# saidwivedi/InteractVLM

Hardware: AMD Instinct MI355X
Metric: images/sec end-to-end contact inference (higher is better)
Workload: dtype f16

## Files before the change

include/ivlm_hip.h:

```cpp
#ifndef IVLM_HIP_H
#define IVLM_HIP_H

#include <stddef.h>
#include <stdint.h>

#ifdef __cplusplus
extern "C" {
#endif

#define IVLM_OK 0
#define IVLM_ERR_INVALID_ARG (-1)
#define IVLM_ERR_WORKSPACE (-2)
#define IVLM_ERR_LAUNCH (-3)
#define IVLM_ERR_UNSUPPORTED (-4)

#define IVLM_F32 0
#define IVLM_BF16 1
#define IVLM_BF16_SPLIT 2
#define IVLM_F16 4
#define IVLM_F16_SPLIT 5
#define IVLM_FP8 3

#define IVLM_GEMM_A_F32 1
#define IVLM_GEMM_RES_F32 2
// ... 170 lines not shown
                     ivlm_stream_t stream);

int ivlm_llama_decode_attn_split(const void *qkv, void *kcache, void *kcache_lo, void *vcache, void *vcache_lo, int tmax, void *o,
                                 int H, int D, int pos, const int32_t *pos_dev, float theta, float scale, const float *cos_tab,
                                 const float *sin_tab, ivlm_stream_t stream);
int ivlm_llama_decode_attn_batch_split(const void *qkv, int64_t ldq, void *kcache, void *kcache_lo, void *vcache, void *vcache_lo,
                                       int64_t cache_stride, int tmax, void *o, int64_t ldo, int B, int H, int D,
                                       const int32_t *pos_dev, float theta, float scale, const float *cos_tab,
                                       const float *sin_tab, ivlm_stream_t stream);

typedef struct {
    int layers, hidden, heads, inter, max_len;
    float eps, theta;
    int fuse_attn_oproj;
} ivlm_llama_cfg;
typedef struct {
    const void *ln1, *qkv, *o, *ln2, *gu, *down;
} ivlm_llama_layer;
size_t ivlm_llama_prefill_workspace_bytes(const ivlm_llama_cfg *cfg, int T);
int ivlm_llama_prefill(const ivlm_llama_cfg *cfg, const ivlm_llama_layer *layers_host, const void *final_norm, void *kcache,
                       void *vcache, const float *cos_tab, const float *sin_tab, const float *x_in, int T, int pos0,
                       float *hidden_out, void *workspace, size_t workspace_bytes, ivlm_stream_t stream);
int ivlm_llama_prefill_f16(const ivlm_llama_cfg *cfg, const ivlm_llama_layer *layers16_host, const void *final_norm, void *kcache16,
                           void *vcache16, const float *cos_tab, const float *sin_tab, const float *x_in, int T, int pos0,
                           float *hidden_out, void *workspace, size_t workspace_bytes, ivlm_stream_t stream);
size_t ivlm_llama_decode_workspace_bytes(const ivlm_llama_cfg *cfg);
int ivlm_llama_decode_step(const ivlm_llama_cfg *cfg, const ivlm_llama_layer *layers_host, const void *final_norm, void *kcache,
                           void *vcache, const float *cos_tab, const float *sin_tab, const float *x_in, int32_t *pos_dev,
                           int advance, float *hidden_out, void *workspace, size_t workspace_bytes, ivlm_stream_t stream);
int ivlm_llama_decode_step_f16kv(const ivlm_llama_cfg *cfg, const ivlm_llama_layer *layers_host, const void *final_norm, void *kcache16,
                                 void *vcache16, const float *cos_tab, const float *sin_tab, const float *x_in, int32_t *pos_dev,
                                 int advance, float *hidden_out, void *workspace, size_t workspace_bytes, ivlm_stream_t stream);
typedef struct {
    const void *Pf, *Ef;
    const int32_t *ebase;
    const int32_t *patch_ptr;
    const int32_t *patch_col;
    const void *patch_val;
} ivlm_bf12m;
typedef struct {
    const void *ln1, *ln2;
    ivlm_bf12m qkv, o, gu, down;
} ivlm_llama_layer_bf12;
int ivlm_llama_decode_step_bf12(const ivlm_llama_cfg *cfg, const ivlm_llama_layer_bf12 *layers_host, const void *final_norm,
                                void *kcache, void *vcache, int cache_dtype, const float *cos_tab, const float *sin_tab,
                                const float *x_in, int32_t *pos_dev, int advance, float *hidden_out, void *workspace,
                                size_t workspace_bytes, ivlm_stream_t stream);
typedef struct {
    int layers_run, hidden, heads, inter, image_size, patch, kpad, tokens;
    float eps;
} ivlm_clip_cfg;
typedef struct {
    const void *patch_w, *pos, *cls_row, *pre_ln_w, *pre_ln_b;
} ivlm_clip_head;
typedef struct {
    const void *ln1_w, *ln1_b, *qkv_w, *qkv_b, *out_w, *out_b, *ln2_w, *ln2_b, *fc1_w, *fc1_b, *fc2_w, *fc2_b;
} ivlm_clip_layer;
size_t ivlm_clip_encode_workspace_bytes(const ivlm_clip_cfg *cfg, int B);
int ivlm_clip_encode(const ivlm_clip_cfg *cfg, const ivlm_clip_head *head, const ivlm_clip_layer *layers_host, const void *images,
                     int B, void *features_out, void *workspace, size_t workspace_bytes, ivlm_stream_t stream);
int ivlm_clip_encode_f16(const ivlm_clip_cfg *cfg, const ivlm_clip_head *head, const ivlm_clip_layer *layers16_host, const void *images,
                         int B, void *features_split_out, void *workspace, size_t workspace_bytes, ivlm_stream_t stream);

typedef struct {
    int embed_dim, depth, heads, grid, window, patch, img_size, out_chans, mlp_dim;
} ivlm_sam_cfg;
typedef struct {
    const void *patch_w, *patch_b, *pos_embed, *neck0_w, *neck1_w, *neck1_b, *neck2_w, *neck3_w, *neck3_b;
} ivlm_sam_head;
typedef struct {
    const void *norm1_w, *norm1_b, *qkv_w, *qkv_b, *rel_h, *rel_w, *rel_cat, *proj_w, *proj_b, *norm2_w, *norm2_b, *lin1_w, *lin1_b,
        *lin2_w, *lin2_b;
    int global_attn;
} ivlm_sam_block;
size_t ivlm_sam_encode_workspace_bytes(const ivlm_sam_cfg *cfg, int V);
int ivlm_sam_encode(const ivlm_sam_cfg *cfg, const ivlm_sam_head *head, const ivlm_sam_block *blocks_host, const void *images, int V,
                    float *embeddings_out, void *workspace, size_t workspace_bytes, ivlm_stream_t stream);
size_t ivlm_sam_encode_parity_workspace_bytes(const ivlm_sam_cfg *cfg, int V);
int ivlm_sam_encode_parity(const ivlm_sam_cfg *cfg, const ivlm_sam_head *head, const ivlm_sam_block *blocks_host, const void *images,
                           int V, float *embeddings_out, void *workspace, size_t workspace_bytes, ivlm_stream_t stream);
typedef struct {
    const void *lin1_w16, *lin2_w16;
} ivlm_sam_mlp_f16;
int ivlm_sam_encode_parity_f16mlp(const ivlm_sam_cfg *cfg, const ivlm_sam_head *head, const ivlm_sam_block *blocks_host,
                                  const ivlm_sam_mlp_f16 *mlp16_host, const void *images, int V, float *embeddings_out,
                                  void *workspace, size_t workspace_bytes, ivlm_stream_t stream);
typedef struct {
    const void *qkv_w16, *proj_w16, *lin1_w16, *lin2_w16, *qkv_b16, *rel_cat16;
} ivlm_sam_block_f16;
size_t ivlm_sam_encode_f16_workspace_bytes(const ivlm_sam_cfg *cfg, int V);
int ivlm_sam_encode_f16(const ivlm_sam_cfg *cfg, const ivlm_sam_head *head, const ivlm_sam_block *blocks_host,
                        const ivlm_sam_block_f16 *blocks16_host, const void *images, int V, float *embeddings_out, void *workspace,
                        size_t workspace_bytes, ivlm_stream_t stream);
int ivlm_bf16_to_f16(const void *src_bf16, void *dst_f16, int64_t n, ivlm_stream_t stream);

typedef struct {
    const void *w2, *b;
    int n, k;
} ivlm_lin;
typedef struct {
    ivlm_lin q, k, v, o;
} ivlm_dec_attn;
typedef struct {
    ivlm_dec_attn self_attn, t2i, i2t;
    const void *norm1_w, *norm1_b, *norm2_w, *norm2_b, *norm3_w, *norm3_b, *norm4_w, *norm4_b;
    ivlm_lin lin1, lin2;
} ivlm_dec_layer;
typedef struct {
    int C, heads, depth;
    const void *no_mask, *key_pe, *out_tokens;
    ivlm_dec_layer layers[4];
    ivlm_dec_attn final_attn;
    const void *norm_final_w, *norm_final_b, *up_ln_w, *up_ln_b;
    ivlm_lin up0, up1, hyper[3], iou[3];
} ivlm_sam_dec;
size_t ivlm_sam_decode_workspace_bytes(int V, int grid, int C, int n_text, int mlp_dim);
int ivlm_sam_decode(const ivlm_sam_dec *weights, int V, int grid, int n_text, const float *image_embeddings,
                    const float *text_embeds, float *low_res_out, float *iou_out, void *workspace, size_t workspace_bytes,
                    ivlm_stream_t stream);

int ivlm_gemm_splitk_choice(int M, int N, int K, int act, int has_rms);
int ivlm_stages_splitk_fused(int on);

int ivlm_gemv1_bf12(const float *x, const void *P, int64_t ldp, const void *E, int64_t lde, const int32_t *ebase,
                    const int32_t *patch_ptr, const int32_t *patch_col, const void *patch_val, void *C, const void *bias,
                    const void *residual, int N, int K, int act, int out_f32, const void *rms_w, float rms_eps, int flags,
                    ivlm_stream_t stream);
int ivlm_gemv1_bf12m(const float *x, const void *Pf, const void *Ef, const int32_t *ebase, const int32_t *patch_ptr,
                     const int32_t *patch_col, const void *patch_val, void *C, const void *bias, const void *residual, int N, int K,
                     int act, int out_f32, const void *rms_w, float rms_eps, int flags, ivlm_stream_t stream);
int ivlm_llama_decode_attn_parts(const float *qkv, int cache_dtype, void *kcache, void *vcache, int tmax, float *parts, int H, int D,
                                 int pos, const int32_t *pos_dev, float theta, float scale, const float *cos_tab, const float *sin_tab,
                                 ivlm_stream_t stream);
int ivlm_gemv1_bf12m_parts(const float *parts, int D, const void *Pf, const void *Ef, const int32_t *ebase, const int32_t *patch_ptr,
                           const int32_t *patch_col, const void *patch_val, void *C, const void *bias, const void *residual, int N, int K,
                           int act, int out_f32, int flags, ivlm_stream_t stream);
int ivlm_pack_bf12m_count(const void *w, int N_valid, int n_rows, int K, int32_t *ebase, int32_t *patch_ptr, ivlm_stream_t stream);
int ivlm_pack_bf12m_fill(const void *w, int N_valid, int n_rows, int K, const int32_t *ebase, const int32_t *patch_ptr, void *Pf, void *Ef,
                         int32_t *patch_col, void *patch_val, ivlm_stream_t stream);
int ivlm_gemv16_bf12m(const float *x, int64_t lda, int M, const void *Pf, const void *Ef, const int32_t *ebase,
                      const int32_t *patch_ptr, const int32_t *patch_col, const void *patch_val, void *C, int64_t ldc, const void *bias,
                      const void *residual, int64_t ldr, int N, int K, int act, int out_f32, const void *rms_w, float rms_eps, int flags,
                      ivlm_stream_t stream);
void ivlm_gemv16_bf12m_tuning(int tiles_per_block);
int ivlm_decode_parts_tuning(int ranges);
void ivlm_gemv1_bf12m_tuning(int wide_max_blocks);
int ivlm_gemv1_bf12m_staging(int form);
int ivlm_unpack_bf12(const void *P, int64_t ldp, const void *E, int64_t lde, const int32_t *ebase, const int32_t *patch_ptr,
                     const int32_t *patch_col, const void *patch_val, int N, int K, void *w_out, ivlm_stream_t stream);

int ivlm_argmax_f32(const float *x, int rows, int cols, int32_t *out, ivlm_stream_t stream);
int ivlm_argmax_f32_bump(const float *x, int rows, int cols, int32_t *out, int32_t *bump, ivlm_stream_t stream);

int ivlm_im2col_nchw(const void *x, void *out, int B, int C, int H, int W, int ks, int stride, int Kpad,
                     ivlm_stream_t stream);
int ivlm_im2col3x3_nhwc(const void *x, void *out, int B, int H, int W, int C, ivlm_stream_t stream);
int ivlm_im2col3x3_nhwc_strided(const void *x, int64_t ldx, void *out, int64_t ldo, int B, int H, int W, int C,
                                ivlm_stream_t stream);
int ivlm_gather_rows(void *dst, int dst_kind, int64_t ldd, const void *src, int src_dtype, int64_t lds, const int32_t *idx,
                     const void *add, int add_dtype, int64_t lda, int64_t rows, int cols, const float *fp8_scale,
                     ivlm_stream_t stream);
int ivlm_amax(const void *x, int dtype, int64_t n, float *out, ivlm_stream_t stream);
int ivlm_add_rows(void *out, int out_kind, const void *a, int a_dtype, const void *b, int b_dtype, int64_t rows, int cols,
                  int64_t b_rows, int op, ivlm_stream_t stream);
int ivlm_fill_rows(void *dst, int64_t ldd, const int32_t *idx, int64_t n_idx, const void *row, int cols,
                   ivlm_stream_t stream);
int ivlm_dense_pe(const void *gauss, void *pe, int pe_dtype, int h, int w, int F, ivlm_stream_t stream);
int ivlm_rope_kv(void *qkv, int64_t ld, int T, int H, int D, int pos0, float theta, void *kcache, void *vcache,
                 const float *cos_tab, const float *sin_tab, ivlm_stream_t stream);
int ivlm_rope_kv_f16(void *qkv, int64_t ld, int T, int H, int D, int pos0, float theta, void *kcache, void *vcache,
                     const float *cos_tab, const float *sin_tab, ivlm_stream_t stream);
int ivlm_rope_kv_split(void *qkv, int64_t ld, int T, int H, int D, int pos0, void *kcache, void *kcache_lo, void *vcache,
                       void *vcache_lo, const float *cos_tab, const float *sin_tab, ivlm_stream_t stream);
int ivlm_llama_attn_oproj(const float *qkv, void *kcache, void *vcache, int tmax, float *attn_scratch, const void *wo,
                          const float *x, float *x_out, int H, int D, float theta, float scale, const float *cos_tab,
                          const float *sin_tab, const int32_t *pos_dev, const int32_t *step_dev, int32_t *counter,
                          int32_t *status, ivlm_stream_t stream);
int ivlm_rope_table(float *cos_tab, float *sin_tab, int T, int D, float theta, ivlm_stream_t stream);
int ivlm_normalize_pad_u8(const uint8_t *src, int H, int W, int y0, int x0, int ch, int cw, const float *mean3_host,
                          const float *std3_host, void *out, int out_bf16, int OH, int OW, ivlm_stream_t stream);
int ivlm_mask_dot(const void *up, const void *hyper, int dtype, float *low, int B, int gh, int gw, int C,
                  ivlm_stream_t stream);

size_t ivlm_h_geo_workspace_bytes(int n);
int ivlm_h_geo_metric(const float *dist, const float *pred, const float *gt, int B, int n, float *out, void *workspace,
                      size_t workspace_bytes, ivlm_stream_t stream);
int ivlm_contact_prf(const float *gt, const float *pred, int B, int n, float thr, float *out, ivlm_stream_t stream);
int ivlm_spmv_csr(const int32_t *row_ptr, const int32_t *col, const float *val, const float *x, int B, int rows,
                  int cols, float *y, ivlm_stream_t stream);

int ivlm_contact_band_census(const float *p, int64_t ld, int B, int Nv, const float *thr, int J, float margin, int32_t *counts,
                             float *mindist, ivlm_stream_t stream);
size_t ivlm_mask_band_census_workspace_bytes(void);
int ivlm_mask_band_census(const float *logits, int V, int64_t HW, const int32_t *ent_pix, const int32_t *row_ptr, int n_rows,
                          float thr_p, float margin_p, int32_t *counts, void *workspace, size_t workspace_bytes,
                          ivlm_stream_t stream);

#define IVLM_SEG_GT_U8 0
#define IVLM_SEG_GT_I32 1
#define IVLM_SEG_GT_F32 2
size_t ivlm_seg_iou_workspace_bytes(int V);
int ivlm_seg_iou_counts(const float *pred, const void *gt, int gt_dtype, int V, int H, int W, int ignore_label, int32_t *out,
                        void *workspace, size_t workspace_bytes, ivlm_stream_t stream);
#define IVLM_AFFORD_MAX_N 4096
#define IVLM_AFFORD_MAX_T 64
int ivlm_afford_metrics(const float *gt, const float *pred, int B, int n, const float *thresholds, int T, float mae_div,
                        float *out, int32_t *valid, ivlm_stream_t stream);

#define IVLM_CONTACT_PAIR_CHAIN 512
size_t ivlm_contact_pair_workspace_bytes(int B, int N_o, int N_h);
int ivlm_contact_pair(const float *o, const float *h, const void *p, const void *q, int p_dtype, int B, int N_o, int N_h,
                      int64_t o_batch_stride, int64_t h_batch_stride, float *value_out, float *grad_o, float *grad_h,
                      void *workspace, size_t workspace_bytes, ivlm_stream_t stream);

#define IVLM_ICP_ESTIMATE_SCALE 1
#define IVLM_ICP_ALLOW_REFLECTION 2
#define IVLM_ICP_REQUERY 4
size_t ivlm_contact_icp_workspace_bytes(int B, int N_o);
int ivlm_contact_icp(const float *x, const float *y, const float *xn, const float *yn, const float *w, const float *init_R,
                     const float *init_T, const float *init_s, int B, int N_o, int N_h, int64_t x_batch_stride, int64_t y_batch_stride,
                     int64_t xn_batch_stride, int64_t yn_batch_stride, int64_t w_batch_stride, int max_iterations, float relative_rmse_thr,
                     int flags, float *R_out, float *T_out, float *s_out, float *rmse_out, int32_t *converged_out, int32_t *iterations_out,
                     int32_t *nn_idx_out, float *hist_R, float *hist_T, float *hist_s, void *workspace, size_t workspace_bytes,
                     ivlm_stream_t stream);

int ivlm_points_align(const float *X, const float *Y, const float *w, int B, int N, int64_t x_batch_stride, int64_t y_batch_stride,
                      int64_t w_batch_stride, int flags, float *R_out, float *T_out, float *s_out, void *workspace, size_t workspace_bytes,
                      ivlm_stream_t stream);

int ivlm_contact_nearest(const float *q, const float *t, int D, int B, int N_o, int N_h, int64_t q_batch_stride, int64_t t_batch_stride,
                         int32_t *idx_out, float *d2_out, ivlm_stream_t stream);

int ivlm_contact_normal_filter(const float *obj_normals, const float *human_normals, int N_o, int N_h, float c_pos, float c_neg,
                               int has_neg, uint8_t *keep_out, ivlm_stream_t stream);

#define IVLM_SILHOUETTE_CHAIN 32
#define IVLM_SILHOUETTE_POS_ULPS 12
#define IVLM_SILHOUETTE_REL_ULPS 6
#define IVLM_SILHOUETTE_EXP_ULPS 3
#define IVLM_SILHOUETTE_T_ULPS 8
size_t ivlm_soft_silhouette_workspace_bytes(int B, int N, int F, int H, int W);
int ivlm_soft_silhouette_forward(const float *verts, const int32_t *faces, int B, int N, int F, int H, int W, float fx, float fy,
                                 float px, float py, float sigma, float blur_radius, float *alpha_out, void *workspace,
                                 size_t workspace_bytes, ivlm_stream_t stream);
int ivlm_soft_silhouette_backward(const float *verts, const int32_t *vert_face_offsets, const int32_t *vert_face_list,
                                  const float *grad_alpha, int B, int N, int F, int H, int W, float fx, float fy, float px, float py,
                                  float sigma, float blur_radius, float *grad_verts_out, void *workspace, size_t workspace_bytes,
                                  ivlm_stream_t stream);

#define IVLM_SILHOUETTE_TERMS_CHAIN 1
#define IVLM_SILHOUETTE_TERMS_WORKSPACE(B, H) ((size_t)(B) * (size_t)(H) * 40)
int ivlm_silhouette_terms(const float *alpha, const float *target, int64_t target_batch_stride, int B, int H, int W, float *loss_out,
                          float *centroid_out, double *sums, const float *g_loss, const float *g_centroid, float *grad_alpha_out,
                          void *workspace, size_t workspace_bytes, ivlm_stream_t stream);

#define IVLM_POSE_CHUNK 1024
#define IVLM_POSE_CHAIN 1
#define IVLM_POSE_FWD_ULPS 6
#define IVLM_POSE_GRAD_ULPS 16
size_t ivlm_pose_transform_workspace_bytes(int B, int N);
int ivlm_pose_transform_forward(const float *verts, const float *rot6d, const float *translation, const float *scale, int B, int N,
                                float *out, ivlm_stream_t stream);
int ivlm_pose_transform_backward(const float *verts, const float *rot6d, const float *scale, const float *grad_out, int B, int N,
                                 float *grad_rot6d, float *grad_translation, float *grad_scale, void *workspace,
                                 size_t workspace_bytes, ivlm_stream_t stream);

size_t ivlm_raster_workspace_bytes(int n_verts_or_points, int H, int W);
int ivlm_rasterize_mesh(const float *verts, int nv, const int32_t *faces, int nf, const float *cam12_host,
                        float fov_deg, int H, int W, int32_t *p2v, float *bary, int32_t *pix_to_face,
                        void *workspace, size_t workspace_bytes, ivlm_stream_t stream);
int ivlm_rasterize_points(const float *pts, int np, const float *cam12_host, float fov_deg, float radius, int H,
                          int W, int32_t *map, void *workspace, size_t workspace_bytes, ivlm_stream_t stream);
int ivlm_phong_shade(const int32_t *p2v, const float *bary, const float *verts, const float *normals, const float *colors,
                     int npix, const float *light3_host, const float *cam3_host, float ambient, float diffuse,
                     float specular, float shininess, const float *bg3_host, uint8_t *out_rgb, ivlm_stream_t stream);

#ifdef __cplusplus
}
#endif
#endif
```

interactvlm_amd/csrc/elementwise.hip:

```cpp
#include "kernels.h"

namespace ivlm {
namespace {

constexpr int kT = 256;

inline int grid_for(int64_t work_items, int max_blocks = 8192) {
    int64_t b = (work_items + kT - 1) / kT;
    if (b < 1) b = 1;
    return (int)(b < max_blocks ? b : max_blocks);
}

__global__ __launch_bounds__(kT) void im2col_nchw_kernel(const bf16_t* __restrict__ x, bf16_t* __restrict__ out, int B,
                                                         int C, int H, int W, int ks, int stride, int Kpad) {
    const int gh = (H - ks) / stride + 1, gw = (W - ks) / stride + 1;
    const int K = C * ks * ks;
    const int64_t total = (int64_t)B * gh * gw * (Kpad >> 3);
    for (int64_t i = (int64_t)blockIdx.x * kT + threadIdx.x; i < total; i += (int64_t)gridDim.x * kT) {
        const int c8 = (int)(i % (Kpad >> 3));
        const int64_t row = i / (Kpad >> 3);
        const int gx = (int)(row % gw), gy = (int)((row / gw) % gh), b = (int)(row / ((int64_t)gw * gh));
        bf16_t v[8];
#pragma unroll
        for (int e = 0; e < 8; ++e) {
            const int col = c8 * 8 + e;
            bf16_t val = 0;
            if (col < K) {
                const int c = col / (ks * ks), r = col - c * ks * ks, ky = r / ks, kx = r - ky * ks;
                val = x[(((int64_t)b * C + c) * H + gy * stride + ky) * W + gx * stride + kx];
            }
            v[e] = val;
        }
        *reinterpret_cast<uint4*>(out + row * Kpad + c8 * 8) = *reinterpret_cast<const uint4*>(v);
    }
}

__global__ __launch_bounds__(kT) void im2col3x3_nhwc_kernel(const bf16_t* __restrict__ x, bf16_t* __restrict__ out,
                                                            int B, int H, int W, int C, int64_t ldx, int64_t ldo) {
    const int c8n = C >> 3;
    const int64_t total = (int64_t)B * H * W * 9 * c8n;
    for (int64_t i = (int64_t)blockIdx.x * kT + threadIdx.x; i < total; i += (int64_t)gridDim.x * kT) {
        const int c8 = (int)(i % c8n);
        const int tap = (int)((i / c8n) % 9);
        const int64_t row = i / ((int64_t)c8n * 9);
        const int xx = (int)(row % W), yy = (int)((row / W) % H), b = (int)(row / ((int64_t)W * H));
        const int sy = yy + tap / 3 - 1, sx = xx + tap % 3 - 1;
        uint4 v = make_uint4(0, 0, 0, 0);
        if (sy >= 0 && sy < H && sx >= 0 && sx < W)
            v = *reinterpret_cast<const uint4*>(x + (((int64_t)b * H + sy) * W + sx) * ldx + c8 * 8);
        *reinterpret_cast<uint4*>(out + row * ldo + tap * C + c8 * 8) = v;
    }
}

__device__ __forceinline__ void load8(const void* base, int kind, int64_t elem, float* f) {
    if (kind == 1) {
        const float4* p = reinterpret_cast<const float4*>(static_cast<const float*>(base) + elem);
        const float4 a = p[0], b = p[1];
        f[0] = a.x; f[1] = a.y; f[2] = a.z; f[3] = a.w; f[4] = b.x; f[5] = b.y; f[6] = b.z; f[7] = b.w;
    } else {
        const uint4 u = *reinterpret_cast<const uint4*>(static_cast<const bf16_t*>(base) + elem);
        f[0] = __uint_as_float(u.x << 16); f[1] = __uint_as_float(u.x & 0xffff0000u);
        f[2] = __uint_as_float(u.y << 16); f[3] = __uint_as_float(u.y & 0xffff0000u);
        f[4] = __uint_as_float(u.z << 16); f[5] = __uint_as_float(u.z & 0xffff0000u);
        f[6] = __uint_as_float(u.w << 16); f[7] = __uint_as_float(u.w & 0xffff0000u);
    }
}
__device__ __forceinline__ uint2 pack_fp8x8(const float* f, float inv_scale) {
    float c[8];
#pragma unroll
    for (int j = 0; j < 8; ++j) c[j] = fminf(fmaxf(f[j] * inv_scale, -448.0f), 448.0f);
    uint32_t a = 0, b = 0;
    a = __builtin_amdgcn_cvt_pk_fp8_f32(c[0], c[1], a, false);
    a = __builtin_amdgcn_cvt_pk_fp8_f32(c[2], c[3], a, true);
    b = __builtin_amdgcn_cvt_pk_fp8_f32(c[4], c[5], b, false);
    b = __builtin_amdgcn_cvt_pk_fp8_f32(c[6], c[7], b, true);
    return make_uint2(a, b);
}

__device__ __forceinline__ void store8(void* base, int kind, int64_t elem, int cols, const float* f, float inv_scale = 1.0f) {
    if (kind == 3) {
        *reinterpret_cast<uint2*>(static_cast<uint8_t*>(base) + elem) = pack_fp8x8(f, inv_scale);
        return;
    }
    if (kind == 1) {
        float4* p = reinterpret_cast<float4*>(static_cast<float*>(base) + elem);
        p[0] = make_float4(f[0], f[1], f[2], f[3]);
        p[1] = make_float4(f[4], f[5], f[6], f[7]);
        return;
    }
    bf16_t* o = static_cast<bf16_t*>(base) + elem;
    *reinterpret_cast<uint4*>(o) = make_uint4(pack_bf16x2(f[0], f[1]), pack_bf16x2(f[2], f[3]), pack_bf16x2(f[4], f[5]),
                                              pack_bf16x2(f[6], f[7]));
    if (kind == 2) {
        float l[8];
#pragma unroll
        for (int j = 0; j < 8; ++j) l[j] = f[j] - bf16_to_f32(f32_to_bf16(f[j]));
        *reinterpret_cast<uint4*>(o + cols) = make_uint4(pack_bf16x2(l[0], l[1]), pack_bf16x2(l[2], l[3]),
                                                         pack_bf16x2(l[4], l[5]), pack_bf16x2(l[6], l[7]));
    }
}

__global__ __launch_bounds__(kT) void gather_rows_kernel(void* __restrict__ dst, int dst_kind, int64_t ldd,
                                                         const void* __restrict__ src, int src_kind, int64_t lds_,
                                                         const int32_t* __restrict__ idx, const void* __restrict__ add,
                                                         int add_kind, int64_t lda, int64_t rows, int cols,
                                                         const float* __restrict__ scale) {
    const int c8n = cols >> 3;
    const int64_t total = rows * c8n;
    const float inv_scale = scale ? 1.0f / *scale : 1.0f;
    for (int64_t i = (int64_t)blockIdx.x * kT + threadIdx.x; i < total; i += (int64_t)gridDim.x * kT) {
        const int c8 = (int)(i % c8n);
        const int64_t r = i / c8n;
        const int64_t s = idx ? (int64_t)idx[r] : r;
        float v[8] = {0.f, 0.f, 0.f, 0.f, 0.f, 0.f, 0.f, 0.f};
        if (s >= 0) load8(src, src_kind, s * lds_ + c8 * 8, v);
        if (add) {
            float a[8];
            load8(add, add_kind, r * lda + c8 * 8, a);
#pragma unroll
            for (int j = 0; j < 8; ++j) v[j] += a[j];
        }
        store8(dst, dst_kind, r * ldd + c8 * 8, cols, v, inv_scale);
    }
}

__global__ __launch_bounds__(kT) void amax_kernel(const void* __restrict__ x, int kind, int64_t n8, float* __restrict__ out) {
    float m = 0.0f;
    for (int64_t i = (int64_t)blockIdx.x * kT + threadIdx.x; i < n8; i += (int64_t)gridDim.x * kT) {
        float v[8];
        load8(x, kind, i * 8, v);
#pragma unroll
        for (int j = 0; j < 8; ++j) m = fmaxf(m, fabsf(v[j]));
    }
    m = wave_max(m);
    if ((threadIdx.x & 63) == 0) atomicMax(reinterpret_cast<unsigned int*>(out), __float_as_uint(m));
}

__global__ __launch_bounds__(kT) void fill_rows_kernel(bf16_t* __restrict__ dst, int64_t ldd, const int32_t* __restrict__ idx,
                                                       int64_t n_idx, const bf16_t* __restrict__ row, int cols) {
    const int c8n = cols >> 3;
    const int64_t total = n_idx * c8n;
    for (int64_t i = (int64_t)blockIdx.x * kT + threadIdx.x; i < total; i += (int64_t)gridDim.x * kT) {
        const int c8 = (int)(i % c8n);
        const int64_t r = idx[i / c8n];
        *reinterpret_cast<uint4*>(dst + r * ldd + c8 * 8) = *reinterpret_cast<const uint4*>(row + c8 * 8);
    }
}

__global__ __launch_bounds__(kT) void bf16_to_f16_kernel(const bf16_t* __restrict__ src, uint16_t* __restrict__ dst, int64_t n) {
    const int64_t n8 = n >> 3;
    for (int64_t i = (int64_t)blockIdx.x * kT + threadIdx.x; i < n8; i += (int64_t)gridDim.x * kT) {
        const uint4 u = *reinterpret_cast<const uint4*>(src + i * 8);
        const uint32_t w[4] = {u.x, u.y, u.z, u.w};
        uint4 o;
        uint32_t* ow = reinterpret_cast<uint32_t*>(&o);
#pragma unroll
        for (int j = 0; j < 4; ++j) ow[j] = pack_f16x2(__uint_as_float(w[j] << 16), __uint_as_float(w[j] & 0xffff0000u));
        *reinterpret_cast<uint4*>(dst + i * 8) = o;
    }
    if (blockIdx.x == 0 && threadIdx.x < (n & 7)) {
        const int64_t i = n8 * 8 + threadIdx.x;
        dst[i] = (uint16_t)(pack_f16x2(bf16_to_f32(src[i]), 0.f) & 0xffffu);
    }
}

__global__ __launch_bounds__(kT) void add_rows_kernel(void* __restrict__ out, int out_kind, const void* __restrict__ a,
                                                      int a_kind, const void* __restrict__ b, int b_kind, int64_t rows,
                                                      int cols, int64_t b_rows, int op) {
    const int c8n = cols >> 3;
    const int64_t total = rows * c8n;
    const int64_t ldo = out_kind == 2 ? 2 * (int64_t)cols : cols;
    for (int64_t i = (int64_t)blockIdx.x * kT + threadIdx.x; i < total; i += (int64_t)gridDim.x * kT) {
        const int c8 = (int)(i % c8n);
        const int64_t r = i / c8n;
        float va[8], vb[8];
        load8(a, a_kind, r * cols + c8 * 8, va);
        load8(b, b_kind, (r % b_rows) * cols + c8 * 8, vb);
#pragma unroll
        for (int j = 0; j < 8; ++j) va[j] = op ? va[j] * vb[j] : va[j] + vb[j];
        store8(out, out_kind, r * ldo + c8 * 8, cols, va);
    }
}

__global__ __launch_bounds__(kT) void dense_pe_kernel(const float* __restrict__ gauss ,
                                                      void* __restrict__ pe , int pe_f32, int h, int w, int F) {
    const int64_t total = (int64_t)h * w * 2 * F;
    for (int64_t i = (int64_t)blockIdx.x * kT + threadIdx.x; i < total; i += (int64_t)gridDim.x * kT) {
        const int c = (int)(i % (2 * F));
        const int64_t p = i / (2 * F);
        const int xx = (int)(p % w), yy = (int)(p / w);
        const int f = c < F ? c : c - F;
        const float cx = 2.0f * (((float)xx + 0.5f) / (float)w) - 1.0f;
        const float cy = 2.0f * (((float)yy + 0.5f) / (float)h) - 1.0f;
        float t = cx * gauss[f] + cy * gauss[F + f];
        t = 6.283185307179586f * t;
        const float val = c < F ? sinf(t) : cosf(t);
        if (pe_f32) static_cast<float*>(pe)[i] = val;
        else static_cast<bf16_t*>(pe)[i] = f32_to_bf16(val);
    }
}

__global__ __launch_bounds__(kT) void rope_table_kernel(float* __restrict__ ct, float* __restrict__ st, int T, int D,
                                                        float theta) {
    const int half = D >> 1;
    const int i = blockIdx.x * kT + threadIdx.x;
    if (i >= T * half) return;
    const int j = i % half, pos = i / half;
    const float ang = (float)pos * powf(theta, -(float)(2 * j) / (float)D);
    ct[i] = cosf(ang);
    st[i] = sinf(ang);
}

template <bool F16>
__global__ __launch_bounds__(kT) void rope_kv_kernel(bf16_t* __restrict__ qkv, int64_t ld, int T, int H, int D,
                                                     int pos0, float theta, bf16_t* __restrict__ kcache,
                                                     bf16_t* __restrict__ vcache, const float* __restrict__ ct,
                                                     const float* __restrict__ stab) {
    const int half = D >> 1;
    const int64_t total = (int64_t)T * H * half;
    for (int64_t i = (int64_t)blockIdx.x * kT + threadIdx.x; i < total; i += (int64_t)gridDim.x * kT) {
        const int j = (int)(i % half);
        const int h = (int)((i / half) % H);
        const int t = (int)(i / ((int64_t)half * H));
        const int pos = pos0 + t;
        float c, s;
        if (ct) {
            c = ct[pos * half + j];
            s = stab[pos * half + j];
        } else {
            const float ang = (float)pos * powf(theta, -(float)(2 * j) / (float)D);
            c = cosf(ang);
            s = sinf(ang);
        }
        bf16_t* row = qkv + (int64_t)t * ld;
        bf16_t* q = row + h * D;
        bf16_t* k = row + (int64_t)H * D + h * D;
        const bf16_t* v = row + 2 * (int64_t)H * D + h * D;
        const float q0 = h16_to_f32<F16>(q[j]), q1 = h16_to_f32<F16>(q[j + half]);
        const float k0 = h16_to_f32<F16>(k[j]), k1 = h16_to_f32<F16>(k[j + half]);
        const bf16_t qa = f32_to_h16<F16>(q0 * c - q1 * s), qb = f32_to_h16<F16>(q1 * c + q0 * s);
        const bf16_t ka = f32_to_h16<F16>(k0 * c - k1 * s), kb = f32_to_h16<F16>(k1 * c + k0 * s);
        q[j] = qa;
        q[j + half] = qb;
        k[j] = ka;
        k[j + half] = kb;
        if (kcache) {
            bf16_t* kc = kcache + ((int64_t)pos * H + h) * D;
            bf16_t* vc = vcache + ((int64_t)pos * H + h) * D;
            kc[j] = ka;
            kc[j + half] = kb;
            vc[j] = v[j];
            vc[j + half] = v[j + half];
        }
    }
}

__global__ __launch_bounds__(kT) void rope_kv_split_kernel(bf16_t* __restrict__ qkv, int64_t ld, int T, int H, int D, int pos0,
                                                           bf16_t* __restrict__ kcache, bf16_t* __restrict__ kcache_lo,
                                                           bf16_t* __restrict__ vcache, bf16_t* __restrict__ vcache_lo,
                                                           const float* __restrict__ ct, const float* __restrict__ stab) {
    const int half = D >> 1;
    const int64_t total = (int64_t)T * H * half;
    const int64_t lo = 3 * (int64_t)H * D;
    for (int64_t i = (int64_t)blockIdx.x * kT + threadIdx.x; i < total; i += (int64_t)gridDim.x * kT) {
        const int j = (int)(i % half);
        const int h = (int)((i / half) % H);
        const int t = (int)(i / ((int64_t)half * H));
        const int pos = pos0 + t;
        const float c = ct[pos * half + j], s = stab[pos * half + j];
        bf16_t* row = qkv + (int64_t)t * ld;
        bf16_t* q = row + h * D;
        bf16_t* k = row + (int64_t)H * D + h * D;
        const bf16_t* v = row + 2 * (int64_t)H * D + h * D;
        auto val = [&](const bf16_t* p, int e) { return bf16_to_f32(p[e]) + bf16_to_f32(p[lo + e]); };
        const float q0 = val(q, j), q1 = val(q, j + half), k0 = val(k, j), k1 = val(k, j + half);
        const float qa = q0 * c - q1 * s, qb = q1 * c + q0 * s, ka = k0 * c - k1 * s, kb = k1 * c + k0 * s;
        auto put = [&](bf16_t* p, int e, float x, bf16_t* ch, bf16_t* cl) {
            const bf16_t hi = f32_to_bf16(x), l = f32_to_bf16(x - bf16_to_f32(hi));
            p[e] = hi;
            p[lo + e] = l;
            if (ch) {
                ch[e] = hi;
                cl[e] = l;
            }
        };
        const int64_t crow = ((int64_t)pos * H + h) * D;
        put(q, j, qa, nullptr, nullptr);
        put(q, j + half, qb, nullptr, nullptr);
        put(k, j, ka, kcache ? kcache + crow : nullptr, kcache ? kcache_lo + crow : nullptr);
        put(k, j + half, kb, kcache ? kcache + crow : nullptr, kcache ? kcache_lo + crow : nullptr);
        if (kcache) {
            vcache[crow + j] = v[j];
            vcache[crow + j + half] = v[j + half];
            vcache_lo[crow + j] = v[lo + j];
            vcache_lo[crow + j + half] = v[lo + j + half];
        }
    }
}

__global__ __launch_bounds__(kT) void mask_dot_kernel(const void* __restrict__ up, const void* __restrict__ hyper, int kind,
                                                      float* __restrict__ low, int B, int gh, int gw, int C) {
    const int64_t total = (int64_t)B * gh * gw * 16;
    for (int64_t i = (int64_t)blockIdx.x * kT + threadIdx.x; i < total; i += (int64_t)gridDim.x * kT) {
        const int sub = (int)(i & 15);
        const int64_t cell = i >> 4;
        const int xx = (int)(cell % gw), yy = (int)((cell / gw) % gh), b = (int)(cell / ((int64_t)gw * gh));
        const int dy = sub >> 3, dx = (sub >> 2) & 1, dy2 = (sub >> 1) & 1, dx2 = sub & 1;
        float acc = 0.0f;
        for (int c = 0; c < C; c += 8) {
            float a[8], h[8];
            load8(up, kind, i * C + c, a);
            load8(hyper, kind, (int64_t)b * C + c, h);
#pragma unroll
            for (int j = 0; j < 8; ++j) acc += a[j] * h[j];
        }
        const int Y = 4 * yy + 2 * dy + dy2, X = 4 * xx + 2 * dx + dx2;
        low[((int64_t)b * 4 * gh + Y) * (4 * gw) + X] = acc;
    }
}

template <typename T>
__global__ __launch_bounds__(kT) void normalize_pad_kernel(const uint8_t* __restrict__ src, int W, int y0, int x0,
                                                           int ch, int cw, float m0, float m1, float m2, float s0,
                                                           float s1, float s2, T* __restrict__ out, int OH, int OW) {
    const int64_t total = (int64_t)OH * OW;
    for (int64_t i = (int64_t)blockIdx.x * kT + threadIdx.x; i < total; i += (int64_t)gridDim.x * kT) {
        const int x = (int)(i % OW), y = (int)(i / OW);
        float r = 0.f, g = 0.f, b = 0.f;
        if (y < ch && x < cw) {
            const uint8_t* p = src + ((int64_t)(y0 + y) * W + (x0 + x)) * 3;
            r = ((float)p[0] - m0) / s0;
            g = ((float)p[1] - m1) / s1;
            b = ((float)p[2] - m2) / s2;
        }
        if (sizeof(T) == 2) {
            reinterpret_cast<bf16_t*>(out)[i] = f32_to_bf16(r);
            reinterpret_cast<bf16_t*>(out)[total + i] = f32_to_bf16(g);
            reinterpret_cast<bf16_t*>(out)[2 * total + i] = f32_to_bf16(b);
        } else {
            reinterpret_cast<float*>(out)[i] = r;
            reinterpret_cast<float*>(out)[total + i] = g;
            reinterpret_cast<float*>(out)[2 * total + i] = b;
        }
    }
}

}

int normalize_pad_u8(const uint8_t* src, int H, int W, int y0, int x0, int ch, int cw, const float* mean3,
                     const float* std3, void* out, int out_bf16, int OH, int OW, hipStream_t st) {
    if (!src || !out || !mean3 || !std3 || y0 < 0 || x0 < 0 || y0 + ch > H || x0 + cw > W || ch > OH || cw > OW)
        return IVLM_ERR_INVALID_ARG;
    const int grid = grid_for((int64_t)OH * OW);
    if (out_bf16)
        normalize_pad_kernel<bf16_t><<<grid, kT, 0, st>>>(src, W, y0, x0, ch, cw, mean3[0], mean3[1], mean3[2], std3[0],
                                                          std3[1], std3[2], static_cast<bf16_t*>(out), OH, OW);
    else
        normalize_pad_kernel<float><<<grid, kT, 0, st>>>(src, W, y0, x0, ch, cw, mean3[0], mean3[1], mean3[2], std3[0],
                                                         std3[1], std3[2], static_cast<float*>(out), OH, OW);
    return ivlm_launch_status();
}

int im2col_nchw(const bf16_t* x, bf16_t* out, int B, int C, int H, int W, int ks, int stride, int Kpad,
                hipStream_t st) {
    if (!x || !out || (Kpad & 7) || Kpad < C * ks * ks) return IVLM_ERR_INVALID_ARG;
    const int gh = (H - ks) / stride + 1, gw = (W - ks) / stride + 1;
    im2col_nchw_kernel<<<grid_for((int64_t)B * gh * gw * (Kpad >> 3)), kT, 0, st>>>(x, out, B, C, H, W, ks, stride, Kpad);
    return ivlm_launch_status();
}
int im2col3x3_nhwc(const bf16_t* x, bf16_t* out, int B, int H, int W, int C, hipStream_t st, int64_t ldx, int64_t ldo) {
    if (!x || !out || (C & 7)) return IVLM_ERR_INVALID_ARG;
    if (ldx == 0) ldx = C;
    if (ldo == 0) ldo = 9 * (int64_t)C;
    if (ldx < C || ldo < 9 * (int64_t)C || ((ldx | ldo) & 7)) return IVLM_ERR_INVALID_ARG;
    im2col3x3_nhwc_kernel<<<grid_for((int64_t)B * H * W * 9 * (C >> 3)), kT, 0, st>>>(x, out, B, H, W, C, ldx, ldo);
    return ivlm_launch_status();
}
int gather_rows(void* dst, int dst_kind, int64_t ldd, const void* src, int src_kind, int64_t lds_, const int32_t* idx,
                const void* add, int add_kind, int64_t lda, int64_t rows, int cols, hipStream_t st, const float* scale) {
    if (!dst || !src || rows <= 0 || (cols & 7) || (ldd & 7) || (lds_ & 7) || (lda & 7)) return IVLM_ERR_INVALID_ARG;
    if (dst_kind < 0 || dst_kind > 3 || (src_kind & ~1) || (add_kind & ~1)) return IVLM_ERR_INVALID_ARG;
    if (dst_kind == 2 && ldd < 2 * (int64_t)cols) return IVLM_ERR_INVALID_ARG;
    if (dst_kind == 3 && !scale) return IVLM_ERR_INVALID_ARG;
    gather_rows_kernel<<<grid_for(rows * (cols >> 3)), kT, 0, st>>>(dst, dst_kind, ldd, src, src_kind, lds_, idx, add,
                                                                    add_kind, lda, rows, cols, scale);
    return ivlm_launch_status();
}
int amax(const void* x, int kind, int64_t n, float* out, hipStream_t st) {
    if (!x || !out || n <= 0 || (n & 7) || (kind & ~1)) return IVLM_ERR_INVALID_ARG;
    amax_kernel<<<grid_for(n >> 3, 2048), kT, 0, st>>>(x, kind, n >> 3, out);
    return ivlm_launch_status();
}
int add_rows(void* out, int out_kind, const void* a, int a_kind, const void* b, int b_kind, int64_t rows, int cols,
             int64_t b_rows, hipStream_t st, int op) {
    if (!out || !a || !b || rows <= 0 || b_rows <= 0 || (cols & 7)) return IVLM_ERR_INVALID_ARG;
    if (out_kind < 0 || out_kind > 2 || (a_kind & ~1) || (b_kind & ~1)) return IVLM_ERR_INVALID_ARG;
    add_rows_kernel<<<grid_for(rows * (cols >> 3)), kT, 0, st>>>(out, out_kind, a, a_kind, b, b_kind, rows, cols, b_rows, op);
    return ivlm_launch_status();
}
int fill_rows(bf16_t* dst, int64_t ldd, const int32_t* idx, int64_t n_idx, const bf16_t* row, int cols, hipStream_t st) {
    if (n_idx == 0) return IVLM_OK;
    if (!dst || !idx || !row || n_idx < 0 || (cols & 7) || (ldd & 7)) return IVLM_ERR_INVALID_ARG;
    fill_rows_kernel<<<grid_for(n_idx * (cols >> 3)), kT, 0, st>>>(dst, ldd, idx, n_idx, row, cols);
    return ivlm_launch_status();
}
int dense_pe(const float* gauss, void* pe, int pe_f32, int h, int w, int F, hipStream_t st) {
    if (!gauss || !pe) return IVLM_ERR_INVALID_ARG;
    dense_pe_kernel<<<grid_for((int64_t)h * w * 2 * F), kT, 0, st>>>(gauss, pe, pe_f32, h, w, F);
    return ivlm_launch_status();
}
int rope_kv(bf16_t* qkv, int64_t ld, int T, int H, int D, int pos0, float theta, bf16_t* kcache, bf16_t* vcache,
            hipStream_t st, const float* cos_tab, const float* sin_tab, int f16) {
    if (!qkv || T <= 0 || (D & 1) || (kcache && !vcache) || (cos_tab && !sin_tab)) return IVLM_ERR_INVALID_ARG;
    if (f16)
        rope_kv_kernel<true><<<grid_for((int64_t)T * H * (D >> 1)), kT, 0, st>>>(qkv, ld, T, H, D, pos0, theta, kcache, vcache,
                                                                                 cos_tab, sin_tab);
    else
        rope_kv_kernel<false><<<grid_for((int64_t)T * H * (D >> 1)), kT, 0, st>>>(qkv, ld, T, H, D, pos0, theta, kcache, vcache,
                                                                                  cos_tab, sin_tab);
    return ivlm_launch_status();
}
int rope_kv_split(bf16_t* qkv, int64_t ld, int T, int H, int D, int pos0, bf16_t* kcache, bf16_t* kcache_lo, bf16_t* vcache,
                  bf16_t* vcache_lo, const float* cos_tab, const float* sin_tab, hipStream_t st) {
    if (!qkv || T <= 0 || (D & 1) || !cos_tab || !sin_tab || ld < 6LL * H * D) return IVLM_ERR_INVALID_ARG;
    if (kcache && (!kcache_lo || !vcache || !vcache_lo)) return IVLM_ERR_INVALID_ARG;
    rope_kv_split_kernel<<<grid_for((int64_t)T * H * (D >> 1)), kT, 0, st>>>(qkv, ld, T, H, D, pos0, kcache, kcache_lo, vcache,
                                                                             vcache_lo, cos_tab, sin_tab);
    return ivlm_launch_status();
}
int rope_table(float* cos_tab, float* sin_tab, int T, int D, float theta, hipStream_t st) {
    if (!cos_tab || !sin_tab || T <= 0 || (D & 1)) return IVLM_ERR_INVALID_ARG;
    rope_table_kernel<<<(T * (D >> 1) + kT - 1) / kT, kT, 0, st>>>(cos_tab, sin_tab, T, D, theta);
    return ivlm_launch_status();
}
int mask_dot(const void* up, const void* hyper, int kind, float* low, int B, int gh, int gw, int C, hipStream_t st) {
    if (!up || !hyper || !low || (C & 7) || (kind & ~1)) return IVLM_ERR_INVALID_ARG;
    mask_dot_kernel<<<grid_for((int64_t)B * gh * gw * 16), kT, 0, st>>>(up, hyper, kind, low, B, gh, gw, C);
    return ivlm_launch_status();
}

}

extern "C" {
#define BF(p) static_cast<bf16_t*>(p)
#define CBF(p) static_cast<const bf16_t*>(p)
int ivlm_im2col_nchw(const void* x, void* out, int B, int C, int H, int W, int ks, int stride, int Kpad,
                     ivlm_stream_t s) {
    ivlm_enter();
    return ivlm::im2col_nchw(CBF(x), BF(out), B, C, H, W, ks, stride, Kpad, ivlm_stream(s));
}
int ivlm_im2col3x3_nhwc(const void* x, void* out, int B, int H, int W, int C, ivlm_stream_t s) {
    ivlm_enter();
    return ivlm::im2col3x3_nhwc(CBF(x), BF(out), B, H, W, C, ivlm_stream(s));
}
int ivlm_im2col3x3_nhwc_strided(const void* x, int64_t ldx, void* out, int64_t ldo, int B, int H, int W, int C, ivlm_stream_t s) {
    ivlm_enter();
    return ivlm::im2col3x3_nhwc(CBF(x), BF(out), B, H, W, C, ivlm_stream(s), ldx, ldo);
}
int ivlm_gather_rows(void* dst, int dst_kind, int64_t ldd, const void* src, int src_dtype, int64_t lds_, const int32_t* idx,
                     const void* add, int add_dtype, int64_t lda, int64_t rows, int cols, const float* fp8_scale,
                     ivlm_stream_t s) {
    ivlm_enter();
    const int k = dst_kind == IVLM_F32 ? 1 : (dst_kind == IVLM_BF16 ? 0 : (dst_kind == IVLM_BF16_SPLIT ? 2 : (dst_kind == IVLM_FP8 ? 3 : -1)));
    return ivlm::gather_rows(dst, k, ldd, src, src_dtype == IVLM_F32, lds_, idx, add, add_dtype == IVLM_F32, lda, rows, cols,
                             ivlm_stream(s), fp8_scale);
}
int ivlm_amax(const void* x, int dtype, int64_t n, float* out, ivlm_stream_t s) {
    ivlm_enter();
    return ivlm::amax(x, dtype == IVLM_F32, n, out, ivlm_stream(s));
}
int ivlm_add_rows(void* out, int out_kind, const void* a, int a_dtype, const void* b, int b_dtype, int64_t rows, int cols,
                  int64_t b_rows, int op, ivlm_stream_t s) {
    ivlm_enter();
    return ivlm::add_rows(out, out_kind == IVLM_F32 ? 1 : (out_kind == IVLM_BF16 ? 0 : (out_kind == IVLM_BF16_SPLIT ? 2 : -1)),
                          a, a_dtype == IVLM_F32, b, b_dtype == IVLM_F32, rows, cols, b_rows, ivlm_stream(s), op);
}
int ivlm_fill_rows(void* dst, int64_t ldd, const int32_t* idx, int64_t n_idx, const void* row, int cols, ivlm_stream_t s) {
    ivlm_enter();
    return ivlm::fill_rows(BF(dst), ldd, idx, n_idx, CBF(row), cols, ivlm_stream(s));
}
int ivlm_dense_pe(const void* gauss, void* pe, int pe_dtype, int h, int w, int F, ivlm_stream_t s) {
    ivlm_enter();
    return ivlm::dense_pe(static_cast<const float*>(gauss), pe, pe_dtype == IVLM_F32, h, w, F, ivlm_stream(s));
}
int ivlm_rope_kv(void* qkv, int64_t ld, int T, int H, int D, int pos0, float theta, void* kcache, void* vcache,
                 const float* cos_tab, const float* sin_tab, ivlm_stream_t s) {
    ivlm_enter();
    return ivlm::rope_kv(BF(qkv), ld, T, H, D, pos0, theta, BF(kcache), BF(vcache), ivlm_stream(s), cos_tab, sin_tab);
}
int ivlm_rope_kv_f16(void* qkv, int64_t ld, int T, int H, int D, int pos0, float theta, void* kcache, void* vcache,
                     const float* cos_tab, const float* sin_tab, ivlm_stream_t s) {
    ivlm_enter();
    return ivlm::rope_kv(BF(qkv), ld, T, H, D, pos0, theta, BF(kcache), BF(vcache), ivlm_stream(s), cos_tab, sin_tab, 1);
}
int ivlm_rope_kv_split(void* qkv, int64_t ld, int T, int H, int D, int pos0, void* kcache, void* kcache_lo, void* vcache,
                       void* vcache_lo, const float* cos_tab, const float* sin_tab, ivlm_stream_t s) {
    ivlm_enter();
    return ivlm::rope_kv_split(BF(qkv), ld, T, H, D, pos0, BF(kcache), BF(kcache_lo), BF(vcache), BF(vcache_lo), cos_tab, sin_tab,
                               ivlm_stream(s));
}
int ivlm_bf16_to_f16(const void* src, void* dst, int64_t n, ivlm_stream_t s) {
    ivlm_enter();
    if (n == 0) return IVLM_OK;
    if (!src || !dst || n < 0 || ((uintptr_t)src & 15) || ((uintptr_t)dst & 15)) return IVLM_ERR_INVALID_ARG;
    ivlm::bf16_to_f16_kernel<<<ivlm::grid_for((n >> 3) + 1), ivlm::kT, 0, ivlm_stream(s)>>>(CBF(src), static_cast<uint16_t*>(dst), n);
    return ivlm_launch_status();
}
int ivlm_rope_table(float* cos_tab, float* sin_tab, int T, int D, float theta, ivlm_stream_t s) {
    ivlm_enter();
    return ivlm::rope_table(cos_tab, sin_tab, T, D, theta, ivlm_stream(s));
}
int ivlm_mask_dot(const void* up, const void* hyper, int dtype, float* low, int B, int gh, int gw, int C, ivlm_stream_t s) {
    ivlm_enter();
    return ivlm::mask_dot(up, hyper, dtype == IVLM_F32, low, B, gh, gw, C, ivlm_stream(s));
}
int ivlm_normalize_pad_u8(const uint8_t* src, int H, int W, int y0, int x0, int ch, int cw, const float* mean3_host,
                          const float* std3_host, void* out, int out_bf16, int OH, int OW, ivlm_stream_t s) {
    ivlm_enter();
    return ivlm::normalize_pad_u8(src, H, W, y0, x0, ch, cw, mean3_host, std3_host, out, out_bf16, OH, OW,
                                  ivlm_stream(s));
}
#undef BF
#undef CBF
}
```

interactvlm_amd/csrc/gemv.hip:

```cpp
#include <stdlib.h>

#include <algorithm>

#include "gemv_common.h"

namespace ivlm {
namespace {

constexpr int kMaxM = 8;

__device__ __forceinline__ float dot8(const u32x4_t& w, const u32x4_t& x) {
    float acc = 0.0f;
#pragma unroll
    for (int j = 0; j < 4; ++j) {
        acc += __uint_as_float(w[j] << 16) * __uint_as_float(x[j] << 16);
        acc += __uint_as_float(w[j] & 0xffff0000u) * __uint_as_float(x[j] & 0xffff0000u);
    }
    return acc;
}

__device__ __forceinline__ float dot8f(const u32x4_t& w, const f32x4v_t& xa, const f32x4v_t& xb) {
    float acc = __uint_as_float(w[0] << 16) * xa[0];
    acc = fmaf(__uint_as_float(w[0] & 0xffff0000u), xa[1], acc);
    acc = fmaf(__uint_as_float(w[1] << 16), xa[2], acc);
// ... 157 lines not shown
                } else {
                    bf16_t* C = static_cast<bf16_t*>(g.C) + (int64_t)m * g.ldc;
                    C[n0] = f32_to_bf16(v0);
                    if (n1 != n0) C[n1] = f32_to_bf16(v1);
                }
            }
        }
#pragma unroll
        for (int m = 0; m < M; ++m) a0[m] = a1[m] = 0.0f;
    };

    u32x4_t wa0[U], wb0[U], wa1[U], wb1[U];
    if (nsteps > 0) issue(wa0, wb0, 0);
    if (XLDS) prologue();
    for (int s2 = 0; s2 < nsteps; s2 += 2) {
        if (s2 + 1 < nsteps) issue(wa1, wb1, s2 + 1);
        consume(wa0, wb0, s2);
        if (s2 + 1 < nsteps) {
            if (s2 + 2 < nsteps) issue(wa0, wb0, s2 + 2);
            consume(wa1, wb1, s2 + 1);
        }
    }
}

constexpr int kG1Waves = kRowWaves;

template <bool RMS, int KS>
__global__ __launch_bounds__(64 * kG1Waves, 8) void gemv1_kernel(GemmArgs g) {
    extern __shared__ __attribute__((aligned(16))) unsigned char smem[];
    __shared__ float s_red[kG1Waves];
    __shared__ float s_val[kG1Waves];
    constexpr int U = 8 / KS;
    const int lane = threadIdx.x & 63, wave = threadIdx.x >> 6;
    const int nchunk = g.K >> 3;
    f32x4v_t* xf = reinterpret_cast<f32x4v_t*>(smem);
    const int row = blockIdx.x * (kG1Waves / KS) + wave / KS;
    const bool live = row < g.N;
    const u32x4_t* wp = reinterpret_cast<const u32x4_t*>(g.W + (int64_t)(live ? row : g.N - 1) * g.ldw);
    const int cpp = KS == 1 ? nchunk : ((nchunk + 64 * KS - 1) / (64 * KS)) * 64;
    const int c_lo = (wave % KS) * cpp, c_hi = min(nchunk, c_lo + cpp);
    u32x4_t w[U];
#pragma unroll
    for (int u = 0; u < U; ++u) w[u] = __builtin_nontemporal_load(wp + min(c_lo + lane + 64 * u, nchunk - 1));
    stage_row_f32<RMS, false>(g, xf, nchunk, 64 * kG1Waves, s_red, lane, wave);
    __syncthreads();
    float acc = 0.0f;
    constexpr int UH = U / 2;
    for (int c = c_lo + lane; c < c_hi; c += 64 * U) {
#pragma unroll
        for (int hf = 0; hf < 2; ++hf) {
#pragma unroll
            for (int u = hf * UH; u < (hf + 1) * UH; ++u) {
                const int cc = c + 64 * u;
                if (cc < c_hi) acc += dot8f(w[u], xf[cc], xf[nchunk + cc]);
            }
#pragma unroll
            for (int u = hf * UH; u < (hf + 1) * UH; ++u) {
                const int nc = c + 64 * (U + u);
                if (nc < c_hi) w[u] = __builtin_nontemporal_load(wp + nc);
            }
        }
    }
    acc = wave_sum(acc);
    if (KS > 1) {
        if (lane == 0) s_val[wave] = acc;
        __syncthreads();
        if (wave % KS) return;
        acc = s_val[wave];
#pragma unroll
        for (int i = 1; i < KS; ++i) acc += s_val[wave + i];
    }
    finish_row<RMS, KS == 1>(g, acc, row, live, lane, wave, s_red, s_val);
}

typedef __attribute__((ext_vector_type(2))) float f32x2v_t;

__device__ __forceinline__ float dot16_fp8(const u32x4_t& w, const f32x4v_t& a0, const f32x4v_t& a1, const f32x4v_t& b0,
                                           const f32x4v_t& b1, float acc) {
    const f32x4v_t* xs[4] = {&a0, &a1, &b0, &b1};
#pragma unroll
    for (int j = 0; j < 4; ++j) {
        const f32x2v_t lo = __builtin_amdgcn_cvt_pk_f32_fp8(w[j], false);
        const f32x2v_t hi = __builtin_amdgcn_cvt_pk_f32_fp8(w[j], true);
        const f32x4v_t& x = *xs[j];
        acc = fmaf(lo[0], x[0], acc);
        acc = fmaf(lo[1], x[1], acc);
        acc = fmaf(hi[0], x[2], acc);
        acc = fmaf(hi[1], x[3], acc);
    }
    return acc;
}

template <bool RMS>
__global__ __launch_bounds__(64 * kG1Waves, 8) void gemv1_fp8w_kernel(GemmArgs g) {
    extern __shared__ __attribute__((aligned(16))) unsigned char smem[];
    __shared__ float s_red[kG1Waves];
    __shared__ float s_val[kG1Waves];
    constexpr int U = 4;
    const int lane = threadIdx.x & 63, wave = threadIdx.x >> 6;
    const int nchunk = g.K >> 3;
    const int nw16 = g.K >> 4;
    f32x4v_t* xf = reinterpret_cast<f32x4v_t*>(smem);
    const int row = blockIdx.x * kG1Waves + wave;
    const bool live = row < g.N;
    const u32x4_t* wp = reinterpret_cast<const u32x4_t*>(reinterpret_cast<const uint8_t*>(g.W) + (int64_t)(live ? row : g.N - 1) * g.ldw);
    u32x4_t w[U];
#pragma unroll
    for (int u = 0; u < U; ++u) w[u] = __builtin_nontemporal_load(wp + min(lane + 64 * u, nw16 - 1));
    stage_row_f32<RMS, false>(g, xf, nchunk, 64 * kG1Waves, s_red, lane, wave);
    __syncthreads();
    float acc = 0.0f;
    for (int c = lane; c < nw16; c += 64 * U) {
        if (c != lane) {
#pragma unroll
            for (int u = 0; u < U; ++u)
                if (c + 64 * u < nw16) w[u] = __builtin_nontemporal_load(wp + c + 64 * u);
        }
#pragma unroll
        for (int u = 0; u < U; ++u) {
            const int cc = c + 64 * u;
            if (cc < nw16) acc = dot16_fp8(w[u], xf[2 * cc], xf[nchunk + 2 * cc], xf[2 * cc + 1], xf[nchunk + 2 * cc + 1], acc);
        }
    }
    acc = wave_sum(acc) * (*g.scale_w);
    finish_row<RMS>(g, acc, row, live, lane, wave, s_red, s_val);
}

int g_gemv1_ksplit = 0;
int g_gemv1_lds_floor = 0;

template <bool RMS, int KS>
static void launch_gemv1_ks(const GemmArgs& g, hipStream_t st) {
    const int rows_per_block = kG1Waves / KS;
    const int blocks = (g.N + rows_per_block - 1) / rows_per_block;
    size_t lds = (size_t)g.K * 4;
    if (blocks <= 256 && (size_t)g_gemv1_lds_floor > lds) lds = (size_t)g_gemv1_lds_floor;
    ivlm_launch_lds_cap<gemv1_kernel<RMS, KS>>(128 * 1024, dim3(blocks), dim3(64 * kG1Waves), lds, st, g);
}

static int launch_gemv1(const GemmArgs& g, hipStream_t st) {
    int ks = g_gemv1_ksplit > 0 ? g_gemv1_ksplit : 1;
    if (g.act == ACT_SWIGLU || g.K < 2048) ks = 1;
    if (ks == 2) {
        if (g.rms_w) launch_gemv1_ks<true, 2>(g, st);
        else launch_gemv1_ks<false, 2>(g, st);
    } else {
        if (g.rms_w) launch_gemv1_ks<true, 1>(g, st);
        else launch_gemv1_ks<false, 1>(g, st);
    }
    return ivlm_launch_status();
}

__global__ __launch_bounds__(1024) void argmax_kernel(const float* __restrict__ x, int cols, int32_t* __restrict__ out,
                                                      int32_t* __restrict__ bump) {
    __shared__ float sv[16];
    __shared__ int si[16];
    const float* r = x + (int64_t)blockIdx.x * cols;
    float best = -INFINITY;
    int bi = 0x7fffffff;
    auto take = [&](float v, int i) {
        if (v > best || (v == best && i < bi)) {
            best = v;
            bi = i;
        }
    };
    const int head = (int)(((16 - ((uintptr_t)r & 15)) & 15) >> 2);
    const int nhead = head < cols ? head : cols;
    if ((int)threadIdx.x < nhead) take(r[threadIdx.x], threadIdx.x);
    const int nvec = (cols - nhead) >> 2;
    const float4* rv = reinterpret_cast<const float4*>(r + nhead);
    for (int i = threadIdx.x; i < nvec; i += 1024) {
        const float4 v = rv[i];
        const int c = nhead + 4 * i;
        take(v.x, c);
        take(v.y, c + 1);
        take(v.z, c + 2);
        take(v.w, c + 3);
    }
    for (int i = nhead + 4 * nvec + threadIdx.x; i < cols; i += 1024) take(r[i], i);
#pragma unroll
    for (int off = 32; off > 0; off >>= 1) {
        const float ov = __shfl_xor(best, off, 64);
        const int oi = __shfl_xor(bi, off, 64);
        if (ov > best || (ov == best && oi < bi)) {
            best = ov;
            bi = oi;
        }
    }
    if ((threadIdx.x & 63) == 0) {
        sv[threadIdx.x >> 6] = best;
        si[threadIdx.x >> 6] = bi;
    }
    __syncthreads();
    if (threadIdx.x == 0) {
        for (int w = 1; w < 16; ++w)
            if (sv[w] > best || (sv[w] == best && si[w] < bi)) {
                best = sv[w];
                bi = si[w];
            }
        out[blockIdx.x] = bi;
        if (bump) bump[blockIdx.x] += 1;
    }
}

}

int g_gemv_max_blocks_per_cu = 0, g_gemv_rows2_min_n = 0;
int g_gemv_legacy = 0;
static int gemv_cu_count() {
    static int cus = 0;
    if (cus == 0) {
        int dev = 0;
        if (hipGetDevice(&dev) != hipSuccess || hipDeviceGetAttribute(&cus, hipDeviceAttributeMultiprocessorCount, dev) != hipSuccess ||
            cus <= 0)
            cus = 256;
    }
    return cus;
}

template <int M>
static int launch_gemv(const GemmArgs& g, hipStream_t st) {
    const size_t xbytes = (size_t)M * g.K * (g.a_f32 ? 4 : 2);
    const bool xlds = xbytes <= (g.a_f32 ? 60 : 48) * 1024;
    if (g.rms_w && !xlds) return IVLM_ERR_UNSUPPORTED;
    const int rows2_min = g_gemv_rows2_min_n > 0 ? g_gemv_rows2_min_n : 8192;
    const bool rows2 = g.act == ACT_SWIGLU || g.N > rows2_min;
    const int ngroups = rows2 ? (g.N + 1) / 2 : g.N;
    const size_t lds = xlds ? xbytes : 0;
    int per_cu = g_gemv_max_blocks_per_cu > 0 ? g_gemv_max_blocks_per_cu : 4;
    if (lds > 0) per_cu = std::min<int>(per_cu, std::max<int>(1, (int)((160 * 1024) / (lds + 512))));
    const int slots = gemv_cu_count() * per_cu;
    const int gpw = std::max(1, (ngroups + 4 * slots - 1) / (4 * slots));
    const int blocks = (ngroups + 4 * gpw - 1) / (4 * gpw);
#define IVLM_GEMV_GO(ROWS, RMS, XL, AF)                                                                            \
    do {                                                                                                           \
        constexpr auto kfn = gemv_kernel<M, ROWS, RMS, XL, AF>;                                                    \
        if (lds > 48 * 1024) ivlm_launch_lds_cap<kfn>(64 * 1024, dim3(blocks), dim3(256), lds, st, g);             \
        else ivlm_launch(kfn, dim3(blocks), dim3(256), lds, st, g);                                                \
    } while (0)
#define IVLM_GEMV_ROWS(ROWS)                                                                   \
    if (g.a_f32) {                                                                             \
        if (g.rms_w) IVLM_GEMV_GO(ROWS, true, true, true);                                     \
        else if (xlds) IVLM_GEMV_GO(ROWS, false, true, true);                                  \
        else IVLM_GEMV_GO(ROWS, false, false, true);                                           \
    } else {                                                                                   \
        if (g.rms_w) IVLM_GEMV_GO(ROWS, true, true, false);                                    \
        else if (xlds) IVLM_GEMV_GO(ROWS, false, true, false);                                 \
        else IVLM_GEMV_GO(ROWS, false, false, false);                                          \
    }
    if (rows2) { IVLM_GEMV_ROWS(2) } else { IVLM_GEMV_ROWS(1) }
#undef IVLM_GEMV_ROWS
#undef IVLM_GEMV_GO
    return ivlm_launch_status();
}

int gemv_bf16(const GemmArgs& g, hipStream_t st) {
    if (!g.A || !g.W || !g.C || g.M <= 0 || g.M > kMaxM || g.N <= 0 || g.K <= 0) return IVLM_ERR_INVALID_ARG;
    if ((g.K & 7) || (g.lda & (g.a_f32 ? 3 : 7)) || (g.ldw & 7) || g.batch != 1) return IVLM_ERR_UNSUPPORTED;
    if (g.act == ACT_SWIGLU && ((g.N & 1) || g.residual)) return IVLM_ERR_UNSUPPORTED;
    if (g.M == 1 && g.a_f32 && (size_t)g.K * 4 <= 60 * 1024 && !g_gemv_legacy) return launch_gemv1(g, st);
    switch (g.M) {
        case 1: return launch_gemv<1>(g, st);
        case 2: return launch_gemv<2>(g, st);
        case 3: return launch_gemv<3>(g, st);
        case 4: return launch_gemv<4>(g, st);
        case 5: return launch_gemv<5>(g, st);
        case 6: return launch_gemv<6>(g, st);
        case 7: return launch_gemv<7>(g, st);
        default: return launch_gemv<8>(g, st);
    }
}

int gemv1_fp8w(const GemmArgs& g, hipStream_t st) {
    if (!g.A || !g.W || !g.C || !g.scale_w || g.M != 1 || !g.a_f32 || g.N <= 0 || g.K <= 0) return IVLM_ERR_INVALID_ARG;
    if ((g.K & 15) || (g.ldw & 15) || (size_t)g.K * 4 > 60 * 1024) return IVLM_ERR_UNSUPPORTED;
    if (g.act == ACT_SWIGLU && ((g.N & 1) || g.residual)) return IVLM_ERR_UNSUPPORTED;
    const dim3 grid((g.N + kG1Waves - 1) / kG1Waves), block(64 * kG1Waves);
    if (g.rms_w) ivlm_launch_lds_cap<gemv1_fp8w_kernel<true>>(64 * 1024, grid, block, (size_t)g.K * 4, st, g);
    else ivlm_launch_lds_cap<gemv1_fp8w_kernel<false>>(64 * 1024, grid, block, (size_t)g.K * 4, st, g);
    return ivlm_launch_status();
}

int argmax_f32(const float* x, int rows, int cols, int32_t* out, hipStream_t st, int32_t* bump) {
    if (!x || !out || rows <= 0 || cols <= 0) return IVLM_ERR_INVALID_ARG;
    argmax_kernel<<<rows, 1024, 0, st>>>(x, cols, out, bump);
    return ivlm_launch_status();
}

}

extern "C" int ivlm_gemv_tuning(int max_blocks_per_cu, int rows2_min_n) {
    ivlm::g_gemv_legacy = max_blocks_per_cu < 0 ? 1 : 0;
    ivlm::g_gemv_max_blocks_per_cu = max_blocks_per_cu > 0 ? max_blocks_per_cu : 0;
    ivlm::g_gemv_rows2_min_n = rows2_min_n;
    return 0;
}

extern "C" void ivlm_gemv1_tuning(int ksplit) { ivlm::g_gemv1_ksplit = ksplit; }
extern "C" void ivlm_gemv1_lds_floor(int bytes) { ivlm::g_gemv1_lds_floor = bytes < 0 ? 0 : (bytes > 128 * 1024 ? 128 * 1024 : bytes); }

extern "C" int ivlm_gemv_fp8w(const float* x, const void* Wq, int64_t ldw, const float* scale_w, void* C, const void* bias,
                              const void* residual, int N, int K, int act, int out_f32, const void* rms_w, float rms_eps, int flags,
                              ivlm_stream_t stream) {
    ivlm_enter();
    ivlm::GemmArgs g = ivlm::gemv_row_args(x, C, bias, residual, N, K, act, out_f32, rms_w, rms_eps, flags);
    g.W = static_cast<const bf16_t*>(Wq);
    g.ldw = ldw;
    g.scale_w = scale_w;
    return ivlm::gemv1_fp8w(g, ivlm_stream(stream));
}

extern "C" int ivlm_argmax_f32(const float* x, int rows, int cols, int32_t* out, ivlm_stream_t stream) {
    ivlm_enter();
    return ivlm::argmax_f32(x, rows, cols, out, ivlm_stream(stream), nullptr);
}

extern "C" int ivlm_argmax_f32_bump(const float* x, int rows, int cols, int32_t* out, int32_t* bump, ivlm_stream_t stream) {
    ivlm_enter();
    return ivlm::argmax_f32(x, rows, cols, out, ivlm_stream(stream), bump);
}
```

interactvlm_amd/csrc/kernels.h:

```cpp
#pragma once
#include "ivlm_common.h"

namespace ivlm {

enum Act : int { ACT_NONE = 0, ACT_GELU = 1, ACT_QUICK_GELU = 2, ACT_RELU = 3, ACT_SILU = 4, ACT_SWIGLU = 5, ACT_SIGMOID = 6 };

struct SplitKFused {
    int32_t* count = nullptr;
    void* C = nullptr;
    const bf16_t* bias = nullptr;
    const bf16_t* residual = nullptr;
    int64_t ldc = 0, ldr = 0, c_lo = 0;
    int res_mod = 0, act = 0, out_f32 = 0, out_f16 = 0, out_split = 0, res_f32 = 0;
};
constexpr int kSplitKCounters = 4096;

struct GemmArgs {
    const bf16_t* A = nullptr;
    const bf16_t* W = nullptr;
    void* C = nullptr;
    const bf16_t* bias = nullptr;
    const bf16_t* residual = nullptr;
    int64_t lda = 0, ldw = 0, ldc = 0, ldr = 0;
    int res_mod = 0;
// ... 29 lines not shown

int layernorm(const void* x, int x_f32, const bf16_t* w, const bf16_t* b, void* y, int y_f32, int64_t rows, int cols, float eps,
              hipStream_t st, int gelu = 0, const int32_t* out_rows = nullptr, const float* fp8_scale = nullptr);
int rmsnorm(const void* x, int x_f32, const bf16_t* w, void* y, int y_f32, int64_t rows, int cols, float eps, hipStream_t st,
            const float* fp8_scale = nullptr);

struct AttnArgs {
    const bf16_t *q, *k, *v;
    bf16_t* o;
    int64_t q_bs, q_hs, q_rs;
    int64_t k_bs, k_hs, k_rs;
    int64_t v_bs, v_hs, v_rs;
    int64_t o_bs, o_hs, o_rs;
    int B, H, Sq, Sk, D;
    float scale;
    int causal;
    int q_pos0;
    const float* rel_h;
    const float* rel_w;
    int rel_kh, rel_kw;
    int kv_batch_div;
    int prescale_q;
    const bf16_t *q_lo = nullptr, *k_lo = nullptr, *v_lo = nullptr;
    bf16_t* o_lo = nullptr;
    int xcd_map = 1;
    int q_lo_level = 0;
    int f16 = 0;
};

int attention_bf16(const AttnArgs& a, hipStream_t st);
int attention_f32(const float* q, const float* k, const float* v, float* o, const int64_t* st12, int B, int H, int Sq, int Sk,
                  int D, float scale, int kv_div, hipStream_t st);
int relpos_bias(const bf16_t* q, int64_t q_bs, int64_t q_hs, int64_t q_rs, const bf16_t* tab_h, const bf16_t* tab_w,
                int B, int H, int SH, int SW, int D, float* rel_h, float* rel_w, hipStream_t st, const bf16_t* q_lo = nullptr);

int im2col_nchw(const bf16_t* x, bf16_t* out, int B, int C, int H, int W, int ks, int stride, int Kpad, hipStream_t st);
int im2col3x3_nhwc(const bf16_t* x, bf16_t* out, int B, int H, int W, int C, hipStream_t st, int64_t ldx = 0, int64_t ldo = 0);
int rope_kv_split(bf16_t* qkv, int64_t ld, int T, int H, int D, int pos0, bf16_t* kcache, bf16_t* kcache_lo, bf16_t* vcache,
                  bf16_t* vcache_lo, const float* cos_tab, const float* sin_tab, hipStream_t st);
int gather_rows(void* dst, int dst_kind, int64_t ldd, const void* src, int src_kind, int64_t lds_, const int32_t* idx,
                const void* add, int add_kind, int64_t lda, int64_t rows, int cols, hipStream_t st, const float* scale = nullptr);
int amax(const void* x, int kind, int64_t n, float* out, hipStream_t st);
int add_rows(void* out, int out_kind, const void* a, int a_kind, const void* b, int b_kind, int64_t rows, int cols,
             int64_t b_rows, hipStream_t st, int op = 0);
int fill_rows(bf16_t* dst, int64_t ldd, const int32_t* idx, int64_t n_idx, const bf16_t* row, int cols, hipStream_t st);
int dense_pe(const float* gauss, void* pe, int pe_f32, int h, int w, int F, hipStream_t st);
int rope_kv(bf16_t* qkv, int64_t ld, int T, int H, int D, int pos0, float theta, bf16_t* kcache, bf16_t* vcache,
            hipStream_t st, const float* cos_tab = nullptr, const float* sin_tab = nullptr, int f16 = 0);
int rope_table(float* cos_tab, float* sin_tab, int T, int D, float theta, hipStream_t st);
int normalize_pad_u8(const uint8_t* src, int H, int W, int y0, int x0, int ch, int cw, const float* mean3,
                     const float* std3, void* out, int out_bf16, int OH, int OW, hipStream_t st);
int mask_dot(const void* up, const void* hyper, int kind, float* low, int B, int gh, int gw, int C, hipStream_t st);

int contact_prf(const float* gt, const float* pred, int B, int n, float thr, float* out, hipStream_t st);
int spmv_csr(const int32_t* row_ptr, const int32_t* col, const float* val, const float* x, int B, int rows, int cols,
             float* y, hipStream_t st);

int contact_band_census(const float* p, int64_t ld, int B, int nv, const float* thr, int J, float margin, int32_t* counts,
                        float* mindist, hipStream_t st);
size_t mask_band_census_workspace_bytes();
int mask_band_census(const float* logits, int V, int64_t HW, const int32_t* ent_pix, const int32_t* row_ptr, int n_rows,
                     float thr_p, float margin_p, int32_t* counts, void* ws, size_t ws_bytes, hipStream_t st);

size_t seg_iou_workspace_bytes(int V);
int seg_iou_counts(const float* pred, const void* gt, int gt_dtype, int V, int H, int W, int ignore_label, int32_t* out, void* ws,
                   size_t ws_bytes, hipStream_t st);
int afford_metrics(const float* gt, const float* pred, int B, int n, const float* thresholds, int T, float mae_div, float* out,
                   int32_t* valid, hipStream_t st);

size_t contact_pair_workspace_bytes(int B, int n_o, int n_h);
int contact_pair(const float* o, const float* h, const void* p, const void* q, int p_dtype, int B, int n_o, int n_h,
                 int64_t o_bstride, int64_t h_bstride, float* value, float* grad_o, float* grad_h, void* ws, size_t ws_bytes,
                 hipStream_t st);

size_t soft_silhouette_workspace_bytes(int B, int N, int F, int H, int W);
int soft_silhouette_forward(const float* verts, const int32_t* faces, int B, int N, int F, int H, int W, float fx, float fy, float px,
                            float py, float sigma, float blur, float* alpha, void* ws, size_t ws_bytes, hipStream_t st);
int soft_silhouette_backward(const float* verts, const int32_t* vf_off, const int32_t* vf_list, const float* galpha, int B, int N, int F,
                             int H, int W, float fx, float fy, float px, float py, float sigma, float blur, float* gverts, void* ws,
                             size_t ws_bytes, hipStream_t st);
int silhouette_terms(const float* alpha, const float* target, int64_t t_bstride, int B, int H, int W, float* loss, float* centroid,
                     double* sums, const float* g_loss, const float* g_centroid, float* galpha, void* ws, size_t ws_bytes,
                     hipStream_t st);

size_t pose_transform_workspace_bytes(int B, int N);
int pose_transform_forward(const float* verts, const float* rot6d, const float* trans, const float* scale, int B, int N, float* out,
                           hipStream_t st);
int pose_transform_backward(const float* verts, const float* rot6d, const float* scale, const float* grad_out, int B, int N,
                            float* grad_r6, float* grad_t, float* grad_s, void* ws, size_t ws_bytes, hipStream_t st);

size_t contact_icp_workspace_bytes(int B, int n_o);
int contact_icp(const float* x, const float* y, const float* xn, const float* yn, const float* w, const float* init_R, const float* init_T,
                const float* init_s, int B, int n_o, int n_h, int64_t x_bs, int64_t y_bs, int64_t xn_bs, int64_t yn_bs, int64_t w_bs,
                int max_iterations, float relative_rmse_thr, int flags, float* R, float* T, float* s, float* rmse, int32_t* converged,
                int32_t* iterations, int32_t* nn_idx, float* hist_R, float* hist_T, float* hist_s, void* ws, size_t ws_bytes,
                hipStream_t st);
int points_align(const float* X, const float* Y, const float* w, int B, int n, int64_t x_bs, int64_t y_bs, int64_t w_bs, int flags,
                 float* R, float* T, float* s, void* ws, size_t ws_bytes, hipStream_t st);
int contact_nearest(const float* q, const float* t, int D, int B, int n_o, int n_h, int64_t q_bs, int64_t t_bs, int32_t* idx, float* d2,
                    hipStream_t st);
int contact_normal_filter(const float* on, const float* hn, int n_o, int n_h, float c_pos, float c_neg, int has_neg, uint8_t* keep,
                          hipStream_t st);

size_t raster_workspace_bytes(int n_prims_verts, int H, int W);
int rasterize_mesh(const float* verts, int nv, const int32_t* faces, int nf, const float* cam12_host, float fov_deg,
                   int H, int W, int32_t* p2v, float* bary, int32_t* pix_to_face, void* ws, size_t ws_bytes,
                   hipStream_t st);
int rasterize_points(const float* pts, int np, const float* cam12_host, float fov_deg, float radius, int H, int W,
                     int32_t* map, void* ws, size_t ws_bytes, hipStream_t st);

int phong_shade(const int32_t* p2v, const float* bary, const float* verts, const float* normals, const float* colors, int npix,
                const float* light3_host, const float* cam3_host, float ambient, float diffuse, float specular, float shininess,
                const float* bg3_host, uint8_t* out, hipStream_t st);

int llama_decode_attn(const void* qkv, int io_f32, bf16_t* kcache, bf16_t* vcache, int tmax, void* o, int H, int D, int pos,
                      float theta, float scale, hipStream_t st, const float* cos_tab = nullptr, const float* sin_tab = nullptr,
                      const int32_t* pos_dev = nullptr, bf16_t* kcache_lo = nullptr, bf16_t* vcache_lo = nullptr, int cache_f16 = 0);
int llama_decode_attn_batch(const void* qkv, int io_f32, int64_t ldq, bf16_t* kcache, bf16_t* vcache, int64_t cache_stride,
                            int tmax, void* o, int64_t ldo, int B, int H, int D, const int32_t* pos_dev, float theta, float scale,
                            const float* cos_tab, const float* sin_tab, hipStream_t st, bf16_t* kcache_lo = nullptr,
                            bf16_t* vcache_lo = nullptr, int cache_f16 = 0);

size_t llama_decode_attn_splitkv_scratch_bytes(int H, int D);
int llama_decode_attn_splitkv(const float* qkv, bf16_t* kcache, bf16_t* vcache, int tmax, float* o, int H, int D, int pos, float theta,
                              float scale, hipStream_t st, const float* cos_tab, const float* sin_tab, const int32_t* pos_dev,
                              int cache_f16, void* scratch, size_t scratch_bytes);

extern int g_decode_parts_S;
constexpr int kDecodePartsMaxS = 4;
__host__ __device__ constexpr int decode_parts_stride(int D) { return D + 4; }
int llama_decode_attn_parts(const float* qkv, bf16_t* kcache, bf16_t* vcache, int tmax, float* parts, int H, int D, int pos, float theta,
                            float scale, hipStream_t st, const float* cos_tab, const float* sin_tab, const int32_t* pos_dev,
                            int cache_f16);

size_t llama_decode_attn_batch_prefix_scratch_bytes(int B, int H, int D);
int llama_decode_attn_batch_prefix(const void* qkv, int io_f32, int64_t ldq, bf16_t* kcache, bf16_t* vcache, int64_t cache_stride,
                                   int tmax, void* o, int64_t ldo, int B, int H, int D, const int32_t* pos_dev,
                                   const int32_t* prefix_len_dev, float theta, float scale, const float* cos_tab,
                                   const float* sin_tab, int cache_f16, void* scratch, size_t scratch_bytes, hipStream_t st);
int llama_verify_attn(const float* qkv, int k, bf16_t* kcache, bf16_t* vcache, int tmax, float* o, int H, int D, const int32_t* pos_dev,
                      float theta, float scale, const float* cos_tab, const float* sin_tab, int cache_f16, hipStream_t st);
int spec_accept(const int32_t* amax, const int32_t* fed, const int32_t* nd_dev, int k, int32_t* n_acc, int32_t* tok, int32_t* pos,
                hipStream_t st);

int llama_attn_oproj(const float* qkv, bf16_t* kcache, bf16_t* vcache, int tmax, float* attn_scratch, const bf16_t* wo,
                     const float* x, float* x_out, int H, int D, float theta, float scale, const float* cos_tab,
                     const float* sin_tab, const int32_t* pos_dev, const int32_t* step_dev, int32_t* counter, int32_t* status,
                     hipStream_t st);
int gemm_splitk_choice(int M, int N, int K, int act, int has_rms);

int gemv_bf16(const GemmArgs& g, hipStream_t st);
int gemv1_fp8w(const GemmArgs& g, hipStream_t st);
int gemv_mfma_bf16(const GemmArgs& g, hipStream_t st);
int argmax_f32(const float* x, int rows, int cols, int32_t* out, hipStream_t st, int32_t* bump = nullptr);

}
```

interactvlm_amd/csrc/norm.hip:

```cpp
#include "kernels.h"

namespace ivlm {
namespace {

constexpr int kMaxChunks = 16;

__device__ __forceinline__ void unpack8(const uint4& u, float* f) {
    f[0] = __uint_as_float(u.x << 16); f[1] = __uint_as_float(u.x & 0xffff0000u);
    f[2] = __uint_as_float(u.y << 16); f[3] = __uint_as_float(u.y & 0xffff0000u);
    f[4] = __uint_as_float(u.z << 16); f[5] = __uint_as_float(u.z & 0xffff0000u);
    f[6] = __uint_as_float(u.w << 16); f[7] = __uint_as_float(u.w & 0xffff0000u);
}
__device__ __forceinline__ uint4 pack8(const float* f) {
    return make_uint4(pack_bf16x2(f[0], f[1]), pack_bf16x2(f[2], f[3]), pack_bf16x2(f[4], f[5]),
                      pack_bf16x2(f[6], f[7]));
}

template <bool RMS, int MAXC, bool GELU, bool XF32, bool YF32>
__global__ __launch_bounds__(256) void norm_kernel(const void* __restrict__ xv, const bf16_t* __restrict__ w,
                                                   const bf16_t* __restrict__ b, void* __restrict__ yv, int64_t rows,
                                                   int cols, float eps, const int32_t* __restrict__ out_rows,
                                                   const float* __restrict__ fp8_scale, int y_split) {
    const int lane = threadIdx.x & 63;
    const int64_t row = (int64_t)blockIdx.x * 4 + (threadIdx.x >> 6);
    if (row >= rows) return;
    const int nchunk = cols >> 3;
    const uint4* xr = reinterpret_cast<const uint4*>(static_cast<const bf16_t*>(xv) + row * cols);
    const float4* xr4 = reinterpret_cast<const float4*>(static_cast<const float*>(xv) + row * cols);
    float v[MAXC][8];
    float s = 0.0f;
#pragma unroll
    for (int c = 0; c < MAXC; ++c) {
        const int idx = c * 64 + lane;
        if (idx < nchunk) {
            if (XF32) {
                const float4 a = xr4[2 * idx], bq = xr4[2 * idx + 1];
                v[c][0] = a.x; v[c][1] = a.y; v[c][2] = a.z; v[c][3] = a.w;
                v[c][4] = bq.x; v[c][5] = bq.y; v[c][6] = bq.z; v[c][7] = bq.w;
            } else {
                unpack8(xr[idx], v[c]);
            }
#pragma unroll
            for (int j = 0; j < 8; ++j) s += RMS ? v[c][j] * v[c][j] : v[c][j];
        }
    }
    s = wave_sum(s);
    float mean = 0.0f, rstd;
    if (RMS) {
        rstd = rsqrtf(s / (float)cols + eps);
    } else {
        mean = s / (float)cols;
        float q = 0.0f;
#pragma unroll
        for (int c = 0; c < MAXC; ++c) {
            if (c * 64 + lane < nchunk) {
#pragma unroll
                for (int j = 0; j < 8; ++j) {
                    const float d = v[c][j] - mean;
                    q += d * d;
                }
            }
        }
        q = wave_sum(q);
        rstd = rsqrtf(q / (float)cols + eps);
    }
    const int64_t orow = out_rows ? (int64_t)out_rows[row] : row;
    uint4* yr = reinterpret_cast<uint4*>(static_cast<bf16_t*>(yv) + orow * ((y_split & 1) ? 2 * cols : cols));
    float4* yr4 = reinterpret_cast<float4*>(static_cast<float*>(yv) + orow * cols);
    const uint4* wr = reinterpret_cast<const uint4*>(w);
    const uint4* br = reinterpret_cast<const uint4*>(b);
#pragma unroll
    for (int c = 0; c < MAXC; ++c) {
        const int idx = c * 64 + lane;
        if (idx < nchunk) {
            float wv[8], o[8];
            unpack8(wr[idx], wv);
            if (RMS) {
#pragma unroll
                for (int j = 0; j < 8; ++j)
                    o[j] = (XF32 ? v[c][j] * rstd : bf16_to_f32(f32_to_bf16(v[c][j] * rstd))) * wv[j];
            } else {
                float bv[8];
                unpack8(br[idx], bv);
#pragma unroll
                for (int j = 0; j < 8; ++j) {
                    o[j] = (v[c][j] - mean) * rstd * wv[j] + bv[j];
                    if (GELU) o[j] = 0.5f * o[j] * (1.0f + erff(o[j] * 0.70710678118654752f));
                }
            }
            if (!YF32 && fp8_scale) {
                const float inv = 1.0f / *fp8_scale;
                float cl[8];
#pragma unroll
                for (int j = 0; j < 8; ++j) cl[j] = fminf(fmaxf(o[j] * inv, -448.0f), 448.0f);
                uint32_t a = 0, bq = 0;
                a = __builtin_amdgcn_cvt_pk_fp8_f32(cl[0], cl[1], a, false);
                a = __builtin_amdgcn_cvt_pk_fp8_f32(cl[2], cl[3], a, true);
                bq = __builtin_amdgcn_cvt_pk_fp8_f32(cl[4], cl[5], bq, false);
                bq = __builtin_amdgcn_cvt_pk_fp8_f32(cl[6], cl[7], bq, true);
                reinterpret_cast<uint2*>(static_cast<uint8_t*>(yv) + orow * cols)[idx] = make_uint2(a, bq);
            } else if (YF32) {
                yr4[2 * idx] = make_float4(o[0], o[1], o[2], o[3]);
                yr4[2 * idx + 1] = make_float4(o[4], o[5], o[6], o[7]);
            } else if (y_split == 2) {
                yr[idx] = make_uint4(pack_f16x2(o[0], o[1]), pack_f16x2(o[2], o[3]), pack_f16x2(o[4], o[5]), pack_f16x2(o[6], o[7]));
            } else if (y_split) {
                uint32_t h[4], l[4];
#pragma unroll
                for (int j = 0; j < 4; ++j) split_16x2(o[2 * j], o[2 * j + 1], h[j], l[j], y_split == 3);
                yr[idx] = make_uint4(h[0], h[1], h[2], h[3]);
                yr[nchunk + idx] = make_uint4(l[0], l[1], l[2], l[3]);
            } else {
                yr[idx] = pack8(o);
            }
        }
    }
}

}

template <bool RMS, int MAXC, bool GELU>
static void launch_norm(const void* x, int x_f32, const bf16_t* w, const bf16_t* b, void* y, int y_f32, int64_t rows, int cols,
                        float eps, hipStream_t st, const int32_t* out_rows = nullptr, const float* fp8_scale = nullptr) {
    const unsigned grid = (unsigned)((rows + 3) / 4);
    const int y_split = y_f32 == 2 ? 1 : (y_f32 == 4 ? 2 : (y_f32 == 5 ? 3 : 0));
    if (x_f32 && y_f32 == 1) norm_kernel<RMS, MAXC, GELU, true, true><<<grid, 256, 0, st>>>(x, w, b, y, rows, cols, eps, out_rows, fp8_scale, 0);
    else if (x_f32) norm_kernel<RMS, MAXC, GELU, true, false><<<grid, 256, 0, st>>>(x, w, b, y, rows, cols, eps, out_rows, fp8_scale, y_split);
    else if (y_f32 == 1) norm_kernel<RMS, MAXC, GELU, false, true><<<grid, 256, 0, st>>>(x, w, b, y, rows, cols, eps, out_rows, fp8_scale, 0);
    else norm_kernel<RMS, MAXC, GELU, false, false><<<grid, 256, 0, st>>>(x, w, b, y, rows, cols, eps, out_rows, fp8_scale, y_split);
}

int layernorm(const void* x, int x_f32, const bf16_t* w, const bf16_t* b, void* y, int y_f32, int64_t rows, int cols, float eps,
              hipStream_t st, int gelu, const int32_t* out_rows, const float* fp8_scale) {
    if (!x || !w || !b || !y || rows <= 0 || cols <= 0) return IVLM_ERR_INVALID_ARG;
    if ((cols & 7) || cols > kMaxChunks * 512) return IVLM_ERR_UNSUPPORTED;
    if (gelu) {
        if (cols > 4 * 512) return IVLM_ERR_UNSUPPORTED;
        launch_norm<false, 4, true>(x, x_f32, w, b, y, y_f32, rows, cols, eps, st, out_rows);
    } else if (cols <= 4 * 512) {
        launch_norm<false, 4, false>(x, x_f32, w, b, y, y_f32, rows, cols, eps, st, out_rows, fp8_scale);
    } else {
        launch_norm<false, kMaxChunks, false>(x, x_f32, w, b, y, y_f32, rows, cols, eps, st, out_rows);
    }
    return ivlm_launch_status();
}

int rmsnorm(const void* x, int x_f32, const bf16_t* w, void* y, int y_f32, int64_t rows, int cols, float eps, hipStream_t st,
            const float* fp8_scale) {
    if (!x || !w || !y || rows <= 0 || cols <= 0) return IVLM_ERR_INVALID_ARG;
    if ((cols & 7) || cols > kMaxChunks * 512) return IVLM_ERR_UNSUPPORTED;
    if (fp8_scale && y_f32) return IVLM_ERR_INVALID_ARG;
    if (cols <= 4 * 512) launch_norm<true, 4, false>(x, x_f32, w, nullptr, y, y_f32, rows, cols, eps, st, nullptr, fp8_scale);
    else launch_norm<true, kMaxChunks, false>(x, x_f32, w, nullptr, y, y_f32, rows, cols, eps, st, nullptr, fp8_scale);
    return ivlm_launch_status();
}

}

extern "C" {

int ivlm_layernorm(const void* x, int x_dtype, const void* w, const void* b, void* y, int y_dtype, int64_t rows, int cols,
                   float eps, int gelu, const int32_t* out_rows, const float* fp8_scale, ivlm_stream_t stream) {
    ivlm_enter();
    if ((y_dtype == IVLM_FP8) != (fp8_scale != nullptr)) return IVLM_ERR_INVALID_ARG;
    if (y_dtype == IVLM_FP8 && (gelu || cols > 2048)) return IVLM_ERR_UNSUPPORTED;
    return ivlm::layernorm(x, x_dtype == IVLM_F32, static_cast<const bf16_t*>(w), static_cast<const bf16_t*>(b), y,
                           y_dtype == IVLM_F32 ? 1 : (y_dtype == IVLM_BF16_SPLIT ? 2 : (y_dtype == IVLM_F16 ? 4 : (y_dtype == IVLM_F16_SPLIT ? 5 : 0))),
                           rows, cols, eps, ivlm_stream(stream), gelu, out_rows, fp8_scale);
}

int ivlm_rmsnorm_fp8(const void* x, int x_dtype, const void* w, void* y, int64_t rows, int cols, float eps, const float* fp8_scale,
                     ivlm_stream_t stream) {
    ivlm_enter();
    if (!fp8_scale) return IVLM_ERR_INVALID_ARG;
    return ivlm::rmsnorm(x, x_dtype == IVLM_F32, static_cast<const bf16_t*>(w), y, 0, rows, cols, eps, ivlm_stream(stream), fp8_scale);
}

int ivlm_rmsnorm(const void* x, int x_dtype, const void* w, void* y, int y_dtype, int64_t rows, int cols, float eps,
                 ivlm_stream_t stream) {
    ivlm_enter();
    return ivlm::rmsnorm(x, x_dtype == IVLM_F32, static_cast<const bf16_t*>(w), y,
                         y_dtype == IVLM_F32 ? 1 : (y_dtype == IVLM_BF16_SPLIT ? 2 : (y_dtype == IVLM_F16 ? 4 : (y_dtype == IVLM_F16_SPLIT ? 5 : 0))),
                         rows, cols, eps, ivlm_stream(stream));
}

}
```

interactvlm_amd/decoding.py:

```python
from __future__ import annotations

import torch

from . import ops
from .constants import IMAGE_TOKEN_INDEX

_ring = None

SHARED_PREFIX_MODES = ("default", "bf16")


def shared_prefix_len(prompts, one_picture, mode="default", fp8=False, image_rows=256, image_id=IMAGE_TOKEN_INDEX):
    prompts = [[int(t) for t in p] for p in prompts]
    B = len(prompts)
    if B < 2 or not one_picture or fp8 or mode not in SHARED_PREFIX_MODES:
        return 0
    n = 0
    while n < min(len(p) for p in prompts) and all(p[n] == prompts[0][n] for p in prompts):
        n += 1
    spliced = lambda ids: len(ids) + sum(image_rows - 1 for t in ids if t == image_id)
    T0 = [spliced(p) for p in prompts]
    P = min(spliced(prompts[0][:n]), min(T0) - 1)
    if P <= 16 or sum(T0) - B * P <= 16:
        return 0
    return P


def _id_ring(n):
    global _ring
    if _ring is None or _ring.numel() < n:
        _ring = torch.empty(max(n, 64), dtype=torch.int32, pin_memory=torch.cuda.is_available())
    return _ring


class _Step:
    st = None

    def __init__(self, llm, hidden):
        self.llm, self.hidden = llm, hidden

    def event(self):
        ev = torch.cuda.Event()
        ev.record(torch.cuda.current_stream(self.hidden.device))
        return ev


class SingleGraph(_Step):

    def __init__(self, llm, hidden, T0):
        super().__init__(llm, hidden)
        self.st, self.pos = llm.decode_graph(T0), T0

    def __call__(self, tok, out=None):
        st = self.st
        if isinstance(tok, torch.Tensor):
            st["tok"].copy_(tok)
        else:
            st["tok"].fill_(tok)
        st["graph"].replay()
        self.hidden[self.pos: self.pos + 1].copy_(st["hidden"])
        self.pos += 1
        return st["nxt"].clone() if out is None else out.copy_(st["nxt"])

    def resume(self, n, v):
        self.pos += n
        self.st["pos"].copy_(v["pos"])
        self.st["tok"].copy_(v["tok"])


class SingleEager(_Step):

    def __init__(self, llm, hidden, T0):
        super().__init__(llm, hidden)
        self.pos = T0

    def __call__(self, tok, out=None):
        llm = self.llm
        if not isinstance(tok, torch.Tensor):
            tok = torch.tensor([tok], dtype=torch.int32, device=self.hidden.device)
        h = llm.forward(llm.embed_ids(tok), self.pos)
        self.hidden[self.pos: self.pos + 1].copy_(h)
        self.pos += 1
        nxt = ops.argmax(llm.logits(h))
        return nxt if out is None else out.copy_(nxt)

    def resume(self, n, v):
        self.pos += n


class BatchGraph(_Step):

    def __init__(self, llm, hidden, pos, prefix=None):
        super().__init__(llm, hidden)
        self.st = llm.decode_graph_batch(pos.numel(), pos, prefix)
        self.rows = torch.arange(pos.numel(), device=pos.device)

    def __call__(self, tok, out=None):
        st = self.st
        st["tok"].copy_(tok)
        idx = st["pos"].to(torch.int64)
        st["graph"].replay()
        nxt = st["nxt"].clone() if out is None else st["nxt"]
        self.hidden[self.rows, idx] = st["hidden"]
        return nxt if out is None else out.copy_(nxt)


class BatchEager(_Step):

    def __init__(self, llm, hidden, pos, caches, prefix=None):
        super().__init__(llm, hidden)
        self.pos, self.caches = pos, caches
        self.prefix = None if prefix is None else torch.tensor([int(prefix)], dtype=torch.int32, device=pos.device)
        self.rows = torch.arange(pos.numel(), device=pos.device)

    def __call__(self, tok, out=None):
        llm = self.llm
        h = llm.decode_step_batch(llm.embed_ids(tok.contiguous()), self.pos, *self.caches, prefix=self.prefix)
        idx = self.pos.to(torch.int64)
        nxt = ops.argmax(llm.logits(h))
        self.pos = self.pos + 1
        self.hidden[self.rows, idx] = h
        return nxt if out is None else out.copy_(nxt)


def greedy(step, nxt, n_seq, eos, forced=None):
    B, n_max = len(n_seq), max(n_seq)
    new = [[] for _ in range(B)]
    done = [False] * B

    def absorb(toks):
        for b in range(B):
            if not done[b]:
                new[b].append(int(toks[b]))
                done[b] = toks[b] == eos or len(new[b]) >= n_seq[b]
        return all(done)

    if forced is not None:
        host, dev = forced
        amax = [nxt]
        for s in range(n_max):
            if absorb([f[s] for f in host]):
                break
            amax.append(step(dev[s]))
        return new, amax
    ring = _id_ring(n_max * B)[: n_max * B].view(n_max, B)
    ids = torch.empty(n_max, B, dtype=torch.int32, device=nxt.device)
    ids[0].copy_(nxt)
    ring[0].copy_(nxt, non_blocking=True)
    evs, amax = [step.event()], []

    def read():
        s = len(amax)
        evs[s].synchronize()
        amax.append(ids[s])
        return absorb(ring[s].tolist())

    for s in range(n_max - 1):
        if s >= 1 and read():
            break
        ring[s + 1].copy_(step(ids[s], out=ids[s + 1]), non_blocking=True)
        evs.append(step.event())
    while not all(done):
        read()
    return new, amax


def speculative(step, nxt, n_max, eos, draft):
    llm = step.llm
    kmax = max(llm.VERIFY_BUCKETS)
    new_ids, amax = [int(nxt.item())], [nxt]
    stats = dict(passes=0, plain_steps=0, proposed=0, accepted=0, pattern=[])
    observe = getattr(draft, "observe", None)
    while new_ids[-1] != eos and len(new_ids) < n_max:
        rem = n_max - len(new_ids)
        prop = [int(t) for t in draft.propose(list(new_ids), kmax)][: min(kmax - 1, rem - 1)]
        m = len(prop)
        if m == 0:
            stats["plain_steps"] += 1
            amax.append(step(new_ids[-1]))
            new_ids.append(int(amax[-1].item()))
            continue
        kb = next(b for b in llm.VERIFY_BUCKETS if b >= m + 1)
        fed = torch.tensor([new_ids[-1]] + prop + [new_ids[-1]] * (kb - 1 - m), dtype=torch.int32)
        st = llm.verify_graph(kb) if step.st is not None else llm.verify_state(kb)
        st["pos"].fill_(step.pos)
        st["ids"].copy_(fed)
        st["nd"].fill_(m)
        if step.st is not None:
            st["graph"].replay()
        else:
            llm.verify_pass(st)
        n_acc, tok = torch.cat([st["n_acc"], st["tok"]]).tolist()
        stats["passes"] += 1
        stats["proposed"] += m
        stats["accepted"] += n_acc
        stats["pattern"].append((m, n_acc))
        if observe is not None:
            observe(m, n_acc)
        va = st["amax"][: n_acc + 1].clone()
        keep = 0
        for e in prop[:n_acc] + [tok]:
            new_ids.append(e)
            keep += 1
            if e == eos or len(new_ids) >= n_max:
                break
        step.hidden[step.pos: step.pos + keep].copy_(st["hidden"][:keep])
        amax.extend(va[j: j + 1] for j in range(keep))
        step.resume(keep, st)
    return new_ids, amax, stats
```

interactvlm_amd/llava.py:

```python
from __future__ import annotations

import collections
import os

import torch

from . import _lib, graphs, ops
from .sam import _LN, _Lin, _dev
from .weights import CLIP_PREFIX, ClipCfg, LlamaCfg

BF16 = torch.bfloat16
F32 = torch.float32

_GraphKey = collections.namedtuple("_GraphKey", "batched B precision packed fp8 fused verify prefix", defaults=(False, False))


class ClipTower:

    def __init__(self, w, cfg: ClipCfg, device, prefix=CLIP_PREFIX):
        self.cfg, self.device = cfg, device
        self._graphs = graphs.Cache()
        self._patch_rows = {}
        e = prefix + ".embeddings"
        K = 3 * cfg.patch * cfg.patch
        self.kpad = ((K + 63) // 64) * 64
        pw = w[e + ".patch_embedding.weight"].reshape(cfg.hidden, K)
        self.patch_w = _dev(torch.nn.functional.pad(pw, (0, self.kpad - K)), device)
        pos = w[e + ".position_embedding.weight"]
        self.pos = _dev(pos, device)
        self.cls_row = (w[e + ".class_embedding"].float() + pos[0].float()).reshape(1, -1).to(device).contiguous()
        self.pre_ln = _LN(w, prefix + ".pre_layrnorm", device, cfg.eps)
        n_run = cfg.layers + 1 + cfg.select_layer if cfg.select_layer < 0 else cfg.select_layer
        self.layers = []
        for i in range(n_run):
            p = f"{prefix}.encoder.layers.{i}"
            qkv_w = torch.cat([w[f"{p}.self_attn.{n}_proj.weight"] for n in "qkv"], 0)
            qkv_b = torch.cat([w[f"{p}.self_attn.{n}_proj.bias"] for n in "qkv"], 0)
            self.layers.append(dict(
                ln1=_LN(w, p + ".layer_norm1", device, cfg.eps), ln2=_LN(w, p + ".layer_norm2", device, cfg.eps),
                qkv_w=_dev(qkv_w, device), qkv_b=_dev(qkv_b, device), out=_Lin(w, p + ".self_attn.out_proj", device),
                fc1=_Lin(w, p + ".mlp.fc1", device), fc2=_Lin(w, p + ".mlp.fc2", device)))

    use_graph = graphs.ON

    def __call__(self, images):
        if not graphs.enabled(self.use_graph, images):
            return self._forward(images)
        return self._graphs.run((images.shape[0], self.precision, self.fp8), self._forward, [images], BF16)

    precision = "default"

    def _f16(self, L):
        if "qkv_h" not in L:
            L["qkv_h"] = ops.f16_weight(L["qkv_w"], "clip qkv")
            for n in ("out", "fc1", "fc2"):
                L[n + "_h"] = ops.f16_weight(L[n].w, "clip " + n)
        return L

    fp8 = False
    _calibrating = False

    def enable_fp8(self, calib_images):
        dev = self.device
        for L in self.layers:
            for n, w_ in (("qkv", L["qkv_w"]), ("out", L["out"].w), ("fc1", L["fc1"].w), ("fc2", L["fc2"].w)):
                L[n + "_q"], L[n + "_s"] = ops.quantize_fp8(w_)
            L["amax"] = {k: torch.zeros(1, dtype=F32, device=dev) for k in ("y1", "a", "y2", "h")}
        self._calibrating = True
        try:
            self._forward(calib_images.to(dev))
        finally:
            self._calibrating = False
        for L in self.layers:
            L["s"] = {k: (v / 448.0).clamp_(min=1e-12) for k, v in L["amax"].items()}
        self.fp8 = True
        self._graphs.clear()

    def _attention(self, qkv, B, split=False):
        c = self.cfg
        T, H, hd = c.tokens, c.heads, c.hidden // c.heads
        if split:
            q6 = qkv.view(B, T, 2, 3, H, hd)
            (q, k, v), (q_lo, k_lo, v_lo) = ([q6[:, :, j, i].permute(0, 2, 1, 3) for i in range(3)] for j in range(2))
            return ops.attention_split(q, q_lo, k, k_lo, v, v_lo, hd ** -0.5, prescale_q=True)
        q, k, v = (qkv.view(B, T, 3, H, hd)[:, :, i].permute(0, 2, 1, 3) for i in range(3))
        return ops.attention(q, k, v, hd ** -0.5, prescale_q=True).permute(0, 2, 1, 3).reshape(B * T, c.hidden)

    def _forward(self, images):
        c = self.cfg
        B = images.shape[0]
        T = c.tokens
        cols = ops.im2col_nchw(images.to(BF16).contiguous(), c.patch, c.patch, self.kpad)
        x = torch.empty(B, T, c.hidden, dtype=F32, device=images.device)
        for b in range(B):
            ops.linear(cols[b * (T - 1): (b + 1) * (T - 1)], self.patch_w, residual=self.pos[1:], out=x[b, 1:])
            ops.gather_rows(self.cls_row, out=x[b, 0:1])
        x = self.pre_ln(x.view(B * T, c.hidden), out_f32=True)
        norm, lin_in, lin_out = Llama._PREFILL_FLAGS[self.precision]
        split = self.precision == "parity"
        for L in self.layers:
            if self.fp8:
                sc = L["s"]
                a = self._attention(ops.linear_fp8(L["ln1"](x, fp8_scale=sc["y1"]), L["qkv_q"], sc["y1"], L["qkv_s"], L["qkv_b"]), B)
                aq = ops.gather_rows(a, out_kind="fp8", scale=sc["a"])
                x = ops.linear_fp8(aq, L["out_q"], sc["a"], L["out_s"], L["out"].b, residual=x, out_kind="f32")
                h8 = ops.linear_fp8(L["ln2"](x, fp8_scale=sc["y2"]), L["fc1_q"], sc["y2"], L["fc1_s"], L["fc1"].b, act="quick_gelu",
                                    out_kind="fp8", scale_out=sc["h"])
                x = ops.linear_fp8(h8, L["fc2_q"], sc["h"], L["fc2_s"], L["fc2"].b, residual=x, out_kind="f32")
                continue
            wq, wo, w1, w2 = (tuple(self._f16(L)[n + "_h"] for n in ("qkv", "out", "fc1", "fc2")) if self.precision == "f16"
                              else (L["qkv_w"], L["out"].w, L["fc1"].w, L["fc2"].w))
            y = L["ln1"](x, **norm)
            a = self._attention(ops.linear(y, wq, L["qkv_b"], **lin_in), B, split)
            x = ops.linear(a, wo, L["out"].b, residual=x, out_f32=True, **lin_out)
            y2 = L["ln2"](x, **norm)
            h = ops.linear(y2, w1, L["fc1"].b, act="quick_gelu", **lin_in)
            cal = L.get("amax") if self._calibrating and self.precision == "default" else None
            if cal:
                for k_, t_ in (("y1", y), ("a", a), ("y2", y2), ("h", h)):
                    ops.amax(t_, cal[k_])
            x = ops.linear(h, w2, L["fc2"].b, residual=x, out_f32=True, **lin_out)
        if B not in self._patch_rows:
            r = torch.arange(B * T, dtype=torch.int32).view(B, T)[:, 1:].reshape(-1)
            self._patch_rows[B] = r.to(images.device)
        kind = "bf16" if self.precision == "default" else "split"
        return ops.gather_rows(x, self._patch_rows[B], out_kind=kind).view(B, T - 1, -1)


class _LayerW(dict):

    MATS = ("qkv", "o", "gu", "down")

    def __missing__(self, k):
        p = dict.get(self, k + "_p") if k in self.MATS else None
        if p is None:
            raise KeyError(k)
        w = p.unpack().contiguous()
        self[k] = w
        return w


class Llama:

    MAX_LEN_LIMIT = 4096

    def __init__(self, w, cfg: LlamaCfg, device, prefix="model", max_len=640):
        if max_len > self.MAX_LEN_LIMIT:
            raise ops.IvlmError(f"max_len={max_len}: the KV-cached decode kernels support at most {self.MAX_LEN_LIMIT} positions")
        self.cfg, self.device, self.max_len = cfg, device, max_len
        self.embed = _dev(w[prefix + ".embed_tokens.weight"], device)
        self.layers = []
        for i in range(cfg.layers):
            p = f"{prefix}.layers.{i}"
            qkv = torch.cat([w[f"{p}.self_attn.{n}_proj.weight"] for n in "qkv"], 0)
            gu = torch.stack([w[p + ".mlp.gate_proj.weight"], w[p + ".mlp.up_proj.weight"]], 1).reshape(
                2 * cfg.inter, cfg.hidden)
            self.layers.append(_LayerW(
                ln1=_dev(w[p + ".input_layernorm.weight"], device), ln2=_dev(w[p + ".post_attention_layernorm.weight"], device),
                qkv=_dev(qkv, device), o=_dev(w[p + ".self_attn.o_proj.weight"], device), gu=_dev(gu, device),
                down=_dev(w[p + ".mlp.down_proj.weight"], device)))
        self.norm = _dev(w[prefix + ".norm.weight"], device)
        self.lm_head = _dev(w["lm_head.weight"], device)
        H, hd = cfg.heads, cfg.hidden // cfg.heads
        self.kcache = torch.zeros(cfg.layers, max_len, H, hd, dtype=BF16, device=device)
        self.vcache = torch.zeros(cfg.layers, max_len, H, hd, dtype=BF16, device=device)
        self.rope = ops.rope_table(max_len, hd, cfg.theta, device)
        self.precision = "default"
# ... 141 lines not shown
        assert max(int(x.shape[0]) for x in xs) <= self.max_len
        segs, r0 = [], 0
        for b, x in enumerate(xs):
            segs.append((r0, r0 + x.shape[0], 0, (kc[:, b], vc[:, b]) + ((lo[0][:, b], lo[1][:, b]) if lo is not None else ())))
            r0 += x.shape[0]
        return self._prefill(torch.cat(xs, 0) if len(xs) > 1 else xs[0], segs)

    def prefix_supported(self):
        return self.precision != "parity" and not self.fp8

    def forward_shared_prefix(self, xs, P, kc, vc):
        B = len(xs)
        T = [int(x.shape[0]) for x in xs]
        if not self.prefix_supported():
            raise ops.IvlmError(f"forward_shared_prefix: not in precision {self.precision!r} / fp8")
        if B < 2 or not 16 < P < min(T) or sum(T) - B * P <= 16 or max(T) > self.max_len:
            raise ops.IvlmError(f"forward_shared_prefix: B={B}, P={P}, lengths {T}: need B >= 2, 16 < P < min length, > 16 suffix rows")
        pre = self._prefill(xs[0][:P], [(0, P, 0, (kc[:, 0], vc[:, 0]))])[0]
        for c in (kc, vc):
            c[:, 1:, :P].copy_(c[:, :1, :P])
        segs, r0 = [], 0
        for b in range(B):
            segs.append((r0, r0 + T[b] - P, P, (kc[:, b], vc[:, b])))
            r0 += T[b] - P
        suf = self._prefill(torch.cat([x[P:] for x in xs], 0), segs)
        return [torch.cat([pre, h], 0) for h in suf]

    def _prefill(self, x, segs):
        fp8 = self.fp8 and not self._calibrating and len(segs) == 1 and x.shape[0] > 16
        for li in range(len(self.layers)):
            x = self._prefill_layer(li, x, segs, fp8)
        x = ops.rmsnorm(x, self.norm, self.cfg.eps, out_f32=True)
        return [x[r0: r1] for r0, r1, _, _ in segs]

    _PREFILL_FLAGS = {"default": ({}, {}, {}),
                      "f16": (dict(out_f16=True), dict(out_f16=True), {}),
                      "parity": (dict(out_split=True), dict(a_split=True, out_split=True), dict(a_split=True))}

    def _prefill_layer(self, li, x, segs, fp8=False):
        c, L = self.cfg, self.layers[li]
        if fp8:
            sc = L["s"]
            qkv = ops.linear_fp8(ops.rmsnorm(x, L["ln1"], c.eps, fp8_scale=sc["y1"]), L["qkv_q"], sc["y1"], L["qkv_s"])
            a8 = ops.gather_rows(self._prefill_attn(qkv, li, segs), out_kind="fp8", scale=sc["a"])
            x = ops.linear_fp8(a8, L["o_q"], sc["a"], L["o_s"], residual=x, out_kind="f32")
            h8 = ops.linear_fp8(ops.rmsnorm(x, L["ln2"], c.eps, fp8_scale=sc["y2"]), L["gu_q"], sc["y2"], L["gu_s"], act="swiglu",
                                out_kind="fp8", scale_out=sc["h"])
            return ops.linear_fp8(h8, L["down_q"], sc["h"], L["down_s"], residual=x, out_kind="f32")
        norm, lin_in, lin_out = self._PREFILL_FLAGS[self.precision]
        W = self._f16w(L) if self.precision == "f16" else L
        y = ops.rmsnorm(x, L["ln1"], c.eps, **norm)
        a = self._prefill_attn(ops.linear(y, W["qkv"], **lin_in), li, segs)
        x = ops.linear(a, W["o"], residual=x, out_f32=True, **lin_out)
        y2 = ops.rmsnorm(x, L["ln2"], c.eps, **norm)
        h = ops.linear(y2, W["gu"], act="swiglu", **lin_in)
        if self._calibrating and self.precision == "default":
            for k, t in (("y1", y), ("a", a), ("y2", y2), ("h", h)):
                ops.amax(t, L["amax"][k])
        return ops.linear(h, W["down"], residual=x, out_f32=True, **lin_out)

    def _prefill_attn(self, qkv, li, segs):
        c = self.cfg
        H, hd = c.heads, c.hidden // c.heads
        a = torch.empty(qkv.shape[0], qkv.shape[1] // 3, dtype=qkv.dtype, device=qkv.device)
        for r0, r1, pos0, cache in segs:
            T, qs, out = r1 - r0, qkv[r0: r1], a[r0: r1]
            if self.precision == "parity":
                kc, vc, kcl, vcl = (t[li] for t in cache)
                ops.rope_kv_split(qs, H, hd, pos0, (kc, kcl, vc, vcl), self.rope)
                qh, ql = (qs.view(T, 2, 3, H, hd)[:, i, 0].permute(1, 0, 2).unsqueeze(0) for i in range(2))
                kv = [t[: pos0 + T].permute(1, 0, 2).unsqueeze(0) for t in (kc, kcl, vc, vcl)]
                ops.attention_split(qh, ql, *kv, hd ** -0.5, causal=True, q_pos0=pos0, out=out.view(1, T, 2, H, hd))
            else:
                kc, vc = cache[0][li], cache[1][li]
                ops.rope_kv(qs, H, hd, pos0, c.theta, kc, vc, table=self.rope)
                q = qs.view(T, 3, H, hd)[:, 0].permute(1, 0, 2).unsqueeze(0)
                k, v = (t[: pos0 + T].permute(1, 0, 2).unsqueeze(0) for t in (kc, vc))
                ops.attention(q, k, v, hd ** -0.5, causal=True, q_pos0=pos0, out=out.view(1, T, H, hd).permute(0, 2, 1, 3))
        return a

    def _graph_key(self, B, batched):
        if batched:
            return _GraphKey(True, B, self.precision, self.decode_packed and self.decode_packed_batch and B > 1, self.fp8, False)
        c = self.cfg
        fused = bool(self.fuse_attn_oproj and c.hidden in (512, 1024, 4096, 5120)
                     and c.heads + c.hidden // 32 <= torch.cuda.get_device_properties(self.device).multi_processor_count)
        return _GraphKey(False, 1, self.precision, bool(self.decode_packed), self.fp8, fused)

    def _drop_graphs(self, pred):
        self._graphs = {k: st for k, st in self._graphs.items() if not pred(k)}

    def fused_wait_expired(self, st):
        fz = st.get("fused")
        if fz is None or int(fz["status"].item()) == 0:
            return False
        self.fuse_attn_oproj = False
        self._drop_graphs(lambda k: k.fused)
        return True

    def _capture_decode(self, key, st, body, caches, counters, rows=1):
        saved = [t[..., :rows, :, :].clone() for t in caches]
        st["graph"], _ = graphs.capture(body, self.device)
        for t in counters:
            t.zero_()
        for t, sv in zip(caches, saved):
            t[..., :rows, :, :].copy_(sv)
        self._graphs[key] = st

    def decode_graph(self, pos=None):
        key = self._graph_key(1, batched=False)
        st = self._graphs.get(key)
        if st is None:
            dev, c = self.device, self.cfg
            st = dict(tok=torch.zeros(1, dtype=torch.int32, device=dev), pos=torch.zeros(1, dtype=torch.int32, device=dev),
                      pos64=torch.zeros(1, dtype=torch.int64, device=dev))
            if key.fused:
                st["fused"] = dict(step=torch.zeros(1, dtype=torch.int32, device=dev),
                                   counters=torch.zeros(c.layers, 32, dtype=torch.int32, device=dev),
                                   status=torch.zeros(1, dtype=torch.int32, device=dev),
                                   scratch=torch.zeros(c.layers, c.hidden, dtype=F32, device=dev))
            fz = self._fused = st.get("fused")

            def body():
                e = self.embed_ids(st["tok"])
                h = self._decode_step(e, st["pos"])
                st["hidden"] = h
                st["nxt"] = ops.argmax(self.logits(h), bump=st["pos"])
                if fz is not None:
                    fz["step"].add_(1)

            caches = [self.kcache, self.vcache] + ([self.kcache_lo, self.vcache_lo] if self.precision == "parity" else [])
            counters = [st["pos"], st["pos64"]] + ([fz["step"], fz["counters"]] if fz is not None else [])
            self._capture_decode(key, st, body, caches, counters)
        if pos is not None:
            st["pos"].fill_(pos)
            st["pos64"].fill_(pos)
            if "fused" in st:
                for k in ("step", "counters", "status"):
                    st["fused"][k].zero_()
        return st

    def batch_cache(self, B):
        bc = getattr(self, "_bcache", None)
        if bc is None or bc[0].shape[1] < B:
            c = self.cfg
            H, hd = c.heads, c.hidden // c.heads
            bc = self._bcache = tuple(torch.zeros(c.layers, B, self.max_len, H, hd, dtype=BF16, device=self.device)
                                      for _ in range(2))
            self._drop_graphs(lambda k: k.batched)
        if self.precision == "f16":
            return bc[0].view(torch.float16)[:, :B], bc[1].view(torch.float16)[:, :B]
        return bc[0][:, :B], bc[1][:, :B]

    def decode_step_batch(self, x, pos_dev, kc, vc, lo=None, prefix=None):
        c = self.cfg
        H, hd = c.heads, c.hidden // c.heads
        if x.shape[0] > 16:
            raise ops.IvlmError("decode_step_batch: at most 16 sequences per step (weight-streaming kernels)")
        lin = self._lin("frag" if self.decode_packed and self.decode_packed_batch and x.shape[0] > 1 else None)
        if prefix is not None:
            if lo is not None or not self.prefix_supported():
                raise ops.IvlmError(f"decode_step_batch(prefix=...): not in precision {self.precision!r} / fp8")
            if getattr(self, "_prefix_scratch", None) is None:
                self._prefix_scratch = ops.decode_attn_prefix_scratch(16, H, hd, self.norm.device)
            return self._decode_layers(x, lin, self._attn_then_o(lin, lambda qkv, li: (
                ops.llama_decode_attn_batch_prefix(qkv, kc[li], vc[li], H, hd, pos_dev, prefix, c.theta, hd ** -0.5, table=self.rope,
                                                   scratch=self._prefix_scratch))))
        return self._decode_layers(x, lin, self._attn_then_o(lin, lambda qkv, li: (
            ops.llama_decode_attn_batch(qkv, kc[li], vc[li], H, hd, pos_dev, c.theta, hd ** -0.5, table=self.rope,
                                        lo=(lo[0][li], lo[1][li]) if lo is not None else None))))

    @staticmethod
    def _planes(L, n):
        if n + "_p" not in L:
            L[n + "_p"] = ops.PackedBf12(L[n]) if ops.PackedBf12.takes(*L[n].shape) else None
        return L[n + "_p"]

    def _decode_layers(self, x, lin, attn_o):
        c = self.cfg
        for li, L in enumerate(self.layers):
            qkv = lin(x, L, "qkv", rms=(L["ln1"], c.eps))
            x = attn_o(qkv, li, L, x)
            h = lin(x, L, "gu", act="swiglu", rms=(L["ln2"], c.eps))
            x = lin(h, L, "down", residual=x)
        return ops.rmsnorm(x, self.norm, c.eps, out_f32=True)

    @staticmethod
    def _attn_then_o(lin, attn):
        return lambda qkv, li, L, x: lin(attn(qkv, li), L, "o", residual=x)

    def _lin(self, planes=None):
        def lin(x, L, n, **kw):
            wp = self._planes(L, n) if planes else None
            if wp is not None and (planes == "any" or wp.frag):
                return ops.linear_bf12(x, wp, **kw)
            return ops.linear(x, L[n], out_f32=True, **kw)
        return lin

    VERIFY_BUCKETS = (4, 8, 16)

    def verify_supported(self):
        return self.precision != "parity" and not self.fp8

    def verify_step(self, x, pos_dev):
        c = self.cfg
        H, hd = c.heads, c.hidden // c.heads
        if not 1 <= x.shape[0] <= 16:
            raise ops.IvlmError("verify_step: 1 .. 16 rows per pass (weight-streaming kernels)")
        if not self.verify_supported():
            raise ops.IvlmError(f"verify_step: not in precision {self.precision!r} / fp8 (no multi-token attention on hi + lo planes)")
        kc, vc = self._caches()
        lin = self._lin("frag" if self.decode_packed and self.decode_packed_batch else None)
        return self._decode_layers(x, lin, self._attn_then_o(lin, lambda qkv, li: (
            ops.llama_verify_attn(qkv, kc[li], vc[li], H, hd, pos_dev, c.theta, hd ** -0.5, table=self.rope))))

    def verify_pass(self, st):
        h = self.verify_step(self.embed_ids(st["ids"]), st["pos"])
        st["hidden"] = h
        st["amax"] = ops.argmax(self.logits(h))
        ops.spec_accept(st["amax"], st["ids"], st["nd"], st["n_acc"], st["tok"], st["pos"])
        return st

    def verify_state(self, kb):
        i32 = lambda n: torch.zeros(n, dtype=torch.int32, device=self.device)
        return dict(ids=i32(kb), nd=i32(1), pos=i32(1), n_acc=i32(1), tok=i32(1))

    def verify_graph(self, kb):
        key = _GraphKey(False, kb, self.precision, bool(self.decode_packed and self.decode_packed_batch), self.fp8, False, True)
        st = self._graphs.get(key)
        if st is None:
            st = self.verify_state(kb)
            caches = [self.kcache, self.vcache]
            self._capture_decode(key, st, lambda: self.verify_pass(st), caches, [st["pos"], st["n_acc"], st["tok"]], rows=kb)
        return st

    def decode_graph_batch(self, B, pos=None, prefix=None):
        kc, vc = self.batch_cache(B)
        lo = self.batch_cache_lo(B) if self.precision == "parity" else None
        key = self._graph_key(B, batched=True)
        if prefix is not None:
            key = key._replace(prefix=True)
        st = self._graphs.get(key)
        if st is None:
            dev = self.device
            st = dict(tok=torch.zeros(B, dtype=torch.int32, device=dev), pos=torch.zeros(B, dtype=torch.int32, device=dev))
            if prefix is not None:
                st["prefix"] = torch.zeros(1, dtype=torch.int32, device=dev)

            def body():
                h = self.decode_step_batch(self.embed_ids(st["tok"]), st["pos"], kc, vc, lo, st.get("prefix"))
                st["hidden"] = h
                st["nxt"] = ops.argmax(self.logits(h), bump=st["pos"])

            self._capture_decode(key, st, body, [kc, vc] + list(lo or ()), [st["pos"]])
        if pos is not None:
            st["pos"].copy_(pos)
        if prefix is not None:
            st["prefix"].fill_(int(prefix))
        return st

    def _attn_scratch(self):
        if not (self.decode_splitkv or os.environ.get("IVLM_DECODE_SPLITKV", "0") == "1") or self.precision == "parity":
            return None
        if getattr(self, "_dec_scratch", None) is None:
            self._dec_scratch = ops.decode_attn_scratch(self.cfg.heads, self.cfg.hidden // self.cfg.heads, self.norm.device)
        return self._dec_scratch

    def _decode_step(self, x, pos):
        c = self.cfg
        H, hd = c.heads, c.hidden // c.heads
        fz = self._fused if isinstance(pos, torch.Tensor) else None
        if self.fp8:
            lin = lambda x_, L, n, **kw: ops.linear_fp8w(x_, L[n + "_q"], L[n + "_s"], **kw)
            return self._decode_layers(x, lin, self._attn_then_o(lin, lambda qkv, li: ops.llama_decode_attn(
                qkv, self.kcache[li], self.vcache[li], H, hd, pos, c.theta, hd ** -0.5, table=self.rope)))
        kc, vc = self._caches()
        packed = self.decode_packed and fz is None
        lin = self._lin("any" if packed else None)
        attn_o = plain = self._attn_then_o(lin, lambda qkv, li: ops.llama_decode_attn(
            qkv, kc[li], vc[li], H, hd, pos, c.theta, hd ** -0.5, table=self.rope, lo=self._lo(li), scratch=self._attn_scratch()))
        if packed:
            split = self.decode_attn_parts and self._lo(0) is None
            if split and getattr(self, "_parts", None) is None:
                self._parts = torch.zeros(H * 4 * (hd + 4), dtype=F32, device=self.norm.device)

            def attn_o(qkv, li, L, x):
                wo = self._planes(L, "o")
                if not split or wo is None:
                    return plain(qkv, li, L, x)
                ops.llama_decode_attn_parts(qkv, kc[li], vc[li], H, hd, pos, c.theta, hd ** -0.5, self._parts, table=self.rope)
                return ops.linear_bf12(None, wo, residual=x, parts=(self._parts, hd))
        elif fz is not None and self.precision == "default":
            attn_o = lambda qkv, li, L, x: ops.llama_attn_oproj(
                qkv, self.kcache[li], self.vcache[li], L["o"], x, H, hd, pos, fz["step"], fz["counters"][li], fz["status"], c.theta,
                hd ** -0.5, self.rope, fz["scratch"][li])
        return self._decode_layers(x, lin, attn_o)

    def logits(self, hidden_rows):
        if hidden_rows.shape[0] > 16:
            return ops.linear(ops.split_rows(hidden_rows.contiguous()), self.lm_head, out_f32=True, a_split=True)
        if hidden_rows.shape[0] == 1 and self.decode_packed and ops.PackedBf12.takes(16, self.cfg.hidden):
            if getattr(self, "lm_head_p", None) is None:
                self.lm_head_p = ops.PackedBf12(self.lm_head, pad_rows=True)
            return ops.linear_bf12(hidden_rows.contiguous(), self.lm_head_p)
        return ops.linear(hidden_rows, self.lm_head, out_f32=True)
```

interactvlm_amd/model.py:

```python
from __future__ import annotations

import os
from types import SimpleNamespace
from typing import List, Optional

import torch

from . import decoding, graphs, ops
from . import exact_sets as _es
from .components import HumanContact3DPredictor, ObjectMeshContact3DPredictor, ObjectPCAfford3DPredictor
from .constants import IGNORE_LABEL, IMAGE_TOKEN_INDEX
from .heads import SamFusionHead, UncertaintyHead
from .llava import ClipTower, Llama
from .sam import SamImageEncoder, SamMaskDecoder, _Lin, _dev, postprocess_masks
from .weights import IvlmCfg

BF16 = torch.bfloat16
F32 = torch.float32


class _CamPoseEncoder:

    def __init__(self, w, kind, V, device, prefix="cam_pose_encoder"):
        self.kind, self.V = kind, V

        def lin(name, pad_k=None):
            W, b = w[name + ".weight"], w[name + ".bias"]
            if pad_k:
                W = torch.nn.functional.pad(W, (0, pad_k - W.shape[1]))
            return _dev(W, device), _dev(b, device)

        if kind == "simple":
            self.l1 = lin(prefix + ".linear1", 8)
        else:
            self.s0 = lin(prefix + ".spatial_encoder.0", 8)
            self.s2 = lin(prefix + ".spatial_encoder.2")
            self.views = [lin(f"{prefix}.view_transforms.{v}") for v in range(V)]

    def __call__(self, cam_params):
        c = torch.nn.functional.pad(cam_params.to(F32), (0, 3)).contiguous()
        if self.kind == "simple":
            return ops.linear(c, self.l1[0], self.l1[1], act="relu", out_f32=True)
        h = ops.linear(c, self.s0[0], self.s0[1], act="relu", out_f32=True)
        vi = self.kind == "view_index"
        base = ops.linear(h, self.s2[0], self.s2[1], act="sigmoid" if vi else "relu", out_f32=True)
        enc = torch.empty(self.V, self.views[0][0].shape[0], dtype=F32, device=base.device)
        for v in range(self.V):
            ops.linear(base[v: v + 1], *self.views[v], act="none" if vi else "sigmoid", out=enc[v: v + 1])
        return enc


class InteractVLMForCausalLM:
    def __init__(self, config: IvlmCfg, weights: dict, device="cuda:0", lift_tables=None, metadata_root="./data",
                 max_len=1024, precision=None, nonfinite_fallback=None):
        c = self.config = config
        if nonfinite_fallback is not None:
            if nonfinite_fallback not in ("bf16", "parity"):
                raise ValueError(f"nonfinite_fallback must be 'bf16' or 'parity', got {nonfinite_fallback!r}")
            self.nonfinite_fallback = nonfinite_fallback
        self.device = dev = torch.device(device)
        w = weights
        self.hC_sam_view_type, self.oC_sam_view_type = c.hC_sam_view_type, c.oC_sam_view_type
        self.hC_loss_weight, self.oC_loss_weight = c.hC_loss_weight, c.oC_loss_weight
        self.seg_token_idx, self.hseg_token_idx, self.oseg_token_idx = c.seg_token_idx, c.hseg_token_idx, c.oseg_token_idx
        self.token_type, self.img_emb_len = c.token_type, c.img_emb_len
        self.multiview_channels, self.multiview_cam_cond = c.multiview_channels, c.multiview_cam_cond
        self.cam_encoder_type = c.cam_encoder_type
        self.base_token_type = c.token_type.replace("-DifDe", "")
        self.use_fusion, self.use_uncertainty = bool(c.use_fusion), bool(c.use_uncertainty)
        self.debug_taps = None
        self.overlap_sam_encoder = True
        self.graph_decode = graphs.ON
        self.sam_after_prefill = bool(os.environ.get("IVLM_SAM_AFTER_PREFILL"))
        self.fused_lowres_lift = False
        self._side_stream = torch.cuda.Stream(device=dev) if dev.type == "cuda" else None
        self._hi_stream = torch.cuda.Stream(device=dev, priority=-1) if dev.type == "cuda" else None
        self.prioritise_llm = False

        self.vision_tower = ClipTower(w, c.clip, dev)
        self.mm_projector = _Lin(w, "model.mm_projector", dev)
        self.llm = Llama(w, c.llama, dev, max_len=max_len)
        self.text_hidden_fcs = (_Lin(w, "model.text_hidden_fcs.0.0", dev), _Lin(w, "model.text_hidden_fcs.0.2", dev))
        vm = SimpleNamespace()
        vm.image_encoder = SamImageEncoder(w, c.sam, dev)
        vm.mask_decoder = SamMaskDecoder(w, dev, grid=c.sam.grid)
        vm.prompt_encoder = vm.mask_decoder
        self.use_diff_decoder = "DifDe" in c.token_type
        if self.use_diff_decoder:
            assert c.difde_load in ("separate", "reference"), c.difde_load
            if c.difde_load == "reference":
                vm.mask_decoder = SamMaskDecoder(w, dev, grid=c.sam.grid, decoder="object_mask_decoder")
                vm.prompt_encoder = vm.mask_decoder
            names = ("object_mask_decoder",) * 2 if c.difde_load == "reference" else ("human_mask_decoder", "object_mask_decoder")
            vm.human_mask_decoder = SamMaskDecoder(w, dev, grid=c.sam.grid, decoder=names[0])
            vm.object_mask_decoder = SamMaskDecoder(w, dev, grid=c.sam.grid, decoder=names[1])
        if self.use_fusion:
            vm.fusion = SamFusionHead(w, dev)
        if self.use_uncertainty:
            vm.uncertainty = UncertaintyHead(w, dev, grid=c.sam.grid)
        vm.postprocess_masks = lambda m, input_size, original_size: postprocess_masks(
            m, input_size, original_size, c.sam.img_size)
        self.model = SimpleNamespace(visual_model=vm, text_hidden_fcs=self.text_hidden_fcs,
                                     mm_projector=self.mm_projector, vision_tower=self.vision_tower)
        self.lm_head = self.llm.lm_head
        self.human_3d_contact_predictor = self.object_3d_afford_predictor = self.object_3d_contact_predictor = None
        if c.hC_loss_weight > 0:
            self.human_3d_contact_predictor = HumanContact3DPredictor(
                c.hC_sam_view_type, c.multiview_channels, metadata_root=metadata_root, tables=lift_tables)
        if c.oC_loss_weight > 0:
            self.object_3d_afford_predictor = ObjectPCAfford3DPredictor(c.oC_sam_view_type, c.multiview_channels)
            self.object_3d_contact_predictor = ObjectMeshContact3DPredictor(c.oC_sam_view_type, c.multiview_channels)
        self.cam_pose_encoder = (_CamPoseEncoder(w, c.cam_encoder_type, c.multiview_channels, dev)
                                 if c.multiview_cam_cond else None)
        self.attention_splitter = None
        if self.base_token_type in ("Gen-Hu-Obj", "Gen-Int"):
            self.attention_splitter = {n: _Lin(w, "attention_splitter." + n, dev) for n in
                                       ("input_proj", "query_human", "query_object", "key", "value", "output_proj")}
        self.set_precision(precision or os.environ.get("IVLM_PRECISION", "default"))

    def eval(self):
        return self

    precision_modes = ("default", "bf16", "parity-fast", "parity")
    precision = "default"
    _TOWER_MODES = {"default": ("f16", "f16", "f16q"), "f16": ("f16", "f16", "f16"), "bf16": ("default", "default", "default"),
                    "parity-fast": ("parity", "parity", "parity-fast"), "parity": ("parity", "parity", "parity")}

    def set_precision(self, mode):
        assert mode in self._TOWER_MODES, mode
        self.precision = mode
        clip, llm, enc = self._TOWER_MODES[mode]
        self.vision_tower.precision = clip
        self.llm.set_precision(llm)
        self.model.visual_model.image_encoder.precision = enc
        if self.device.type == "cuda" and not self.fp8:
            self.llm.prepare()
            if self.free_unused_weights:
                self.llm.release_unused()

    free_unused_weights = os.environ.get("IVLM_KEEP_ALL_WEIGHTS", "0") != "1"

    def resident_weight_bytes(self):
        return self.llm.resident_bytes()

    def enable_fp8(self, images_clip, images, input_ids):
        self._precision_before_fp8 = self.precision
        self.set_precision("bf16")
        dev = self.device
        self.model.visual_model.image_encoder.enable_fp8(images[0].to(dev))
        self.vision_tower.enable_fp8(images_clip.to(dev))
        feats = self.encode_images(images_clip)[0]
        self.llm.enable_fp8(self._input_embeds(input_ids[0].to(dev), feats))
        self.fp8 = True

    def disable_fp8(self):
        self.model.visual_model.image_encoder.fp8 = False
        self.vision_tower.fp8 = False
        self.llm.disable_fp8()
        self.fp8 = False
        self.set_precision(getattr(self, "_precision_before_fp8", "default"))

    fp8 = False
    nonfinite_guard = os.environ.get("IVLM_NONFINITE_GUARD", "1") != "0"
    nonfinite_fallback = "bf16"
    recomputations = None

    def _guard_applies(self):
        return (self.nonfinite_guard and not self.fp8 and self.precision in ("default", "f16", "parity-fast")
                and not getattr(self, "_in_guard", False))

    def _guarded(self, fn, args, kwargs, supplied_embeddings=None):
        self._in_guard = True
        self._finite_flags = []
        try:
            out = fn(*args, **kwargs)
            if not self._guard_ok(out, supplied_embeddings):
                out = self._recompute_fallback(lambda: fn(*args, **kwargs))
            return out
        finally:
            self._in_guard = False

    def _guard_ok(self, out, supplied_embeddings=None):
        flags = self._guard_flags(out)
        if not flags or bool(torch.stack(flags).all()):
            return True
        self._check_supplied(supplied_embeddings)
        return False

    def _guard_flags(self, out):
        outs = out if isinstance(out, list) else [out]
        return self._finite_flags + [torch.isfinite(o[k]).all() for o in outs
                                     for k in ("pred_contact_3d", "pred_human_3d_contact", "pred_object_3d_contact",
                                               "pred_object_3d_afford") if o.get(k) is not None]

    def _check_supplied(self, supplied_embeddings):
        if supplied_embeddings is not None:
            embs = supplied_embeddings if isinstance(supplied_embeddings, (list, tuple)) else [supplied_embeddings]
            if not all(bool(torch.isfinite(e).all()) for e in embs):
                raise ops.IvlmError("image_embeddings passed by the caller are not finite (an fp16-mode encoder pass that "
                                    "overflowed?): re-encode them, e.g. model.precompute_visual_embs(views) - which checks")

    def _recompute_bf16(self, fn):
        import warnings

        warnings.warn(f"non-finite contacts in precision mode {self.precision!r} (an activation left fp16's exponent "
                      "range): this call is recomputed with bf16 operands; consider model.set_precision('bf16')")
        out = self._recompute_in("bf16", fn)
        for o in (out if isinstance(out, list) else [out]):
            o["recomputed_in_bf16"] = True
        return out

    def _recompute_fallback(self, fn):
        if self.nonfinite_fallback != "parity":
            return self._recompute_bf16(fn)
        import warnings

        warnings.warn(f"non-finite contacts in precision mode {self.precision!r} (an activation left fp16's exponent "
                      "range): this call is recomputed in the parity mode (nonfinite_fallback='parity')")
        out = self._recompute_in("parity", fn)
        for o in (out if isinstance(out, list) else [out]):
            o["recomputed_in_parity"] = True
        return out

    def _recompute_in(self, target, fn, unpacked_decode=True):
        mode, packed, free = self.precision, self.llm.decode_packed, self.free_unused_weights
# ... 159 lines not shown
    def encode_images(self, images_clip):
        f = self.vision_tower(images_clip.to(self.device))
        B, T, C = f.shape
        return self.mm_projector(f.reshape(B * T, C), out_f32=True,
                                 a_split=self.vision_tower.precision in ("parity", "f16")).view(B, T, -1)

    def _seg_token_ids(self):
        ids = [self.seg_token_idx]
        if self.base_token_type in ("Gen-Hu-Obj", "Gen-Int"):
            ids += [self.hseg_token_idx, self.oseg_token_idx]
        return [i for i in ids if i is not None]

    def _seg_rows(self, ids, extra_false_col):
        ids = ids.cpu()
        m = torch.zeros_like(ids, dtype=torch.bool)
        for s in self._seg_token_ids():
            m |= ids == s
        m = m[1:]
        if extra_false_col:
            m = torch.cat([m, torch.zeros(1, dtype=torch.bool)])
        return torch.cat([torch.zeros(self.img_emb_len, dtype=torch.bool), m])

    def _mask_decoder_for(self, ds_name):
        vm = self.model.visual_model
        if self.use_diff_decoder and ds_name is not None:
            if "hcontact" in ds_name:
                return vm.human_mask_decoder
            if "oafford" in ds_name or "ocontact" in ds_name:
                return vm.object_mask_decoder
        return vm.mask_decoder

    def _decode_sample(self, hidden, rows_mask, ids, cam_params, image_embeddings, input_size, original_size, ds_name=None,
                       sigmoid_gt=None, llava_features=None):
        if getattr(self, "_in_guard", False):
            self._finite_flags.append(torch.isfinite(hidden).all() & torch.isfinite(image_embeddings).all())
        rows = rows_mask.cpu().nonzero().flatten()
        ids = ids.cpu()
        V = self.multiview_channels
        if rows.numel() == 0:
            return torch.zeros((0,) + tuple(original_size), dtype=torch.float32, device=self.device), None
        if self.use_fusion:
            image_embeddings = self.model.visual_model.fusion(image_embeddings, llava_features)
        sel = hidden[rows.to(hidden.device)].contiguous()
        if sel.shape[0] > 16:
            raise ops.IvlmError("more than 16 [SEG] rows in one sample")
        emb = self.text_hidden_fcs[1](self.text_hidden_fcs[0](sel, act="relu", out_f32=True), out_f32=True)
        if self.debug_taps is not None:
            self.debug_taps.update(hidden=hidden, seg_emb=emb, sam_emb=image_embeddings)
        k = int(rows[0]) - self.img_emb_len + 1
        token = int(ids[k]) if k > 0 else None
        emb = emb.unsqueeze(1)
        if V > 1:
            emb = emb.repeat(1, V, 1)
        emb = self.process_embeddings(emb, cam_params, token)
        low, iou = self._mask_decoder_for(ds_name)(image_embeddings, emb)
        if self.debug_taps is not None:
            self.debug_taps.update(prompt_emb=emb, low_res=low, iou=iou)
        self._last_low = (low, tuple(input_size), tuple(original_size))
        if sigmoid_gt is not None:
            gt = sigmoid_gt.to(self.device, F32).reshape(low.shape[0], 1, *tuple(original_size)).contiguous()
            return postprocess_masks(low, input_size, original_size, self.config.sam.img_size, sigmoid_gt=gt,
                                     ignore_label=float(IGNORE_LABEL))[:, 0], iou
        return postprocess_masks(low, input_size, original_size, self.config.sam.img_size)[:, 0], iou

    @torch.no_grad()
    def model_forward(self, images, images_clip, input_ids, labels=None, attention_masks=None, offset=None,
                      masks_list=None, label_list=None, gt_contact_3d_list=None, cam_params=None, resize_list=None,
                      ds_name_list=None, mask_paths_list=None, inference=False, **kwargs):
        if not inference:
            raise NotImplementedError("training (loss) path is out of scope of the inference hot path")
        if self._guard_applies():
            return self._guarded(self.model_forward, (images, images_clip, input_ids, labels, attention_masks, offset, masks_list,
                                                      label_list, gt_contact_3d_list, cam_params, resize_list, ds_name_list,
                                                      mask_paths_list, inference), kwargs)
        B = images.shape[0]
        assert offset is None or B == len(offset) - 1
        assert images_clip.shape[0] == 1 or images_clip.shape[0] == B
        feats = self.encode_images(images_clip)
        if self.debug_taps is not None:
            self.debug_taps["clip_feat"] = feats
        emb_sam = self.model.visual_model.image_encoder(
            images.to(self.device).reshape((B * images.shape[1],) + tuple(images.shape[2:])))
        V = images.shape[1]
        emb_sam = emb_sam.view(B, V, emb_sam.shape[1], emb_sam.shape[2])
        pred_masks, gt_masks, uncertainty_maps = [], [], []
        for i in range(B):
            ids = input_ids[i].to(self.device)
            x = self._input_embeds(ids, feats[i if feats.shape[0] > 1 else 0])
            hidden = self.llm.forward(x, 0)
            rows = self._seg_rows(ids, extra_false_col=True)
            osz = tuple(label_list[i].shape[-2:]) if label_list is not None else tuple(resize_list[i])
            ds_name = ds_name_list[i] if ds_name_list else "hcontact"
            gt = masks_list[i][:, 0] if masks_list is not None else None
            hm = gt is not None and "oafford" in ds_name and "HM" in (self.oC_sam_view_type or "")
            pm, _ = self._decode_sample(hidden, rows, ids, cam_params[i], emb_sam[i], resize_list[i], osz, ds_name=ds_name,
                                        sigmoid_gt=gt if hm else None, llava_features=hidden if self.use_fusion else None)
            pred_masks.append(pm)
            gt_masks.append(gt)
            if self.use_uncertainty:
                uncertainty_maps.append(self.model.visual_model.uncertainty.resized(emb_sam[i], osz).squeeze(0))
        ds_name_list = ds_name_list or ["hcontact"] * B
        result = {"gt_masks": gt_masks, "pred_masks": pred_masks}
        if self.use_uncertainty:
            result["uncertainty_maps"] = uncertainty_maps
        if self.hC_loss_weight > 0:
            result["pred_human_3d_contact"] = self.human_3d_contact_predictor(pred_masks, ds_name_list)
        if self.oC_loss_weight > 0:
            result["pred_object_3d_contact"] = self.object_3d_contact_predictor(pred_masks, ds_name_list, mask_paths_list)
            result["pred_object_3d_afford"] = self.object_3d_afford_predictor(pred_masks, ds_name_list, mask_paths_list)
        return result

    @torch.no_grad()
    def generate(self, images_clip, input_ids, max_new_tokens=32, eos_token_id=2, forced_new_tokens=None,
                 after_prefill=None, draft=None):
        feats = self.encode_images(images_clip)[0]
        ids = input_ids[0]
        x = self._input_embeds(ids, feats)
        T0 = x.shape[0]
        n_max = len(forced_new_tokens) if forced_new_tokens is not None else max_new_tokens
        n_max = min(n_max, self.llm.max_len - T0)
        if n_max <= 0:
            raise ops.IvlmError(f"prompt of {T0} positions does not fit the KV cache (max_len={self.llm.max_len})")
        hidden_all = torch.empty(T0 + n_max, self.config.llama.hidden, dtype=F32, device=self.device)
        h = self.llm.forward(x, 0)
        hidden_all[:T0].copy_(h)
        if after_prefill is not None:
            after_prefill()
        last = h[T0 - 1: T0]
        if draft is not None and forced_new_tokens is None and self.llm.verify_supported():
            out = self._generate_speculative(ids, last, T0, n_max, eos_token_id, hidden_all, draft)
        else:
            out = self._generate_greedy(ids, last, T0, n_max, eos_token_id, hidden_all, forced_new_tokens)
        if out is None:
            return self.generate(images_clip, input_ids, max_new_tokens, eos_token_id, forced_new_tokens, None, draft)
        return out

    def _generate_greedy(self, ids, last, T0, n_max, eos_token_id, hidden_all, forced_new_tokens=None):
        forced = None
        if forced_new_tokens is not None:
            host = [int(t) for t in list(forced_new_tokens)[:n_max]]
            forced = ([host], torch.tensor(host, dtype=torch.int32, device=self.device)[:, None])
        step = self._single_step(hidden_all, T0)
        self.last_spec = None
        (new_ids,), self.last_argmax = decoding.greedy(step, ops.argmax(self.llm.logits(last)), [n_max], eos_token_id, forced)
        return self._generated(ids, step, T0, new_ids)

    def _generate_speculative(self, ids, last, T0, n_max, eos_token_id, hidden_all, draft):
        step = self._single_step(hidden_all, T0)
        new_ids, self.last_argmax, self.last_spec = decoding.speculative(step, ops.argmax(self.llm.logits(last)), n_max,
                                                                         eos_token_id, draft)
        return self._generated(ids, step, T0, new_ids)

    def _single_step(self, hidden_all, T0):
        return (decoding.SingleGraph if graphs.enabled(self.graph_decode) else decoding.SingleEager)(self.llm, hidden_all, T0)

    def _generated(self, ids, step, T0, new_ids):
        if step.st is not None and self.llm.fused_wait_expired(step.st):
            return None
        out_ids = torch.cat([ids.cpu(), torch.tensor(new_ids, dtype=ids.dtype)])[None]
        return out_ids, step.hidden[: T0 + len(new_ids) - 1]

    @torch.no_grad()
    def generate_batch(self, images_clip, input_ids_list, max_new_tokens=32, eos_token_id=2, forced_new_tokens=None,
                       share_prefix=False):
        B = len(input_ids_list)
        if B > 16:
            raise ops.IvlmError(f"generate_batch: {B} sequences per call, at most 16 (evaluate_batch chunks larger batches itself)")
        dev = self.device
        feats = self.encode_images(images_clip)
        kc, vc = self.llm.batch_cache(B)
        lo = self.llm.batch_cache_lo(B) if self.llm.precision == "parity" else None
        shared = feats.shape[0] == 1 and B > 1
        xs = [self._input_embeds(input_ids_list[b].reshape(-1), feats[0 if shared else b]) for b in range(B)]
        T0 = [int(x.shape[0]) for x in xs]
        if forced_new_tokens is not None:
            if not isinstance(forced_new_tokens[0], (list, tuple)):
                forced_new_tokens = [list(forced_new_tokens)] * B
            n_seq = [len(f) for f in forced_new_tokens]
        else:
            n_seq = [max_new_tokens] * B
        n_seq = [min(n, self.llm.max_len - t) for n, t in zip(n_seq, T0)]
        if min(n_seq) <= 0:
            raise ops.IvlmError(f"a prompt of {max(T0)} positions does not fit the KV cache (max_len={self.llm.max_len})")
        n_max = max(n_seq)
        hidden_all = torch.empty(B, max(T0) + n_max, self.config.llama.hidden, dtype=F32, device=dev)
        last = torch.empty(B, self.config.llama.hidden, dtype=F32, device=dev)
        P = 0
        if share_prefix:
            P = decoding.shared_prefix_len([t.reshape(-1).tolist() for t in input_ids_list], images_clip.shape[0] == 1,
                                           self.precision, self.fp8, image_rows=feats.shape[1])
        prefix = P if P > 0 else None
        assert P < min(T0)
        hs = self.llm.forward_shared_prefix(xs, P, kc, vc) if prefix else self.llm.forward_packed(xs, kc, vc, lo)
        for b, h in enumerate(hs):
            hidden_all[b, : T0[b]].copy_(h)
            last[b].copy_(h[T0[b] - 1])
        forced = None
        if forced_new_tokens is not None:
            pad = [list(map(int, f[:n])) + [eos_token_id] * (n_max - n) for f, n in zip(forced_new_tokens, n_seq)]
            forced = (pad, torch.tensor(pad, dtype=torch.int32, device=dev).t().contiguous())
        pos = torch.tensor(T0, dtype=torch.int32, device=dev)
        if graphs.enabled(self.graph_decode):
            step = decoding.BatchGraph(self.llm, hidden_all, pos, prefix)
        else:
            step = decoding.BatchEager(self.llm, hidden_all, pos, (kc, vc, lo), prefix)
        new_ids, _ = decoding.greedy(step, ops.argmax(self.llm.logits(last)), n_seq, eos_token_id, forced)
        out = []
        for b in range(B):
            ids = input_ids_list[b].reshape(-1).cpu()
            out_ids = torch.cat([ids, torch.tensor(new_ids[b], dtype=ids.dtype)])[None]
            out.append((out_ids, hidden_all[b, : T0[b] + len(new_ids[b]) - 1]))
        return out

    def evaluate_batch(self, images_clip, images, input_ids_list, cam_params, resize_list, original_size_list,
                       contact_type="hcontact", max_new_tokens=32, forced_new_tokens=None, eos_token_id=2,
                       lift2d_dict_path=None, image_embeddings=None, deferred=False, share_prefix=False, exact_sets=None):
        args = (images_clip, images, input_ids_list, cam_params, resize_list, original_size_list, contact_type, max_new_tokens,
                forced_new_tokens, eos_token_id, lift2d_dict_path, image_embeddings)
        B = len(input_ids_list)
        if B > 16:
            if images_clip.shape[0] == 1:
                raise ops.IvlmError("evaluate_batch: more than 16 prompts about ONE picture are not supported")
            subs = []
            for lo in range(0, B, 16):
                hi = min(lo + 16, B)
                fn = forced_new_tokens
                if fn is not None and isinstance(fn[0], (list, tuple)):
                    fn = fn[lo:hi]
                emb = image_embeddings[lo:hi] if isinstance(image_embeddings, (list, tuple)) else image_embeddings
                subs.append((images_clip[lo:hi], None if images is None else images[lo:hi], input_ids_list[lo:hi], cam_params[lo:hi],
                             resize_list[lo:hi], original_size_list[lo:hi],
                             contact_type if isinstance(contact_type, str) else contact_type[lo:hi], max_new_tokens, fn, eos_token_id,
                             lift2d_dict_path[lo:hi] if isinstance(lift2d_dict_path, (list, tuple)) else lift2d_dict_path, emb))

            def finish_all():
                outs, pending = [], None
                for sub in subs:
                    nxt_ = self.evaluate_batch(*sub, deferred=True, share_prefix=share_prefix, exact_sets=exact_sets)
                    if pending is not None:
                        outs.extend(pending())
                    pending = nxt_
                outs.extend(pending())
                return outs
            return finish_all if deferred else finish_all()
        guard = self._guard_applies()
        es = _es.config(exact_sets)
        st = self._evaluate_batch_begin(*args, share_prefix=share_prefix)

        def finish():
            if es is not None:
                return self._exact_sets_pass(
                    es, lambda: self._evaluate_batch_finish(st),
                    lambda idx: self.evaluate_batch(*_es.subset_batch_args(args, idx), share_prefix=share_prefix),
                    supplied_embeddings=image_embeddings)
            if not guard:
                return self._evaluate_batch_finish(st)
            self._in_guard = True
            self._finite_flags = []
            try:
                outs = self._evaluate_batch_finish(st)
                if not self._guard_ok(outs, image_embeddings):
                    outs = self._recompute_fallback(lambda: self.evaluate_batch(*args, share_prefix=share_prefix))
                return outs
            finally:
                self._in_guard = False
        return finish if deferred else finish()

    def _evaluate_batch_begin(self, images_clip, images, input_ids_list, cam_params, resize_list, original_size_list,
                              contact_type, max_new_tokens, forced_new_tokens, eos_token_id, lift2d_dict_path, image_embeddings,
                              share_prefix=False):
        B = len(input_ids_list)
        main = torch.cuda.current_stream(self.device)
        ev = allv = None
        if image_embeddings is not None:
            embs = list(image_embeddings) if isinstance(image_embeddings, (list, tuple)) else [image_embeddings] * B
            gens = self.generate_batch(images_clip, input_ids_list, max_new_tokens, eos_token_id, forced_new_tokens, share_prefix)
        else:
            side = self._side_stream if self.overlap_sam_encoder else main
            embs = []
            if side is not main:
                side.wait_stream(main)
            with torch.cuda.stream(side):
                V_ = images.shape[1]
                allv = self.model.visual_model.image_encoder(
                    images.to(self.device).reshape((B * V_,) + tuple(images.shape[2:])))
                embs = [allv[b * V_: (b + 1) * V_] for b in range(B)]
                if side is not main:
                    ev = torch.cuda.Event()
                    ev.record(side)
            gens = self.generate_batch(images_clip, input_ids_list, max_new_tokens, eos_token_id, forced_new_tokens, share_prefix)
        return dict(B=B, gens=gens, embs=embs, ev=ev, allv=allv, cam_params=cam_params, resize_list=resize_list,
                    original_size_list=original_size_list, contact_type=contact_type, lift2d_dict_path=lift2d_dict_path)

    def _evaluate_batch_finish(self, st):
        B, gens, embs = st["B"], st["gens"], st["embs"]
        cam_params, resize_list, original_size_list = st["cam_params"], st["resize_list"], st["original_size_list"]
        contact_type, lift2d_dict_path = st["contact_type"], st["lift2d_dict_path"]
        main = torch.cuda.current_stream(self.device)
        if st["ev"] is not None:
            main.wait_event(st["ev"])
            st["allv"].record_stream(main)
        outs, lows = [], []
        ctypes = [contact_type] * B if isinstance(contact_type, str) else list(contact_type)
        for b, (output_ids, hidden) in enumerate(gens):
            rows = self._seg_rows(output_ids[0], extra_false_col=False)
            pm, _ = self._decode_sample(hidden, rows, output_ids[0], cam_params[b], embs[b], resize_list[b],
                                        original_size_list[b], ds_name=ctypes[b], llava_features=self._eval_llava_features(hidden, 0))
            outs.append({"output_ids": output_ids, "pred_masks": [pm], "pred_contact_3d": None})
            if self.use_uncertainty:
                outs[-1]["uncertainty_maps"] = [self._eval_uncertainty(embs[b], original_size_list[b])]
            lows.append(pm)
        paths = lift2d_dict_path if isinstance(lift2d_dict_path, (list, tuple)) else [lift2d_dict_path] * B
        have = [b for b in range(B) if lows[b].shape[0] > 0]
        hum = [b for b in have if self.hC_loss_weight > 0 and "hcontact" in ctypes[b]]
        if hum:
            pc = self.human_3d_contact_predictor([lows[b] for b in hum])
            for i, b in enumerate(hum):
                outs[b]["pred_contact_3d"] = pc[i: i + 1]
        for b in have:
            if b in hum:
                continue
            if (self.oC_loss_weight > 0 and "ocontact" in ctypes[b]) or "oafford" in ctypes[b]:
                outs[b]["pred_contact_3d"] = self.object_3d_contact_predictor(
                    [lows[b]], ds_names=["ocontact"], lift2d_dict_path=paths[b])
                self._log_lift(b)
        return outs

    def evaluate(self, images_clip, images, input_ids, cam_params, resize_list, original_size_list,
                 lift2d_dict_path=None, contact_type="hcontact", max_new_tokens=32, tokenizer=None,
                 forced_new_tokens=None, eos_token_id=2, image_embeddings=None, draft=None, exact_sets=None):
        assert input_ids.shape[0] == 1, "the reference only ever calls evaluate with batch 1 (evaluate.py:479)"
        es = _es.config(exact_sets)
        if es is not None:
            one = lambda: [self.evaluate(images_clip, images, input_ids, cam_params, resize_list, original_size_list,
                                         lift2d_dict_path, contact_type, max_new_tokens, tokenizer, forced_new_tokens,
                                         eos_token_id, image_embeddings, draft)]
            return self._exact_sets_pass(es, one, lambda idx: one(), supplied_embeddings=image_embeddings)[0]
        if self._guard_applies():
            return self._guarded(self.evaluate, (images_clip, images, input_ids, cam_params, resize_list, original_size_list,
                                                 lift2d_dict_path, contact_type, max_new_tokens, tokenizer, forced_new_tokens,
                                                 eos_token_id, image_embeddings), {"draft": draft},
                                 supplied_embeddings=image_embeddings)
        side = None
        box = {"emb": image_embeddings, "ev": None}
        main = torch.cuda.current_stream(self.device)

        def launch_sam():
            side.wait_stream(main)
            with torch.cuda.stream(side):
                box["emb"] = self.model.visual_model.image_encoder(images[0].to(self.device))
                box["ev"] = torch.cuda.Event()
                box["ev"].record(side)

        after_prefill = None
        if image_embeddings is None and self.overlap_sam_encoder:
# ... 60 lines not shown
```

interactvlm_amd/ops.py:

```python
from __future__ import annotations

import os

import torch

from . import _lib
from ._lib import IvlmError, check

IVLM_F32, IVLM_BF16 = 0, 1


def _stream() -> int:
    return torch.cuda.current_stream().cuda_stream


class KernelTimer:

    def __init__(self):
        self.enabled = False
        self.records = {}
        self._hip = None

    def _rt(self):
        if self._hip is None:
# ... 498 lines not shown
        call()
    return out


class PackedBf12:

    @staticmethod
    def takes(N, K):
        return N % 16 == 0 and K % 64 == 0 and K * 6 <= 100 * 1024

    def __init__(self, w, fragments=True, pad_rows=False, packer="c"):
        assert w.dtype == BF16 and w.dim() == 2 and w.is_cuda and w.shape[1] % 16 == 0
        self.rows = w.shape[0]
        n_rows = -(-w.shape[0] // 16) * 16
        if fragments and packer == "c" and (pad_rows or n_rows == w.shape[0]) and self.takes(n_rows, w.shape[1]):
            if not bool(torch.isfinite(w).all()):
                raise IvlmError("PackedBf12: inf / nan weights cannot be packed")
            lib, w, K = _lib.load(), w.contiguous(), w.shape[1]
            self.ebase = torch.empty(n_rows, dtype=torch.int32, device=w.device)
            self.patch_ptr = torch.empty(n_rows + 1, dtype=torch.int32, device=w.device)
            check(lib.ivlm_pack_bf12m_count(w.data_ptr(), self.rows, n_rows, K, self.ebase.data_ptr(), self.patch_ptr.data_ptr(),
                                            _stream()), "pack_bf12m_count")
            self.n_patches = int(self.patch_ptr[-1])
            self.patch_col = torch.zeros(max(1, self.n_patches), dtype=torch.int32, device=w.device)
            self.patch_val = torch.zeros(max(1, self.n_patches), dtype=BF16, device=w.device)
            self.P = torch.empty(n_rows // 16, K // 64, 4, 16, 2, 8, dtype=torch.uint8, device=w.device)
            self.E = torch.empty(n_rows // 16, K // 64, 4, 16, 2, 4, dtype=torch.uint8, device=w.device)
            check(lib.ivlm_pack_bf12m_fill(w.data_ptr(), self.rows, n_rows, K, self.ebase.data_ptr(), self.patch_ptr.data_ptr(),
                                           self.P.data_ptr(), self.E.data_ptr(), self.patch_col.data_ptr(), self.patch_val.data_ptr(),
                                           _stream()), "pack_bf12m_fill")
            self.shape, self.frag = (n_rows, K), True
            return
        if pad_rows and w.shape[0] % 16:
            w = torch.cat([w, torch.zeros(16 - w.shape[0] % 16, w.shape[1], dtype=BF16, device=w.device)])
        if not bool(torch.isfinite(w).all()):
            raise IvlmError("PackedBf12: inf / nan weights cannot be packed")
        N, K = w.shape
        bits = w.contiguous().view(torch.int16).to(torch.int32) & 0xFFFF
        ef = (bits >> 7) & 0xFF
        eb = (ef.max(dim=1).values - 15).clamp_(min=0)
        code = ef - eb[:, None]
        inwin = code >= 1
        esc = (~inwin) & ((bits & 0x7FFF) != 0)
        self.P = torch.where(inwin, ((bits >> 8) & 0x80) | (bits & 0x7F), torch.zeros_like(bits)).to(torch.uint8).contiguous()
        code = torch.where(inwin, code, torch.zeros_like(code))
        self.E = (code[:, 0::2] | (code[:, 1::2] << 4)).to(torch.uint8).contiguous()
        self.ebase = eb.to(torch.int32).contiguous()
        rows, cols = esc.nonzero(as_tuple=True)
        self.patch_ptr = torch.zeros(N + 1, dtype=torch.int32, device=w.device)
        if rows.numel():
            self.patch_ptr[1:] = torch.bincount(rows, minlength=N).cumsum(0).to(torch.int32)
        self.patch_col = (cols.to(torch.int32) if rows.numel() else torch.zeros(1, dtype=torch.int32, device=w.device)).contiguous()
        self.patch_val = (w[rows, cols] if rows.numel() else torch.zeros(1, dtype=BF16, device=w.device)).contiguous()
        self.shape, self.n_patches = (N, K), int(rows.numel())
        self.frag = fragments and self.takes(N, K)
        if self.frag:
            self.P = self.P.view(N // 16, 16, K // 64, 2, 4, 8).permute(0, 2, 4, 1, 3, 5).contiguous()
            self.E = self.E.view(N // 16, 16, K // 64, 2, 4, 4).permute(0, 2, 4, 1, 3, 5).contiguous()

    def bytes(self):
        return self.P.numel() + self.E.numel() + 4 * self.ebase.numel() + 4 * self.patch_ptr.numel() + 6 * self.n_patches

    def _rows(self):
        if not self.frag:
            return self.P, self.E
        N, K = self.shape
        return (self.P.permute(0, 3, 1, 4, 2, 5).reshape(N, K).contiguous(), self.E.permute(0, 3, 1, 4, 2, 5).reshape(N, K // 2).contiguous())

    def _args(self):
        P, E = self._rows()
        self._keep = (P, E)
        return (P.data_ptr(), P.stride(0), E.data_ptr(), E.stride(0), self.ebase.data_ptr(),
                self.patch_ptr.data_ptr(), self.patch_col.data_ptr(), self.patch_val.data_ptr())

    def _args_frag(self):
        return (self.P.data_ptr(), self.E.data_ptr(), self.ebase.data_ptr(), self.patch_ptr.data_ptr(), self.patch_col.data_ptr(),
                self.patch_val.data_ptr())

    def unpack(self):
        out = torch.empty(self.shape, dtype=BF16, device=self.P.device)
        check(_lib.load().ivlm_unpack_bf12(*self._args(), self.shape[0], self.shape[1], out.data_ptr(), _stream()), "unpack_bf12")
        self._keep = None
        return out[: self.rows]


def linear_bf12(x, wp: PackedBf12, bias=None, act="none", residual=None, out_f32=True, rms=None, parts=None):
    lib = _lib.load()
    N, K = wp.shape
    if parts is not None:
        pt, pD = parts
        assert x is None and wp.frag and rms is None and pt.dtype == F32 and pt.numel() >= (K // pD) * 4 * (pD + 4)
        dev = pt.device
    else:
        assert x.dtype == F32 and x.is_contiguous() and x.dim() == 2 and x.shape[1] == K and 1 <= x.shape[0] <= 16
        dev = x.device
    n_out = N // 2 if act == "swiglu" else N
    M = 1 if parts is not None else x.shape[0]
    out = torch.empty(M, n_out, dtype=F32 if out_f32 else BF16, device=dev)
    if M > 1:
        assert wp.frag and wp.rows == N
        flags = 0
        if residual is not None:
            assert residual.dtype in (BF16, F32) and residual.is_contiguous() and tuple(residual.shape) == (M, N)
            flags = GEMM_RES_F32 if residual.dtype == F32 else 0
        call = lambda: check(lib.ivlm_gemv16_bf12m(x.data_ptr(), K, M, *wp._args_frag(), out.data_ptr(), n_out, _p(bias), _p(residual), N,
                                                   N, K, ACT[act], 1 if out_f32 else 0, _p(rms[0]) if rms else 0,
                                                   float(rms[1]) if rms else 0.0, flags, _stream()), "gemv16_bf12m")
        if TIMER.enabled:
            TIMER.time("gemv_bf16", 2.0 * N * K, call, tag=(M, N, K, act, "bf12"))
        else:
            call()
        return out
    flags = 0
    if residual is not None:
        assert residual.dtype in (BF16, F32) and residual.is_contiguous() and residual.numel() == N
        if residual.dtype == F32:
            flags |= GEMM_RES_F32
    if parts is not None:
        call = lambda: check(lib.ivlm_gemv1_bf12m_parts(pt.data_ptr(), pD, *wp._args_frag(), out.data_ptr(), _p(bias), _p(residual), N, K,
                                                        ACT[act], 1 if out_f32 else 0, flags, _stream()), "gemv1_bf12m_parts")
    elif wp.frag:
        call = lambda: check(lib.ivlm_gemv1_bf12m(x.data_ptr(), *wp._args_frag(), out.data_ptr(), _p(bias), _p(residual), N, K,
                                                  ACT[act], 1 if out_f32 else 0, _p(rms[0]) if rms else 0,
                                                  float(rms[1]) if rms else 0.0, flags, _stream()), "gemv1_bf12m")
    else:
        call = lambda: check(lib.ivlm_gemv1_bf12(x.data_ptr(), *wp._args(), out.data_ptr(), _p(bias), _p(residual), N, K, ACT[act],
                                                 1 if out_f32 else 0, _p(rms[0]) if rms else 0, float(rms[1]) if rms else 0.0,
                                                 flags, _stream()), "gemv1_bf12")
    if TIMER.enabled:
        TIMER.time("gemv_bf16", 2.0 * N * K, call, tag=(1, N, K, act, "bf12"))
    else:
        call()
    return out if wp.rows == N or act == "swiglu" else out[:, : wp.rows]


def rmsnorm(x, weight, eps=1e-5, out_f32=False, out_split=False, fp8_scale=None, out_f16=False):
    lib = _lib.load()
    x = _req(x, None, "x")
    cols = x.shape[-1]
    if fp8_scale is not None:
        y = torch.empty(x.shape, dtype=U8, device=x.device)
        check(lib.ivlm_rmsnorm_fp8(x.data_ptr(), _dtc(x), weight.data_ptr(), y.data_ptr(), x.numel() // cols, cols, float(eps),
                                   fp8_scale.data_ptr(), _stream()), "rmsnorm_fp8")
        return y
    if out_split:
        y = torch.empty(x.shape[:-1] + (2 * cols,), dtype=BF16, device=x.device)
    else:
        y = torch.empty(x.shape, dtype=F16 if out_f16 else (F32 if out_f32 else BF16), device=x.device)
    check(lib.ivlm_rmsnorm(x.data_ptr(), _dtc(x), weight.data_ptr(), y.data_ptr(), 2 if out_split else (4 if out_f16 else _dtc(y)),
                           x.numel() // cols, cols, float(eps), _stream()), "rmsnorm")
    return y


def bf16_to_f16(w):
    w = w.contiguous()
    assert w.dtype == torch.bfloat16
    out = torch.empty(w.shape, dtype=torch.float16, device=w.device)
    check(_lib.load().ivlm_bf16_to_f16(w.data_ptr(), out.data_ptr(), w.numel(), _stream()), "bf16_to_f16")
    return out


def f16_weight(w, name="weight"):
    w16 = bf16_to_f16(w)
    err = float((w16.float() - w.float()).abs().max())
    if not (err <= 2.0 ** -24) or not bool(torch.isfinite(w16).all()):
        raise IvlmError(f"{name}: weights outside the fp16 range (max conversion error {err:.3g}) - use a split (hi + lo) "
                        f"precision mode instead of fp16 operands")
    return w16


def relpos_table64(tab_h, tab_w):
    n = tab_h.shape[0] + tab_w.shape[0]
    assert n <= 64
    t = torch.zeros(64, tab_h.shape[1], dtype=BF16, device=tab_h.device)
    t[: tab_h.shape[0]] = tab_h
    t[tab_h.shape[0]: n] = tab_w
    return t


def _attn_operands(q, k, v, o, rel, rel_tab, prescale_q, grid_table):
    import ctypes

    st = (ctypes.c_int64 * 12)(*(t.stride(i) for t in (q, k, v, o) for i in range(3)))
    rel_h = rel_w = None
    kh = kw = 0
    if rel is not None:
        rel_h, rel_w = rel
        assert rel_h.dtype == torch.float32 and rel_h.is_contiguous() and rel_w.is_contiguous()
        kh, kw = rel_h.shape[-1], rel_w.shape[-1]
    if rel_tab is not None:
        rel_h, kh = rel_tab
        kw = kh
        assert rel is None and rel_h.dtype == q.dtype and rel_h.is_contiguous()
        if grid_table:
            assert rel_h.shape[1] == q.shape[3]
            assert rel_h.shape[0] == 64 if 2 * kh <= 32 else (kh == 64 and rel_h.shape[0] >= 254)
        else:
            assert rel_h.shape == (64, q.shape[3])
    pre = 1 if (prescale_q or rel is not None or rel_tab is not None) else 0
    return st, _p(rel_h), _p(rel_w), kh, kw, pre


def attention(q, k, v, scale, causal=False, q_pos0=0, rel=None, out=None, prescale_q=False, rel_tab=None, q_lo=None, q_lo_level=1):
    import ctypes

    lib = _lib.load()
    B, H, Sq, D = q.shape
    Bk, Sk = k.shape[0], k.shape[2]
    dt = q.dtype
    assert dt in (BF16, F16) and k.dtype == dt and v.dtype == dt
    assert q.stride(3) == 1 and k.stride(3) == 1 and v.stride(3) == 1 and B % Bk == 0
    if out is None:
        out = torch.empty(B, Sq, H, D, dtype=dt, device=q.device).permute(0, 2, 1, 3)
    assert out.stride(3) == 1 and out.dtype == dt
    st, rel_h, rel_w, kh, kw, pre = _attn_operands(q, k, v, out, rel, rel_tab, prescale_q, grid_table=True)
    if q_lo is not None:
        assert dt == F16 and q_lo.dtype == F16 and q_lo.stride() == q.stride() and q_lo.shape == q.shape and not causal and B == Bk
        check(lib.ivlm_attention_f16_qsplit(q.data_ptr(), q_lo.data_ptr(), k.data_ptr(), v.data_ptr(), out.data_ptr(),
                                            ctypes.cast(st, ctypes.c_void_p), B, H, Sq, Sk, D, float(scale), rel_h, rel_w,
                                            kh, kw, int(q_lo_level), _stream()), "attention_f16_qsplit")
        return out
    fn = lib.ivlm_attention_f16 if dt == F16 else lib.ivlm_attention_bf16
    check(fn(q.data_ptr(), k.data_ptr(), v.data_ptr(), out.data_ptr(),
             ctypes.cast(st, ctypes.c_void_p), B, H, Sq, Sk, D, float(scale), 1 if causal else 0,
             int(q_pos0), rel_h, rel_w, kh, kw, B // Bk, pre, _stream()), "attention")
    return out


def attention_split(q, q_lo, k, k_lo, v, v_lo, scale, causal=False, q_pos0=0, rel=None, out=None, prescale_q=False, rel_tab=None):
    import ctypes

    lib = _lib.load()
    B, H, Sq, D = q.shape
    Bk, Sk = k.shape[0], k.shape[2]
    for t, tl in ((q, q_lo), (k, k_lo), (v, v_lo)):
        assert t.dtype == BF16 and tl.dtype == BF16 and t.stride() == tl.stride() and t.shape == tl.shape and t.stride(3) == 1
    assert B % Bk == 0
    if out is None:
        out = torch.empty(B, Sq, 2, H, D, dtype=BF16, device=q.device)
    assert out.shape == (B, Sq, 2, H, D) and out.stride(4) == 1
    oh, ol = out[:, :, 0].permute(0, 2, 1, 3), out[:, :, 1].permute(0, 2, 1, 3)
    st, rel_h, rel_w, kh, kw, pre = _attn_operands(q, k, v, oh, rel, rel_tab, prescale_q, grid_table=False)
    check(lib.ivlm_attention_bf16_split(q.data_ptr(), q_lo.data_ptr(), k.data_ptr(), k_lo.data_ptr(), v.data_ptr(),
                                        v_lo.data_ptr(), oh.data_ptr(), ol.data_ptr(), ctypes.cast(st, ctypes.c_void_p), B, H,
                                        Sq, Sk, D, float(scale), 1 if causal else 0, int(q_pos0), rel_h, rel_w, kh, kw,
                                        B // Bk, pre, _stream()), "attention_split")
    return out.view(B * Sq, 2 * H * D)


def relpos_bias_split(q, q_lo, tab_h, tab_w, SH, SW):
    lib = _lib.load()
    B, H, S, D = q.shape
    if q_lo is None:
        q_lo = q
    assert S == SH * SW and q.stride(3) == 1 and q.stride() == q_lo.stride() and tab_h.is_contiguous() and tab_w.is_contiguous()
    rel_h = torch.empty(B * H, S, SH, dtype=torch.float32, device=q.device)
    rel_w = torch.empty(B * H, S, SW, dtype=torch.float32, device=q.device)
    check(lib.ivlm_relpos_bias_split(q.data_ptr(), q_lo.data_ptr(), q.stride(0), q.stride(1), q.stride(2), tab_h.data_ptr(),
                                     tab_w.data_ptr(), B, H, SH, SW, D, rel_h.data_ptr(), rel_w.data_ptr(), _stream()),
          "relpos_bias_split")
    return rel_h, rel_w


def attention_f32(q, k, v, scale, out=None):
    import ctypes

    lib = _lib.load()
    B, H, Sq, D = q.shape
    Bk, Sk = k.shape[0], k.shape[2]
    assert q.dtype == F32 and k.dtype == F32 and v.dtype == F32 and B % Bk == 0
    assert q.stride(3) == 1 and k.stride(3) == 1 and v.stride(3) == 1
    if out is None:
        out = torch.empty(B, Sq, H, D, dtype=F32, device=q.device).permute(0, 2, 1, 3)
    st = (ctypes.c_int64 * 12)(q.stride(0), q.stride(1), q.stride(2), k.stride(0), k.stride(1), k.stride(2),
                               v.stride(0), v.stride(1), v.stride(2), out.stride(0), out.stride(1), out.stride(2))
    check(lib.ivlm_attention_f32(q.data_ptr(), k.data_ptr(), v.data_ptr(), out.data_ptr(), ctypes.cast(st, ctypes.c_void_p),
                                 B, H, Sq, Sk, D, float(scale), B // Bk, _stream()), "attention_f32")
    return out


def relpos_tables_cat(tab_h, tab_w):
    n = tab_h.shape[0] + tab_w.shape[0]
    cat = torch.zeros((n + 63) // 64 * 64, tab_h.shape[1], dtype=BF16, device=tab_h.device)
    cat[: tab_h.shape[0]] = tab_h
    cat[tab_h.shape[0]: n] = tab_w
    return cat


RELPOS_GEMM = True


def relpos_bias(q, tab_h, tab_w, SH, SW, cat=None, q_lo=None):
    lib = _lib.load()
    B, H, S, D = q.shape
    assert S == SH * SW and q.stride(3) == 1 and tab_h.is_contiguous() and tab_w.is_contiguous()
    rel_h = torch.empty(B * H, S, SH, dtype=torch.float32, device=q.device)
    rel_w = torch.empty(B * H, S, SW, dtype=torch.float32, device=q.device)
    if q.dtype == F16:
        if not (cat is not None and cat.dtype == F16 and min(SH, SW) >= 32):
            raise IvlmError("relpos_bias: fp16 q needs the fp16 cat table and a grid of 32 x 32 or more (GEMM formulation)")
        npad, M = cat.shape[0], B * S
        assert q_lo is None or (q_lo.dtype == F16 and q_lo.stride() == q.stride())
        G = torch.empty(H, M, npad, dtype=F32, device=q.device)
        call = lambda: check(lib.ivlm_relpos_bias_f16(q.data_ptr(), _p(q_lo), q.stride(0), q.stride(1), q.stride(2), cat.data_ptr(), npad,
                                                      B, H, SH, SW, D, G.data_ptr(), G.numel() * 4, rel_h.data_ptr(), rel_w.data_ptr(),
                                                      _stream()), "relpos_bias_f16")
        if TIMER.enabled:
            TIMER.time("gemm_bf16_mfma", 2.0 * H * M * npad * D, call, tag=("relpos", M, npad, D))
        else:
            call()
        return rel_h, rel_w
    if (RELPOS_GEMM and cat is not None and min(SH, SW) >= 32 and q.dtype == cat.dtype and q.stride(0) == S * q.stride(2) and q.stride(2) % 8 == 0
            and q.stride(1) % 8 == 0 and D % 8 == 0 and q.data_ptr() % 16 == 0):
        npad, M = cat.shape[0], B * S
        G = torch.empty(H, M, npad, dtype=BF16, device=q.device)
        call = lambda: check(lib.ivlm_gemm_bf16(q.data_ptr(), q.stride(2), cat.data_ptr(), D, G.data_ptr(), npad, 0, 0, 0, 0,
                                                M, npad, D, 0, 0, H, q.stride(1), 0, M * npad, 0, 0, 0.0, 0, 0, 0, _stream()),
                             "relpos gemm")
        if TIMER.enabled:
            TIMER.time("gemm_bf16_mfma", 2.0 * H * M * npad * D, call, tag=("relpos", M, npad, D))
        else:
            call()
        check(lib.ivlm_relpos_gather(G.data_ptr(), M * npad, npad, B, H, SH, SW, rel_h.data_ptr(), rel_w.data_ptr(), _stream()),
              "relpos_gather")
        return rel_h, rel_w
    check(lib.ivlm_relpos_bias(q.data_ptr(), q.stride(0), q.stride(1), q.stride(2), tab_h.data_ptr(), tab_w.data_ptr(),
                               B, H, SH, SW, D, rel_h.data_ptr(), rel_w.data_ptr(), _stream()), "relpos_bias")
    return rel_h, rel_w


def argmax(logits, bump=None):
    lib = _lib.load()
    logits = _req(logits, torch.float32, "logits")
    rows, cols = logits.shape
    out = torch.empty(rows, dtype=torch.int32, device=logits.device)
    if bump is not None:
        assert bump.dtype == torch.int32 and bump.is_cuda and bump.numel() == rows and bump.is_contiguous()
        check(lib.ivlm_argmax_f32_bump(logits.data_ptr(), rows, cols, out.data_ptr(), bump.data_ptr(), _stream()), "argmax_bump")
        return out
    check(lib.ivlm_argmax_f32(logits.data_ptr(), rows, cols, out.data_ptr(), _stream()), "argmax")
    return out


def im2col_nchw(x, ks, stride, kpad=None):
    lib = _lib.load()
    x = _req(x, BF16, "x")
    B, C, H, W = x.shape
    K = C * ks * ks
    kpad = kpad or ((K + 63) // 64) * 64
    gh, gw = (H - ks) // stride + 1, (W - ks) // stride + 1
    out = torch.empty(B * gh * gw, kpad, dtype=BF16, device=x.device)
    check(lib.ivlm_im2col_nchw(x.data_ptr(), out.data_ptr(), B, C, H, W, ks, stride, kpad, _stream()), "im2col_nchw")
    return out


def im2col3x3_nhwc(x):
    lib = _lib.load()
    x = _req(x, BF16, "x")
    B, H, W, C = x.shape
    out = torch.empty(B * H * W, 9 * C, dtype=BF16, device=x.device)
    check(lib.ivlm_im2col3x3_nhwc(x.data_ptr(), out.data_ptr(), B, H, W, C, _stream()), "im2col3x3")
    return out


def im2col3x3_nhwc_split(x_split, B, H, W, C):
    lib = _lib.load()
    x_split = _req(x_split, BF16, "x_split")
    assert x_split.shape == (B * H * W, 2 * C)
    out = torch.empty(B * H * W, 18 * C, dtype=BF16, device=x_split.device)
    for half in range(2):
        check(lib.ivlm_im2col3x3_nhwc_strided(x_split.data_ptr() + half * C * 2, 2 * C, out.data_ptr() + half * 9 * C * 2,
                                              18 * C, B, H, W, C, _stream()), "im2col3x3_strided")
    return out


_KIND = {"bf16": IVLM_BF16, "f32": IVLM_F32, "split": 2, "fp8": 3}


def gather_rows(src, idx=None, add=None, out=None, out_kind=None, scale=None):
    lib = _lib.load()
    assert src.dtype in (BF16, F32) and src.stride(-1) == 1
    cols = src.shape[-1]
    if idx is not None:
        assert idx.dtype == torch.int32 and idx.is_contiguous()
        rows = idx.numel()
    else:
        src = src.reshape(-1, cols)
        rows = src.shape[0]
    if out_kind is None:
        ref = out if out is not None else (add if add is not None else src)
        out_kind = "f32" if ref.dtype == F32 else "bf16"
    if out is None:
        out = (torch.empty(rows, 2 * cols, dtype=BF16, device=src.device) if out_kind == "split"
               else torch.empty(rows, cols, dtype={"f32": F32, "fp8": torch.uint8}.get(out_kind, BF16), device=src.device))
    assert out.stride(-1) == 1 and out.dtype == {"f32": F32, "fp8": torch.uint8}.get(out_kind, BF16)
    assert (out_kind == "fp8") == (scale is not None)
    lda = 0
    if add is not None:
        assert add.dtype in (BF16, F32) and add.stride(-1) == 1
        lda = add.stride(0)
    check(lib.ivlm_gather_rows(out.data_ptr(), _KIND[out_kind], out.stride(0), src.data_ptr(), _dtc(src), src.stride(0),
                               _p(idx), _p(add), _dtc(add) if add is not None else 0, lda, rows, cols, _p(scale), _stream()),
          "gather_rows")
    return out


def fill_rows(dst, idx, row):
    lib = _lib.load()
    assert dst.dtype in (BF16, F16) and row.dtype == dst.dtype and dst.stride(-1) == 1 and row.is_contiguous()
    assert idx.dtype == torch.int32 and idx.is_contiguous() and row.numel() == dst.shape[-1]
    check(lib.ivlm_fill_rows(dst.data_ptr(), dst.stride(0), idx.data_ptr(), idx.numel(), row.data_ptr(), dst.shape[-1],
                             _stream()), "fill_rows")
    return dst


def split_rows(x):
    C = x.shape[-1]
    return gather_rows(x.reshape(-1, C), out_kind="split").view(x.shape[:-1] + (2 * C,))


def add_rows(a, b, out=None, op="add", out_kind=None):
    lib = _lib.load()
    a = _req(a, None, "a")
    b = _req(b, None, "b")
    cols = a.shape[-1]
    if out_kind is None:
        out_kind = "f32" if (out if out is not None else a).dtype == F32 else "bf16"
    if out is None:
        out = (torch.empty(a.shape[:-1] + (2 * cols,), dtype=BF16, device=a.device) if out_kind == "split"
               else torch.empty(a.shape, dtype=F32 if out_kind == "f32" else BF16, device=a.device))
    check(lib.ivlm_add_rows(out.data_ptr(), _KIND[out_kind], a.data_ptr(), _dtc(a), b.data_ptr(), _dtc(b),
                            a.numel() // cols, cols, b.numel() // cols, 1 if op == "mul" else 0, _stream()), "add_rows")
    return out


def uncertainty_mlp(emb, w1, b1, w2, b2, w3, b3):
    emb = _req(emb, F32, "emb")
    assert emb.shape[-1] == 256 and tuple(w1.shape) == (64, 256) and tuple(w2.shape) == (16, 64) and w3.numel() == 16
    ws = [_req(t, BF16, "w") for t in (w1, b1, w2, b2, w3, b3)]
    out = torch.empty(emb.shape[:-1], dtype=F32, device=emb.device)
    check(_lib.load().ivlm_uncertainty_mlp(emb.data_ptr(), out.numel(), *[t.data_ptr() for t in ws], out.data_ptr(), _stream()),
          "uncertainty_mlp")
    return out


def resize_bilinear(src, size, dtype=torch.float32):
    src = _req(src, F32, "src")
    h, w = src.shape[-2:]
    oh, ow = int(size[0]), int(size[1])
    out = torch.empty(src.shape[:-2] + (oh, ow), dtype=dtype, device=src.device)
    n = src.numel() // (h * w)
    check(_lib.load().ivlm_resize_bilinear(src.data_ptr(), n, h, w, out.data_ptr(), _dtc(out), oh, ow, _stream()), "resize_bilinear")
    return out


def dense_pe(gauss, h, w, dtype=torch.float32):
    lib = _lib.load()
    gauss = _req(gauss, torch.float32, "gauss")
    nf = gauss.shape[1]
    pe = torch.empty(h * w, 2 * nf, dtype=dtype, device=gauss.device)
    check(lib.ivlm_dense_pe(gauss.data_ptr(), pe.data_ptr(), _dtc(pe), h, w, nf, _stream()), "dense_pe")
    return pe


def _rope_extents(qkv, width, H, D, pos0, table, caches):
    T, end = qkv.shape[0], int(pos0) + qkv.shape[0]
    assert qkv.dim() == 2 and T > 0 and int(pos0) >= 0 and qkv.shape[-1] >= width, f"qkv {tuple(qkv.shape)}: needs {width} columns"
    if table is not None:
        for t in table:
            assert t.is_cuda and t.dtype == F32 and t.is_contiguous(), "rope table: contiguous fp32 on the device"
            assert t.dim() == 2 and t.shape[1] == D // 2 and t.shape[0] >= end, f"rope table {tuple(t.shape)}: needs [>= {end}, {D // 2}]"
    for c in caches:
        if c is not None:
            assert c.is_contiguous() and c.shape[0] >= end and c.numel() >= end * H * D, f"cache {tuple(c.shape)}: needs {end} rows of {H * D}"


def rope_kv(qkv, H, D, pos0, theta, kcache=None, vcache=None, table=None):
    lib = _lib.load()
    assert qkv.dtype in (BF16, F16) and qkv.stride(-1) == 1 and (kcache is None or (kcache.dtype == qkv.dtype == vcache.dtype))
    _rope_extents(qkv, 3 * H * D, H, D, pos0, table, (kcache, vcache))
    T = qkv.shape[0]
    check((lib.ivlm_rope_kv_f16 if qkv.dtype == F16 else lib.ivlm_rope_kv)(qkv.data_ptr(), qkv.stride(0), T, H, D, int(pos0), float(theta), _p(kcache), _p(vcache),
                                                                           _p(table[0]) if table else 0, _p(table[1]) if table else 0, _stream()), "rope_kv")
    return qkv


def rope_kv_split(qkv, H, D, pos0, caches, table):
    lib = _lib.load()
# ... 340 lines not shown
```

Before: 10.64.

## Capture a self-feeding decode loop graph with on-device token ring and hidden slab

Adds a loop-form decode graph. An embed_feed kernel reads the next token id from a device ring (or a forced-token table), the argmax kernel writes its result back into the ring and advances a slot counter, and the final RMSNorm also writes hidden states into a per-position slab. Each replay therefore needs no host-side input copies or per-step hidden copies, and the hidden rows are copied out in bulk at the end. This removes per-step host launches and copies in decode, at the cost of extra state buffers, a full max_len x hidden fp32 slab, and more complex resume and finish logic. It is on by default through IVLM_DECODE_LOOP.

```diff
diff --git a/include/ivlm_hip.h b/include/ivlm_hip.h
--- a/include/ivlm_hip.h
+++ b/include/ivlm_hip.h
@@ -346,6 +346,13 @@
 int ivlm_argmax_f32(const float *x, int rows, int cols, int32_t *out, ivlm_stream_t stream);
 int ivlm_argmax_f32_bump(const float *x, int rows, int cols, int32_t *out, int32_t *bump, ivlm_stream_t stream);
 
+int ivlm_embed_feed(float *x, const void *embed, int64_t lde, int vocab, int cols, const int32_t *forced, const int32_t *ring,
+                    const int32_t *use_forced, const int32_t *slot, int n_slots, int B, ivlm_stream_t stream);
+int ivlm_rmsnorm_slab(const float *x, const void *w, float *y, float *slab, const int32_t *pos, int slab_len, int64_t rows, int cols,
+                      float eps, ivlm_stream_t stream);
+int ivlm_argmax_f32_file(const float *x, int rows, int cols, int32_t *out, int32_t *bump, int32_t *ids, int32_t *slot, int n_ring,
+                         ivlm_stream_t stream);
+
 int ivlm_im2col_nchw(const void *x, void *out, int B, int C, int H, int W, int ks, int stride, int Kpad,
                      ivlm_stream_t stream);
 int ivlm_im2col3x3_nhwc(const void *x, void *out, int B, int H, int W, int C, ivlm_stream_t stream);
diff --git a/interactvlm_amd/csrc/elementwise.hip b/interactvlm_amd/csrc/elementwise.hip
--- a/interactvlm_amd/csrc/elementwise.hip
+++ b/interactvlm_amd/csrc/elementwise.hip
@@ -121,6 +121,24 @@
             for (int j = 0; j < 8; ++j) v[j] += a[j];
         }
         store8(dst, dst_kind, r * ldd + c8 * 8, cols, v, inv_scale);
+    }
+}
+
+__global__ __launch_bounds__(kT) void embed_feed_kernel(float* __restrict__ x, const bf16_t* __restrict__ embed, int64_t lde, int vocab,
+                                                        int cols, const int32_t* __restrict__ forced, const int32_t* __restrict__ ring,
+                                                        const int32_t* __restrict__ use_forced, const int32_t* __restrict__ slot,
+                                                        int n_slots, int B) {
+    const int c8n = cols >> 3;
+    const int total = B * c8n;
+    const int32_t* feed = *use_forced ? forced : ring;
+    for (int i = blockIdx.x * kT + threadIdx.x; i < total; i += gridDim.x * kT) {
+        const int c8 = i % c8n, b = i / c8n;
+        const int s = slot[b];
+        if (s < 0 || s >= n_slots) continue;
+        const int id = min(max(feed[(int64_t)s * B + b], 0), vocab - 1);
+        float v[8];
+        load8(embed, 0, (int64_t)id * lde + c8 * 8, v);
+        store8(x, 1, (int64_t)b * cols + c8 * 8, cols, v);
     }
 }
 
@@ -386,6 +404,14 @@
                                                                     add_kind, lda, rows, cols, scale);
     return ivlm_launch_status();
 }
+int embed_feed(float* x, const bf16_t* embed, int64_t lde, int vocab, int cols, const int32_t* forced, const int32_t* ring,
+               const int32_t* use_forced, const int32_t* slot, int n_slots, int B, hipStream_t st) {
+    if (!x || !embed || !forced || !ring || !use_forced || !slot) return IVLM_ERR_INVALID_ARG;
+    if (vocab <= 0 || cols <= 0 || (cols & 7) || (lde & 7) || lde < cols || n_slots <= 0 || B <= 0) return IVLM_ERR_INVALID_ARG;
+    embed_feed_kernel<<<grid_for((int64_t)B * (cols >> 3)), kT, 0, st>>>(x, embed, lde, vocab, cols, forced, ring, use_forced, slot,
+                                                                        n_slots, B);
+    return ivlm_launch_status();
+}
 int amax(const void* x, int kind, int64_t n, float* out, hipStream_t st) {
     if (!x || !out || n <= 0 || (n & 7) || (kind & ~1)) return IVLM_ERR_INVALID_ARG;
     amax_kernel<<<grid_for(n >> 3, 2048), kT, 0, st>>>(x, kind, n >> 3, out);
@@ -465,6 +491,11 @@
     return ivlm::gather_rows(dst, k, ldd, src, src_dtype == IVLM_F32, lds_, idx, add, add_dtype == IVLM_F32, lda, rows, cols,
                              ivlm_stream(s), fp8_scale);
 }
+int ivlm_embed_feed(float* x, const void* embed, int64_t lde, int vocab, int cols, const int32_t* forced, const int32_t* ring,
+                    const int32_t* use_forced, const int32_t* slot, int n_slots, int B, ivlm_stream_t s) {
+    ivlm_enter();
+    return ivlm::embed_feed(x, CBF(embed), lde, vocab, cols, forced, ring, use_forced, slot, n_slots, B, ivlm_stream(s));
+}
 int ivlm_amax(const void* x, int dtype, int64_t n, float* out, ivlm_stream_t s) {
     ivlm_enter();
     return ivlm::amax(x, dtype == IVLM_F32, n, out, ivlm_stream(s));
diff --git a/interactvlm_amd/csrc/gemv.hip b/interactvlm_amd/csrc/gemv.hip
--- a/interactvlm_amd/csrc/gemv.hip
+++ b/interactvlm_amd/csrc/gemv.hip
@@ -333,7 +333,8 @@
 }
 
 __global__ __launch_bounds__(1024) void argmax_kernel(const float* __restrict__ x, int cols, int32_t* __restrict__ out,
-                                                      int32_t* __restrict__ bump) {
+                                                      int32_t* __restrict__ bump, int32_t* __restrict__ ids,
+                                                      int32_t* __restrict__ slot, int n_ring) {
     __shared__ float sv[16];
     __shared__ int si[16];
     const float* r = x + (int64_t)blockIdx.x * cols;
@@ -381,6 +382,11 @@
             }
         out[blockIdx.x] = bi;
         if (bump) bump[blockIdx.x] += 1;
+        if (ids) {
+            const int s = slot[blockIdx.x];
+            if (s >= -1 && s < n_ring - 1) ids[(int64_t)(s + 1) * gridDim.x + blockIdx.x] = bi;
+            slot[blockIdx.x] = s + 1;
+        }
     }
 }
 
@@ -462,9 +468,11 @@
     return ivlm_launch_status();
 }
 
-int argmax_f32(const float* x, int rows, int cols, int32_t* out, hipStream_t st, int32_t* bump) {
+int argmax_f32(const float* x, int rows, int cols, int32_t* out, hipStream_t st, int32_t* bump, int32_t* ids, int32_t* slot,
+               int n_ring) {
     if (!x || !out || rows <= 0 || cols <= 0) return IVLM_ERR_INVALID_ARG;
-    argmax_kernel<<<rows, 1024, 0, st>>>(x, cols, out, bump);
+    if (ids && (!slot || n_ring <= 0)) return IVLM_ERR_INVALID_ARG;
+    argmax_kernel<<<rows, 1024, 0, st>>>(x, cols, out, bump, ids, slot, n_ring);
     return ivlm_launch_status();
 }
 
@@ -500,3 +508,10 @@
     ivlm_enter();
     return ivlm::argmax_f32(x, rows, cols, out, ivlm_stream(stream), bump);
 }
+
+extern "C" int ivlm_argmax_f32_file(const float* x, int rows, int cols, int32_t* out, int32_t* bump, int32_t* ids, int32_t* slot,
+                                    int n_ring, ivlm_stream_t stream) {
+    ivlm_enter();
+    if (!ids) return IVLM_ERR_INVALID_ARG;
+    return ivlm::argmax_f32(x, rows, cols, out, ivlm_stream(stream), bump, ids, slot, n_ring);
+}
diff --git a/interactvlm_amd/csrc/kernels.h b/interactvlm_amd/csrc/kernels.h
--- a/interactvlm_amd/csrc/kernels.h
+++ b/interactvlm_amd/csrc/kernels.h
@@ -205,6 +205,7 @@
 int gemv_bf16(const GemmArgs& g, hipStream_t st);
 int gemv1_fp8w(const GemmArgs& g, hipStream_t st);
 int gemv_mfma_bf16(const GemmArgs& g, hipStream_t st);
-int argmax_f32(const float* x, int rows, int cols, int32_t* out, hipStream_t st, int32_t* bump = nullptr);
+int argmax_f32(const float* x, int rows, int cols, int32_t* out, hipStream_t st, int32_t* bump = nullptr, int32_t* ids = nullptr,
+               int32_t* slot = nullptr, int n_ring = 0);
 
 }
diff --git a/interactvlm_amd/csrc/norm.hip b/interactvlm_amd/csrc/norm.hip
--- a/interactvlm_amd/csrc/norm.hip
+++ b/interactvlm_amd/csrc/norm.hip
@@ -16,11 +16,12 @@
                       pack_bf16x2(f[6], f[7]));
 }
 
-template <bool RMS, int MAXC, bool GELU, bool XF32, bool YF32>
+template <bool RMS, int MAXC, bool GELU, bool XF32, bool YF32, bool SLAB = false>
 __global__ __launch_bounds__(256) void norm_kernel(const void* __restrict__ xv, const bf16_t* __restrict__ w,
                                                    const bf16_t* __restrict__ b, void* __restrict__ yv, int64_t rows,
                                                    int cols, float eps, const int32_t* __restrict__ out_rows,
-                                                   const float* __restrict__ fp8_scale, int y_split) {
+                                                   const float* __restrict__ fp8_scale, int y_split, float* __restrict__ slab = nullptr,
+                                                   const int32_t* __restrict__ slab_pos = nullptr, int slab_len = 0) {
     const int lane = threadIdx.x & 63;
     const int64_t row = (int64_t)blockIdx.x * 4 + (threadIdx.x >> 6);
     if (row >= rows) return;
@@ -69,6 +70,11 @@
     float4* yr4 = reinterpret_cast<float4*>(static_cast<float*>(yv) + orow * cols);
     const uint4* wr = reinterpret_cast<const uint4*>(w);
     const uint4* br = reinterpret_cast<const uint4*>(b);
+    float4* sr4 = nullptr;
+    if (SLAB) {
+        const int p = slab_pos[row];
+        if (p >= 0 && p < slab_len) sr4 = reinterpret_cast<float4*>(slab + (row * slab_len + p) * cols);
+    }
 #pragma unroll
     for (int c = 0; c < MAXC; ++c) {
         const int idx = c * 64 + lane;
@@ -102,6 +108,10 @@
             } else if (YF32) {
                 yr4[2 * idx] = make_float4(o[0], o[1], o[2], o[3]);
                 yr4[2 * idx + 1] = make_float4(o[4], o[5], o[6], o[7]);
+                if (SLAB && sr4) {
+                    sr4[2 * idx] = make_float4(o[0], o[1], o[2], o[3]);
+                    sr4[2 * idx + 1] = make_float4(o[4], o[5], o[6], o[7]);
+                }
             } else if (y_split == 2) {
                 yr[idx] = make_uint4(pack_f16x2(o[0], o[1]), pack_f16x2(o[2], o[3]), pack_f16x2(o[4], o[5]), pack_f16x2(o[6], o[7]));
             } else if (y_split) {
@@ -155,6 +165,20 @@
     return ivlm_launch_status();
 }
 
+int rmsnorm_slab(const float* x, const bf16_t* w, float* y, float* slab, const int32_t* pos, int slab_len, int64_t rows, int cols,
+                 float eps, hipStream_t st) {
+    if (!x || !w || !y || !slab || !pos || rows <= 0 || cols <= 0 || slab_len <= 0) return IVLM_ERR_INVALID_ARG;
+    if ((cols & 7) || cols > kMaxChunks * 512) return IVLM_ERR_UNSUPPORTED;
+    const unsigned grid = (unsigned)((rows + 3) / 4);
+    if (cols <= 4 * 512)
+        norm_kernel<true, 4, false, true, true, true><<<grid, 256, 0, st>>>(x, w, nullptr, y, rows, cols, eps, nullptr, nullptr, 0, slab, pos,
+                                                                             slab_len);
+    else
+        norm_kernel<true, kMaxChunks, false, true, true, true><<<grid, 256, 0, st>>>(x, w, nullptr, y, rows, cols, eps, nullptr, nullptr, 0,
+                                                                                      slab, pos, slab_len);
+    return ivlm_launch_status();
+}
+
 }
 
 extern "C" {
@@ -184,4 +208,10 @@
                          rows, cols, eps, ivlm_stream(stream));
 }
 
-}
+int ivlm_rmsnorm_slab(const float* x, const void* w, float* y, float* slab, const int32_t* pos, int slab_len, int64_t rows, int cols,
+                      float eps, ivlm_stream_t stream) {
+    ivlm_enter();
+    return ivlm::rmsnorm_slab(x, static_cast<const bf16_t*>(w), y, slab, pos, slab_len, rows, cols, eps, ivlm_stream(stream));
+}
+
+}
diff --git a/interactvlm_amd/decoding.py b/interactvlm_amd/decoding.py
--- a/interactvlm_amd/decoding.py
+++ b/interactvlm_amd/decoding.py
@@ -35,6 +35,7 @@
 
 class _Step:
     st = None
+    loop = False
 
     def __init__(self, llm, hidden):
         self.llm, self.hidden = llm, hidden
@@ -105,6 +106,62 @@
         return nxt if out is None else out.copy_(nxt)
 
 
+class _Loop(_Step):
+    loop = True
+
+    def start(self, first, forced=None):
+        st = self.st
+        if forced is not None:
+            st["forced"][: forced[1].shape[0]].copy_(forced[1])
+        else:
+            st["ring"][0].copy_(first)
+        st["use_forced"].fill_(int(forced is not None))
+
+    def __call__(self, s, out=None):
+        assert s == self.n and out is None
+        self.st["graph"].replay()
+        self.n += 1
+        return self.st["ring"][self.n]
+
+
+class SingleLoop(_Loop):
+
+    def __init__(self, llm, hidden, T0):
+        super().__init__(llm, hidden)
+        self.st, self.pos, self.n, self.runs = llm.decode_loop_graph(T0), T0, 0, []
+
+    def __call__(self, s, out=None):
+        if self.runs and self.runs[-1][1] == self.pos:
+            self.runs[-1][1] += 1
+        else:
+            self.runs.append([self.pos, self.pos + 1])
+        self.pos += 1
+        return super().__call__(s, out)
+
+    def resume(self, n, v):
+        self.pos += n
+        self.st["pos"].copy_(v["pos"])
+        self.st["ring"][self.n].copy_(v["tok"])
+
+    def finish(self):
+        for p0, p1 in self.runs:
+            self.hidden[p0:p1].copy_(self.st["slab"][0, p0:p1])
+        self.runs = []
+
+
+class BatchLoop(_Loop):
+
+    def __init__(self, llm, hidden, pos, T0, prefix=None):
+        super().__init__(llm, hidden)
+        self.st, self.T0, self.n = llm.decode_loop_graph_batch(pos.numel(), pos, prefix), [int(t) for t in T0], 0
+
+    def finish(self):
+        for b, t in enumerate(self.T0):
+            t1 = min(t + self.n, self.llm.max_len, self.hidden.shape[1])
+            self.hidden[b, t:t1].copy_(self.st["slab"][b, t:t1])
+        self.T0 = []
+
+
 class BatchEager(_Step):
 
     def __init__(self, llm, hidden, pos, caches, prefix=None):
@@ -135,17 +192,35 @@
                 done[b] = toks[b] == eos or len(new[b]) >= n_seq[b]
         return all(done)
 
+    loop = getattr(step, "loop", False)
+
+    def handed(amax, first=0):
+        if loop:
+            step.finish()
+            if len(amax) > first:
+                amax[first:] = step.st["ring"][first: len(amax)].clone().unbind(0)
+        return new, amax
+
     if forced is not None:
         host, dev = forced
         amax = [nxt]
+        if loop:
+            vocab = step.llm.embed.shape[0]
+            if not all(0 <= t < vocab for f, n in zip(host, n_seq) for t in f[:n]):
+                raise ops.IvlmError(f"forced ids outside the vocabulary of {vocab} ids")
+            step.start(nxt, forced)
         for s in range(n_max):
             if absorb([f[s] for f in host]):
                 break
-            amax.append(step(dev[s]))
-        return new, amax
+            amax.append(step(s if loop else dev[s]))
+        return handed(amax, 1)
     ring = _id_ring(n_max * B)[: n_max * B].view(n_max, B)
-    ids = torch.empty(n_max, B, dtype=torch.int32, device=nxt.device)
-    ids[0].copy_(nxt)
+    if loop:
+        step.start(nxt)
+        ids = step.st["ring"]
+    else:
+        ids = torch.empty(n_max, B, dtype=torch.int32, device=nxt.device)
+        ids[0].copy_(nxt)
     ring[0].copy_(nxt, non_blocking=True)
     evs, amax = [step.event()], []
 
@@ -158,17 +233,19 @@
     for s in range(n_max - 1):
         if s >= 1 and read():
             break
-        ring[s + 1].copy_(step(ids[s], out=ids[s + 1]), non_blocking=True)
+        ring[s + 1].copy_(step(s) if loop else step(ids[s], out=ids[s + 1]), non_blocking=True)
         evs.append(step.event())
     while not all(done):
         read()
-    return new, amax
+    return handed(amax)
 
 
 def speculative(step, nxt, n_max, eos, draft):
     llm = step.llm
     kmax = max(llm.VERIFY_BUCKETS)
     new_ids, amax = [int(nxt.item())], [nxt]
+    if step.loop:
+        step.start(nxt)
     stats = dict(passes=0, plain_steps=0, proposed=0, accepted=0, pattern=[])
     observe = getattr(draft, "observe", None)
     while new_ids[-1] != eos and len(new_ids) < n_max:
@@ -177,7 +254,7 @@
         m = len(prop)
         if m == 0:
             stats["plain_steps"] += 1
-            amax.append(step(new_ids[-1]))
+            amax.append(step(step.n).clone() if step.loop else step(new_ids[-1]))
             new_ids.append(int(amax[-1].item()))
             continue
         kb = next(b for b in llm.VERIFY_BUCKETS if b >= m + 1)
@@ -207,4 +284,6 @@
         step.hidden[step.pos: step.pos + keep].copy_(st["hidden"][:keep])
         amax.extend(va[j: j + 1] for j in range(keep))
         step.resume(keep, st)
+    if step.loop:
+        step.finish()
     return new_ids, amax, stats
diff --git a/interactvlm_amd/llava.py b/interactvlm_amd/llava.py
--- a/interactvlm_amd/llava.py
+++ b/interactvlm_amd/llava.py
@@ -12,7 +12,7 @@
 BF16 = torch.bfloat16
 F32 = torch.float32
 
-_GraphKey = collections.namedtuple("_GraphKey", "batched B precision packed fp8 fused verify prefix", defaults=(False, False))
+_GraphKey = collections.namedtuple("_GraphKey", "batched B precision packed fp8 fused verify prefix loop", defaults=(False, False, False))
 
 
 class ClipTower:
@@ -460,7 +460,7 @@
             return bc[0].view(torch.float16)[:, :B], bc[1].view(torch.float16)[:, :B]
         return bc[0][:, :B], bc[1][:, :B]
 
-    def decode_step_batch(self, x, pos_dev, kc, vc, lo=None, prefix=None):
+    def decode_step_batch(self, x, pos_dev, kc, vc, lo=None, prefix=None, slab=None):
         c = self.cfg
         H, hd = c.heads, c.hidden // c.heads
         if x.shape[0] > 16:
@@ -473,10 +473,10 @@
                 self._prefix_scratch = ops.decode_attn_prefix_scratch(16, H, hd, self.norm.device)
             return self._decode_layers(x, lin, self._attn_then_o(lin, lambda qkv, li: (
                 ops.llama_decode_attn_batch_prefix(qkv, kc[li], vc[li], H, hd, pos_dev, prefix, c.theta, hd ** -0.5, table=self.rope,
-                                                   scratch=self._prefix_scratch))))
+                                                   scratch=self._prefix_scratch))), None if slab is None else (slab, pos_dev))
         return self._decode_layers(x, lin, self._attn_then_o(lin, lambda qkv, li: (
             ops.llama_decode_attn_batch(qkv, kc[li], vc[li], H, hd, pos_dev, c.theta, hd ** -0.5, table=self.rope,
-                                        lo=(lo[0][li], lo[1][li]) if lo is not None else None))))
+                                        lo=(lo[0][li], lo[1][li]) if lo is not None else None))), None if slab is None else (slab, pos_dev))
 
     @staticmethod
     def _planes(L, n):
@@ -484,13 +484,15 @@
             L[n + "_p"] = ops.PackedBf12(L[n]) if ops.PackedBf12.takes(*L[n].shape) else None
         return L[n + "_p"]
 
-    def _decode_layers(self, x, lin, attn_o):
+    def _decode_layers(self, x, lin, attn_o, slab=None):
         c = self.cfg
         for li, L in enumerate(self.layers):
             qkv = lin(x, L, "qkv", rms=(L["ln1"], c.eps))
             x = attn_o(qkv, li, L, x)
             h = lin(x, L, "gu", act="swiglu", rms=(L["ln2"], c.eps))
             x = lin(h, L, "down", residual=x)
+        if slab is not None:
+            return ops.rmsnorm_slab(x, self.norm, c.eps, *slab)
         return ops.rmsnorm(x, self.norm, c.eps, out_f32=True)
 
     @staticmethod
@@ -567,6 +569,48 @@
             st["prefix"].fill_(int(prefix))
         return st
 
+    def _loop_state(self, B):
+        i32 = lambda *n: torch.zeros(*n, dtype=torch.int32, device=self.device)
+        return dict(pos=i32(B), slot=i32(B), use_forced=i32(1), forced=i32(self.max_len, B), ring=i32(self.max_len + 1, B),
+                    slab=torch.zeros(B, self.max_len, self.cfg.hidden, dtype=F32, device=self.device))
+
+    def _loop_body(self, st, layers):
+        h = layers(ops.embed_feed(self.embed, st["forced"], st["ring"], st["use_forced"], st["slot"], self.max_len), st["slab"])
+        st["hidden"] = h
+        st["nxt"] = ops.argmax(self.logits(h), bump=st["pos"], file=(st["ring"], st["slot"]))
+
+    def decode_loop_graph(self, pos=None):
+        key = self._graph_key(1, batched=False)._replace(fused=False, loop=True)
+        st = self._graphs.get(key)
+        if st is None:
+            st = self._loop_state(1)
+            self._fused = None
+            caches = [self.kcache, self.vcache] + ([self.kcache_lo, self.vcache_lo] if self.precision == "parity" else [])
+            self._capture_decode(key, st, lambda: self._loop_body(st, lambda x, slab: self._decode_step(x, st["pos"], slab)), caches,
+                                 [st["pos"], st["slot"]])
+        if pos is not None:
+            st["pos"].fill_(pos)
+            st["slot"].zero_()
+        return st
+
+    def decode_loop_graph_batch(self, B, pos=None, prefix=None):
+        kc, vc = self.batch_cache(B)
+        lo = self.batch_cache_lo(B) if self.precision == "parity" else None
+        key = self._graph_key(B, batched=True)._replace(prefix=prefix is not None, loop=True)
+        st = self._graphs.get(key)
+        if st is None:
+            st = self._loop_state(B)
+            if prefix is not None:
+                st["prefix"] = torch.zeros(1, dtype=torch.int32, device=self.device)
+            self._capture_decode(key, st, lambda: self._loop_body(st, lambda x, slab: self.decode_step_batch(
+                x, st["pos"], kc, vc, lo, st.get("prefix"), slab)), [kc, vc] + list(lo or ()), [st["pos"], st["slot"]])
+        if pos is not None:
+            st["pos"].copy_(pos)
+            st["slot"].zero_()
+        if prefix is not None:
+            st["prefix"].fill_(int(prefix))
+        return st
+
     def _attn_scratch(self):
         if not (self.decode_splitkv or os.environ.get("IVLM_DECODE_SPLITKV", "0") == "1") or self.precision == "parity":
             return None
@@ -574,14 +618,15 @@
             self._dec_scratch = ops.decode_attn_scratch(self.cfg.heads, self.cfg.hidden // self.cfg.heads, self.norm.device)
         return self._dec_scratch
 
-    def _decode_step(self, x, pos):
-        c = self.cfg
+    def _decode_step(self, x, pos, slab=None):
+        c = self.cfg
+        slab = None if slab is None else (slab, pos)
         H, hd = c.heads, c.hidden // c.heads
         fz = self._fused if isinstance(pos, torch.Tensor) else None
         if self.fp8:
             lin = lambda x_, L, n, **kw: ops.linear_fp8w(x_, L[n + "_q"], L[n + "_s"], **kw)
             return self._decode_layers(x, lin, self._attn_then_o(lin, lambda qkv, li: ops.llama_decode_attn(
-                qkv, self.kcache[li], self.vcache[li], H, hd, pos, c.theta, hd ** -0.5, table=self.rope)))
+                qkv, self.kcache[li], self.vcache[li], H, hd, pos, c.theta, hd ** -0.5, table=self.rope)), slab)
         kc, vc = self._caches()
         packed = self.decode_packed and fz is None
         lin = self._lin("any" if packed else None)
@@ -602,7 +647,7 @@
             attn_o = lambda qkv, li, L, x: ops.llama_attn_oproj(
                 qkv, self.kcache[li], self.vcache[li], L["o"], x, H, hd, pos, fz["step"], fz["counters"][li], fz["status"], c.theta,
                 hd ** -0.5, self.rope, fz["scratch"][li])
-        return self._decode_layers(x, lin, attn_o)
+        return self._decode_layers(x, lin, attn_o, slab)
 
     def logits(self, hidden_rows):
         if hidden_rows.shape[0] > 16:
diff --git a/interactvlm_amd/model.py b/interactvlm_amd/model.py
--- a/interactvlm_amd/model.py
+++ b/interactvlm_amd/model.py
@@ -71,6 +71,7 @@
         self.debug_taps = None
         self.overlap_sam_encoder = True
         self.graph_decode = graphs.ON
+        self.loop_decode = os.environ.get("IVLM_DECODE_LOOP", "1") != "0"
         self.sam_after_prefill = bool(os.environ.get("IVLM_SAM_AFTER_PREFILL"))
         self.fused_lowres_lift = False
         self._side_stream = torch.cuda.Stream(device=dev) if dev.type == "cuda" else None
@@ -536,7 +537,10 @@
         return self._generated(ids, step, T0, new_ids)
 
     def _single_step(self, hidden_all, T0):
-        return (decoding.SingleGraph if graphs.enabled(self.graph_decode) else decoding.SingleEager)(self.llm, hidden_all, T0)
+        if not graphs.enabled(self.graph_decode):
+            return decoding.SingleEager(self.llm, hidden_all, T0)
+        loop = getattr(self, "loop_decode", False) and not self.llm._graph_key(1, batched=False).fused
+        return (decoding.SingleLoop if loop else decoding.SingleGraph)(self.llm, hidden_all, T0)
 
     def _generated(self, ids, step, T0, new_ids):
         if step.st is not None and self.llm.fused_wait_expired(step.st):
@@ -584,7 +588,9 @@
             pad = [list(map(int, f[:n])) + [eos_token_id] * (n_max - n) for f, n in zip(forced_new_tokens, n_seq)]
             forced = (pad, torch.tensor(pad, dtype=torch.int32, device=dev).t().contiguous())
         pos = torch.tensor(T0, dtype=torch.int32, device=dev)
-        if graphs.enabled(self.graph_decode):
+        if graphs.enabled(self.graph_decode) and getattr(self, "loop_decode", False):
+            step = decoding.BatchLoop(self.llm, hidden_all, pos, T0, prefix)
+        elif graphs.enabled(self.graph_decode):
             step = decoding.BatchGraph(self.llm, hidden_all, pos, prefix)
         else:
             step = decoding.BatchEager(self.llm, hidden_all, pos, (kc, vc, lo), prefix)
diff --git a/interactvlm_amd/ops.py b/interactvlm_amd/ops.py
--- a/interactvlm_amd/ops.py
+++ b/interactvlm_amd/ops.py
@@ -674,6 +674,34 @@
     return y
 
 
+def _i32(t, n, name):
+    assert t.dtype == torch.int32 and t.is_cuda and t.is_contiguous() and t.numel() == n, name
+    return t
+
+
+def rmsnorm_slab(x, weight, eps, slab, pos):
+    x = _req(x, F32, "x")
+    B, cols = x.shape
+    assert slab.dtype == F32 and slab.is_cuda and slab.is_contiguous() and slab.dim() == 3 and slab.shape[0] == B and slab.shape[2] == cols
+    y = torch.empty_like(x)
+    check(_lib.load().ivlm_rmsnorm_slab(x.data_ptr(), weight.data_ptr(), y.data_ptr(), slab.data_ptr(), _i32(pos, B, "pos").data_ptr(),
+                                        slab.shape[1], B, cols, float(eps), _stream()), "rmsnorm_slab")
+    return y
+
+
+def embed_feed(embed, forced, ring, use_forced, slot, n_slots, out=None):
+    assert embed.dtype == BF16 and embed.is_cuda and embed.dim() == 2 and embed.stride(1) == 1
+    B = slot.numel()
+    for t in (forced, ring):
+        assert t.dtype == torch.int32 and t.is_cuda and t.is_contiguous() and t.dim() == 2 and t.shape[1] == B and t.shape[0] >= n_slots
+    x = torch.empty(B, embed.shape[1], dtype=F32, device=embed.device) if out is None else out
+    assert x.dtype == F32 and x.is_cuda and x.is_contiguous() and x.shape == (B, embed.shape[1])
+    check(_lib.load().ivlm_embed_feed(x.data_ptr(), embed.data_ptr(), embed.stride(0), embed.shape[0], embed.shape[1], forced.data_ptr(),
+                                      ring.data_ptr(), _i32(use_forced, 1, "use_forced").data_ptr(), _i32(slot, B, "slot").data_ptr(),
+                                      int(n_slots), B, _stream()), "embed_feed")
+    return x
+
+
 def bf16_to_f16(w):
     w = w.contiguous()
     assert w.dtype == torch.bfloat16
@@ -851,11 +879,17 @@
     return rel_h, rel_w
 
 
-def argmax(logits, bump=None):
+def argmax(logits, bump=None, file=None):
     lib = _lib.load()
     logits = _req(logits, torch.float32, "logits")
     rows, cols = logits.shape
     out = torch.empty(rows, dtype=torch.int32, device=logits.device)
+    if file is not None:
+        ids, slot = file
+        assert ids.dtype == torch.int32 and ids.is_cuda and ids.is_contiguous() and ids.dim() == 2 and ids.shape[1] == rows
+        check(lib.ivlm_argmax_f32_file(logits.data_ptr(), rows, cols, out.data_ptr(), _p(_i32(bump, rows, "bump") if bump is not None else None),
+                                       ids.data_ptr(), _i32(slot, rows, "slot").data_ptr(), ids.shape[0], _stream()), "argmax_file")
+        return out
     if bump is not None:
         assert bump.dtype == torch.int32 and bump.is_cuda and bump.numel() == rows and bump.is_contiguous()
         check(lib.ivlm_argmax_f32_bump(logits.data_ptr(), rows, cols, out.data_ptr(), bump.data_ptr(), _stream()), "argmax_bump")
```

New measurement: 10.60. No clear change (-0.4%).
